# hasindu2008/sigtk

Measured on NVIDIA B200. Metric: event_detection_throughput, higher is better.
Workload: dtype f64

## Files before the change

### sigtk_b200/csrc/capi.cu

```cuda
#include "../../include/sigtk_b200.h"

#include <cstddef>
#include <cstdio>
#include <cstdlib>
#include <cstring>
#include <memory>
#include <new>
#include <utility>

#include "kernels.cuh"

using namespace sgpu;

namespace {

enum Out { EV_OFF, EV_START, EV_MEAN, EV_STDV, SEQ_ORDER, FIXUPS, STAT, ENT, JNN_CNT, JNN_SEG, PREFIX_POS, PREFIX_STAT,
           PA, N_OUT };
enum Live { LIVE_EV_OFF, LIVE_EV_START, LIVE_EV_LEN, LIVE_EV_MEAN, LIVE_EV_STDV, N_LIVE_OUT };
static_assert(EV_OFF == 0 && LIVE_EV_OFF == 0, "row 0 of both tables: ev_off, which sizes the event outputs");

enum Count : uint8_t {
    READS, READS_PLUS_1, EVENTS,
    SAMPLES,
    JNN_SLOTS,
};

constexpr int ANY_WANT = 0x100;

struct OutSpec {
    size_t field;
    uint32_t size;
    uint32_t want;
    Count count;
    uint32_t per;
    bool eager;
    int empty;
    bool pa_in;
};

#define OUTPUT(field, want, count, per, eager, empty, pa_in) \
    { offsetof(sgpu_result_t, field), sizeof *sgpu_result_t{}.field, want, count, per, eager, empty, pa_in }
constexpr OutSpec OUTS[] = {
    OUTPUT(ev_off,      SGPU_WANT_EVENTS, READS_PLUS_1, 1,   true,  0 | ANY_WANT, true),
    OUTPUT(ev_start,    SGPU_WANT_EVENTS, EVENTS,       1,   true,  -1,           true),
    OUTPUT(ev_mean,     SGPU_WANT_EVENTS, EVENTS,       1,   true,  -1,           true),
    OUTPUT(ev_stdv,     SGPU_WANT_EVENTS, EVENTS,       1,   true,  -1,           true),
    OUTPUT(seq_order,   SGPU_WANT_EVENTS, READS,        1,   true,  0,            true),
    OUTPUT(fixups,      SGPU_WANT_EVENTS, READS,        1,   true,  0,            true),
    OUTPUT(stat,        SGPU_WANT_STAT,   READS,        6,   true,  0,            false),
    OUTPUT(ent,         SGPU_WANT_ENT,    READS,        3,   false, 0,            false),
    OUTPUT(jnn_cnt,     SGPU_WANT_JNN,    READS,        1,   false, 0,            false),
    OUTPUT(jnn_seg,     SGPU_WANT_JNN,    JNN_SLOTS,    2,   false, -1,           false),
    OUTPUT(prefix_pos,  SGPU_WANT_PREFIX, READS,        4,   false, 0xff,         false),
    OUTPUT(prefix_stat, SGPU_WANT_PREFIX, READS,        6,   false, 0,            false),
    OUTPUT(pa,          SGPU_WANT_PA,     SAMPLES,      1,   false, -1,           false),
};
#undef OUTPUT
static_assert(sizeof OUTS / sizeof OUTS[0] == N_OUT, "one row per output");

#define LIVE_OUTPUT(field, count, empty) \
    { offsetof(sgpu_live_result_t, field), sizeof *sgpu_live_result_t{}.field, SGPU_WANT_EVENTS, count, 1, true, empty, \
      false }
constexpr OutSpec LIVE_OUTS[] = {
    LIVE_OUTPUT(ev_off,   READS_PLUS_1, 0 | ANY_WANT),
    LIVE_OUTPUT(ev_start, EVENTS,       -1),
    LIVE_OUTPUT(ev_len,   EVENTS,       -1),
    LIVE_OUTPUT(ev_mean,  EVENTS,       -1),
    LIVE_OUTPUT(ev_stdv,  EVENTS,       -1),
};
#undef LIVE_OUTPUT
static_assert(sizeof LIVE_OUTS / sizeof LIVE_OUTS[0] == N_LIVE_OUT, "one row per output");

constexpr uint32_t pa_input_wants(int k = 0) {
    return k == N_OUT ? 0u : (OUTS[k].pa_in ? OUTS[k].want : 0u) | pa_input_wants(k + 1);
}
constexpr bool pa_input_want_ok(uint32_t want) { return want != 0 && (want & ~pa_input_wants()) == 0; }
static_assert(pa_input_wants() == SGPU_WANT_EVENTS, "a pA run computes the event table only");

uint64_t out_elems(const OutSpec& s, uint64_t reads, uint64_t samples, uint64_t events) {
    switch (s.count) {
        case READS: return s.per * reads;
        case READS_PLUS_1: return s.per * (reads + 1);
        case EVENTS: return s.per * events;
        case SAMPLES: return s.per * samples;
        case JNN_SLOTS: return s.per * jnn_seg_capacity(samples, (uint32_t)reads);
    }
    return 0;
}

enum class Input : uint8_t { NONE, RAW, SVBZD, PA, LIVE, LIVE_PA };

bool is_live(Input k) { return k == Input::LIVE || k == Input::LIVE_PA; }

uint32_t allowed_wants(Input k) {
    if (k == Input::PA) return pa_input_wants();
    if (is_live(k)) return SGPU_WANT_EVENTS;
    return 63u;
}

struct Slot {
    sgpu_batch_t batch{};
    PinBuf<int16_t> samples;
    PinBuf<uint64_t> read_off;
    PinBuf<uint32_t> read_len;
    PinBuf<float> offset_f, raw_unit_f;
    uint64_t used = 0;
    DevBuf<int16_t> d_samples;
    DevBuf<uint64_t> d_read_off;
    DevBuf<uint32_t> d_read_len;
    DevBuf<float> d_offset, d_unit;
    DevBuf<void> dout[N_OUT];
    PinBuf<void> hout[N_OUT];
    PinBuf<unsigned long long> h_counters;
    PinBuf<int> h_status;
    cudaStream_t stream = nullptr;
    cudaEvent_t in_ready = nullptr, kernels_done = nullptr, small_back = nullptr;
    bool submitted = false;
    uint32_t want = 0;
    Input kind = Input::NONE;
    PinBuf<uint8_t> h_comp;
    DevBuf<uint8_t> d_comp;
    PinBuf<uint64_t> h_comp_off; DevBuf<uint64_t> d_comp_off;
    PinBuf<uint32_t> h_comp_len; DevBuf<uint32_t> d_comp_len;
    uint64_t comp_used = 0, svb_blocks = 0;
    PinBuf<uint32_t> h_channel, h_flags; DevBuf<uint32_t> d_channel, d_flags;
    DevBuf<void> live_dout[N_LIVE_OUT];
    PinBuf<void> live_hout[N_LIVE_OUT];
    std::unique_ptr<uint32_t[]> live_claim;
    uint32_t live_gen = 0;

    ~Slot() {
        if (stream) cudaStreamDestroy(stream);
        if (in_ready) cudaEventDestroy(in_ready);
        if (kernels_done) cudaEventDestroy(kernels_done);
        if (small_back) cudaEventDestroy(small_back);
    }
};

}

struct sgpu_ctx {
    int device = 0;
    int sm_count = 148;
    uint64_t max_samples = 0;
    uint32_t max_reads = 0;
    uint32_t n_slots = 0;
    uint32_t flags = 0;
    uint64_t ev_cap = 0;
    Scratch sc{};
    DevBuf<void> dev_out[N_OUT];
    std::unique_ptr<Slot[]> slots;
    SvbScratch svb{};
    DevBuf<float> jnn_mom;
    int pore_rna004 = 0;
    DevBuf<uint32_t> ent_ovf;
    PaScratch pa{};
    LiveScratch live{};
    DevBuf<void> live_dev_out[N_LIVE_OUT];
    std::unique_ptr<uint32_t[]> live_mirror;
    std::unique_ptr<uint8_t[]> live_form;
    bool live_mirror_stale = false;
    uint32_t live_gen = 0;
    uint64_t comp_cap = 0;
    cudaStream_t compute = nullptr;
    uint64_t last_launches = 0;
    static constexpr int MAX_STAGES = 16;
    cudaEvent_t stage_ev[MAX_STAGES + 1] = {};
    const char* stage_name[MAX_STAGES] = {};
    uint32_t stage_launches[MAX_STAGES] = {};
    int n_stages = 0;
    cudaStream_t stage_stream = nullptr;
    char err[512] = {0};

    ~sgpu_ctx() {
        if (compute) cudaStreamDestroy(compute);
        for (cudaEvent_t e : stage_ev) if (e) cudaEventDestroy(e);
    }
};

namespace {

bool cuda_fail(sgpu_ctx* c, cudaError_t e, const char* what, int line) {
    if (e == cudaSuccess) return false;
    if (c) snprintf(c->err, sizeof c->err, "%s: %s (%s) at capi.cu:%d", what, cudaGetErrorName(e),
                    cudaGetErrorString(e), line);
    return true;
}
#define CU(call)                                                         \
    do {                                                                 \
        if (cuda_fail(ctx, (call), #call, __LINE__)) return SGPU_E_CUDA; \
    } while (0)

uint64_t align_up(uint64_t v, uint64_t a) { return (v + a - 1) / a * a; }

template <size_t N, bool PINNED>
cudaError_t alloc_outputs(const OutSpec (&outs)[N], const sgpu_ctx* ctx, uint64_t ev_cap, Buf<void, PINNED>* o,
                          uint32_t want) {
    for (size_t k = 0; k < N; k++) {
        if (!outs[k].eager && !(want & outs[k].want)) continue;
        const uint64_t n = out_elems(outs[k], ctx->max_reads, ctx->max_samples, ev_cap);
        const cudaError_t e = o[k].ensure(n * outs[k].size);
        if (e != cudaSuccess) return e;
    }
    return cudaSuccess;
}

template <size_t N, typename R, bool PINNED>
void fill_result(const OutSpec (&outs)[N], R* r, const Buf<void, PINNED>* o, uint32_t want, bool all_eager) {
    for (size_t k = 0; k < N; k++)
        if ((want & outs[k].want) || (all_eager && outs[k].eager)) {
            void* const p = o[k];
            memcpy(reinterpret_cast<char*>(r) + outs[k].field, &p, sizeof p);
        }
}

template <size_t N>
cudaError_t queue_d2h(const OutSpec (&outs)[N], const DevBuf<void>* d, PinBuf<void>* h, const Slot& sl, uint32_t want,
                      bool by_events, uint64_t n_events) {
    for (size_t k = 0; k < N; k++) {
        if (!(want & outs[k].want) || (outs[k].count == EVENTS) != by_events) continue;
        const uint64_t n = out_elems(outs[k], sl.batch.n_reads, sl.used, n_events);
        const cudaError_t e = cudaMemcpyAsync(h[k], d[k], (size_t)n * outs[k].size, cudaMemcpyDeviceToHost, sl.stream);
        if (e != cudaSuccess) return e;
    }
    return cudaSuccess;
}

struct StageMarks {
    sgpu_ctx* ctx;
    cudaStream_t st;
    bool on;
    uint64_t launches = 0;
    StageMarks(sgpu_ctx* c, cudaStream_t s) : ctx(c), st(s), on((c->flags & SGPU_F_STAGE_TIMERS) != 0) {}
    int start() {
        CU(cudaMemsetAsync(ctx->sc.status, 0, sizeof(int), st));
        CU(cudaMemsetAsync(ctx->sc.counters, 0, 4 * sizeof(unsigned long long), st));
        ctx->n_stages = 0;
        ctx->stage_stream = st;
        if (on) cudaEventRecord(ctx->stage_ev[0], st);
        return SGPU_OK;
    }
    void done(const char* name, int n) {
        launches += (uint64_t)n;
        if (!on || ctx->n_stages >= sgpu_ctx::MAX_STAGES) return;
        const int k = ctx->n_stages++;
        ctx->stage_name[k] = name;
        ctx->stage_launches[k] = (uint32_t)n;
        cudaEventRecord(ctx->stage_ev[k + 1], st);
    }
    int finish() {
        CU(cudaGetLastError());
        ctx->last_launches = launches;
        return SGPU_OK;
    }
};

int alloc_svb_scratch(sgpu_ctx* ctx) {
    SvbScratch& w = ctx->svb;
    w.max_blocks = svbzd_max_blocks(ctx->max_samples, ctx->max_reads);
    CU(w.cnt.ensure(ctx->max_reads));
    CU(w.base.ensure((uint64_t)ctx->max_reads + 1));
    CU(w.blk_bytes.ensure(w.max_blocks));
    CU(w.blk_gpos.ensure(w.max_blocks + 1));
    CU(w.blk_sum.ensure(w.max_blocks));
    CU(w.blk_vpos.ensure(w.max_blocks + 1));
    CU(w.lane_sum.ensure(w.max_blocks * 32));
    CU(w.blk_read.ensure(w.max_blocks));
    return SGPU_OK;
}

template <size_t N>
int clear_empty_batch(const OutSpec (&outs)[N], uint64_t reads, uint64_t span, uint32_t want, DevBuf<void>* o,
                      StageMarks& run) {
    sgpu_ctx* const ctx = run.ctx;
    for (size_t k = 0; k < N; k++) {
        const OutSpec& s = outs[k];
        if (s.empty < 0 || !((want & s.want) || (s.empty & ANY_WANT))) continue;
        const uint64_t n = out_elems(s, reads, span, 0);
        if (n) CU(cudaMemsetAsync(o[k], s.empty & 0xff, (size_t)n * s.size, run.st));
    }
    return run.finish();
}

bool fits(const sgpu_ctx* ctx, const DevBatch& b) {
    return b.n_reads <= ctx->max_reads && b.span <= ctx->max_samples && !(b.span & (SGPU_ALIGN - 1));
}

int run_pipeline(sgpu_ctx* ctx, const DevBatch& b, uint32_t want, DevBuf<void>* o, cudaStream_t st,
                 const SvbBatch* svb = nullptr, int16_t* svb_out = nullptr) {
    Scratch& sc = ctx->sc;
    if (!fits(ctx, b)) return SGPU_E_INVAL;
    CU(alloc_outputs(OUTS, ctx, ctx->ev_cap, o, want));
    StageMarks marks(ctx, st);
    if (const int rc = marks.start()) return rc;
    if (b.n_reads == 0 || b.span == 0) return clear_empty_batch(OUTS, b.n_reads, b.span, want, o, marks);
    if (svb) marks.done("svbzd_decode", launch_svbzd_decode(*svb, ctx->svb, ctx->sc, svb_out, ctx->sm_count, st));
    const bool force_generic = (ctx->flags & SGPU_F_FORCE_GENERIC) != 0;
    const bool events = (want & SGPU_WANT_EVENTS) != 0;
    float* const pa = (want & SGPU_WANT_PA) ? static_cast<float*>(o[PA].get()) : nullptr;
    uint32_t* const seq = static_cast<uint32_t*>(o[SEQ_ORDER].get());
    uint32_t* const fix = static_cast<uint32_t*>(o[FIXUPS].get());
    if (pa && (!events || force_generic))
        marks.done("pa", launch_pa(b, pa, ctx->sm_count, st));
    if (want & SGPU_WANT_STAT) {
        float* const stat = static_cast<float*>(o[STAT].get());
        marks.done("stat_moments", launch_stat_moments(b, stat, ctx->sc.tune_stat_cta_min, ctx->sm_count, st));
        marks.done("stat_median", launch_stat_median(b, stat, ctx->sc.tune_stat_cta_min, ctx->sm_count, st));
    }
    if (want & SGPU_WANT_ENT) {
        if (!ctx->ent_ovf) {
            const uint64_t words = ent_overflow_words(ctx->sm_count);
            CU(ctx->ent_ovf.ensure(words));
            CU(cudaMemsetAsync(ctx->ent_ovf, 0, (size_t)words * sizeof(uint32_t), st));
        }
        marks.done("ent", launch_ent(b, ctx->ent_ovf, static_cast<double*>(o[ENT].get()), ctx->sm_count, st));
    }
    if (want & SGPU_WANT_JNN) {
        CU(ctx->jnn_mom.ensure((uint64_t)ctx->max_reads * 2));
        marks.done("jnn_moments", launch_jnn_moments(b, ctx->jnn_mom, ctx->sc.tune_stat_cta_min, ctx->sm_count, st));
        marks.done("jnn_walk", launch_jnn(b, ctx->jnn_mom, static_cast<uint32_t*>(o[JNN_CNT].get()),
                                          static_cast<int32_t*>(o[JNN_SEG].get()), ctx->sm_count, st));
    }
    if (want & SGPU_WANT_PREFIX)
        marks.done("prefix", launch_prefix(b, ctx->pore_rna004, static_cast<int32_t*>(o[PREFIX_POS].get()),
                                           static_cast<float*>(o[PREFIX_STAT].get()), ctx->sm_count, st));
    if (events) {
        const uint32_t n_tiles = fast_tiles_for(b.span);
        if (n_tiles > sc.max_tiles) return SGPU_E_INVAL;
        int n = launch_init_reads(b, sc, seq, fix, ctx->sm_count, st);
        if (force_generic) {
            CU(cudaMemsetAsync(sc.bitmap, 0, (size_t)n_tiles * (FAST_TILE / 32) * sizeof(uint32_t), st));
            marks.done("init", n);
        } else {
            marks.done("init", n);
            marks.done("walk_chunks", launch_walk(b, sc, pa, seq, ctx->sm_count, st));
            marks.done("long_jobs", launch_long_jobs(b, sc, seq, ctx->sm_count, st));
            marks.done("verify_chunks", launch_verify_chunks(b, sc, seq, fix, ctx->sm_count, st));
        }
        n = launch_build_seq_list(b, sc, seq, force_generic ? 1 : 0, ctx->sm_count, st);
        WorkList wl{sc.seq_list, sc.seq_sbase, sc.seq_count};
        n += launch_generic_detect(b, wl, sc, ctx->sm_count, st);
        marks.done("sequential_order_detect", n);
        uint64_t* const ev_off = static_cast<uint64_t*>(o[EV_OFF].get());
        uint32_t* const ev_start = static_cast<uint32_t*>(o[EV_START].get());
        float* const ev_mean = static_cast<float*>(o[EV_MEAN].get());
        float* const ev_stdv = static_cast<float*>(o[EV_STDV].get());
        marks.done("rank_events", launch_rank_events(b, sc, ev_off, ctx->sm_count, st));
        marks.done("emit_events",
                   launch_fast_emit(b, sc, ctx->ev_cap, ev_start, ev_mean, ev_stdv, fix, ctx->sm_count, st));
        marks.done("sequential_order_emit",
                   launch_generic_emit(b, wl, sc, ev_off, ctx->ev_cap, ev_start, ev_mean, ev_stdv, ctx->sm_count, st));
    }
    return marks.finish();
}

int alloc_pa_scratch(sgpu_ctx* ctx) {
    PaScratch& w = ctx->pa;
    w.max_tiles = pa_tile_capacity(ctx->max_samples, ctx->max_reads);
    CU(w.tile_cnt.ensure(ctx->max_reads));
    CU(w.tile_base.ensure((uint64_t)ctx->max_reads + 1));
    CU(w.tS.ensure(w.max_tiles));
    CU(w.tQ.ensure(w.max_tiles));
    CU(w.tA.ensure(w.max_tiles));
    CU(w.tB.ensure(w.max_tiles));
    CU(w.tmin.ensure(w.max_tiles));
    CU(w.ord_list.ensure(ctx->max_reads));
    CU(w.ord_sbase.ensure(ctx->max_reads));
    CU(w.ord_count.ensure(1));
    return SGPU_OK;
}

int grow_seq_scratch(sgpu_ctx* ctx) {
    Scratch& sc = ctx->sc;
    const uint64_t n = ctx->max_samples;
    DevBuf<double> S, Q;
    DevBuf<float> t1, t2;
    cudaError_t e = S.ensure(n);
    if (e == cudaSuccess) e = Q.ensure(n);
    if (e == cudaSuccess) e = t1.ensure(n);
    if (e == cudaSuccess) e = t2.ensure(n);
    if (e != cudaSuccess) {
        cudaGetLastError();
        snprintf(ctx->err, sizeof ctx->err, "growing the sequential-order scratch to %llu samples: %s",
                 (unsigned long long)n, cudaGetErrorString(e));
        return SGPU_E_NOMEM;
    }
    sc.Sinc = std::move(S); sc.Qinc = std::move(Q); sc.t1 = std::move(t1); sc.t2 = std::move(t2);
    sc.gen_cap = n;
    return SGPU_OK;
}

int run_pipeline_pa(sgpu_ctx* ctx, const DevBatch& b, const float* pa, uint32_t want, DevBuf<void>* o,
                    cudaStream_t st) {
    Scratch& sc = ctx->sc;
    if (!fits(ctx, b) || (b.n_reads && b.span && !pa)) return SGPU_E_INVAL;
    CU(alloc_outputs(OUTS, ctx, ctx->ev_cap, o, want));
    int rc = alloc_pa_scratch(ctx);
    if (!rc && b.span > sc.gen_cap) rc = grow_seq_scratch(ctx);
    if (rc) return rc;
    StageMarks marks(ctx, st);
    if ((rc = marks.start())) return rc;
    if (b.n_reads == 0 || b.span == 0) return clear_empty_batch(OUTS, b.n_reads, b.span, want, o, marks);
    const uint32_t n_tiles = fast_tiles_for(b.span);
    if (n_tiles > sc.max_tiles) return SGPU_E_INVAL;
    uint32_t* const seq = static_cast<uint32_t*>(o[SEQ_ORDER].get());
    uint32_t* const fix = static_cast<uint32_t*>(o[FIXUPS].get());
    CU(cudaMemsetAsync(sc.bitmap, 0, (size_t)n_tiles * (FAST_TILE / 32) * sizeof(uint32_t), st));
    const int force = (ctx->flags & SGPU_F_FORCE_GENERIC) ? 1 : 0;
    marks.done("pa_prefix", launch_pa_prefix(b, pa, ctx->pa, sc, seq, fix, force, ctx->sm_count, st));
    const WorkList ordered{ctx->pa.ord_list, ctx->pa.ord_sbase, ctx->pa.ord_count};
    const WorkList all{sc.seq_list, sc.seq_sbase, sc.seq_count};
    marks.done("sequential_order_detect", launch_generic_detect_pa(b, pa, ordered, all, sc, fix, ctx->sm_count, st));
    uint64_t* const ev_off = static_cast<uint64_t*>(o[EV_OFF].get());
    marks.done("rank_events", launch_rank_events(b, sc, ev_off, ctx->sm_count, st));
    marks.done("sequential_order_emit",
               launch_generic_emit(b, all, sc, ev_off, ctx->ev_cap, static_cast<uint32_t*>(o[EV_START].get()),
                                   static_cast<float*>(o[EV_MEAN].get()), static_cast<float*>(o[EV_STDV].get()),
                                   ctx->sm_count, st));
    return marks.finish();
}

int run_pipeline_live(sgpu_ctx* ctx, const LiveBatch& b, bool pa, DevBuf<void>* o, cudaStream_t st) {
    if (b.n_entries > ctx->max_reads || b.span > ctx->max_samples) return SGPU_E_INVAL;
    if (b.n_entries && (!b.samples || !b.read_off || !b.read_len || !b.channel || !b.flags ||
                        (!pa && (!b.offset || !b.unit))))
        return SGPU_E_INVAL;
    StageMarks marks(ctx, st);
    if (const int rc = marks.start()) return rc;
    if (b.n_entries == 0) return clear_empty_batch(LIVE_OUTS, 0, b.span, SGPU_WANT_EVENTS, o, marks);
    marks.done(pa ? "live_pa" : "live",
               launch_live(b, pa, ctx->live, ctx->sc, static_cast<uint64_t*>(o[LIVE_EV_OFF].get()),
                           static_cast<uint32_t*>(o[LIVE_EV_START].get()), static_cast<uint32_t*>(o[LIVE_EV_LEN].get()),
                           static_cast<float*>(o[LIVE_EV_MEAN].get()), static_cast<float*>(o[LIVE_EV_STDV].get()),
                           ctx->sm_count, st));
    return marks.finish();
}

int run_slot(sgpu_ctx* ctx, Slot& sl, uint32_t want) {
    const uint32_t nr = sl.batch.n_reads;
    const int rna = (int)sl.batch.rna;
    if (is_live(sl.kind)) {
        const LiveBatch b{sl.d_samples, sl.d_read_off, sl.d_read_len, sl.d_channel, sl.d_flags, sl.d_offset, sl.d_unit,
                          nr, sl.used};
        return run_pipeline_live(ctx, b, sl.kind == Input::LIVE_PA, sl.live_dout, ctx->compute);
    }
    CU(alloc_outputs(OUTS, ctx, ctx->ev_cap, sl.hout, want));
    if (sl.kind == Input::PA)
        return run_pipeline_pa(ctx, DevBatch{nullptr, sl.d_read_off, sl.d_read_len, nullptr, nullptr, nr, rna, sl.used},
                               reinterpret_cast<const float*>(sl.d_samples.get()), want, sl.dout, ctx->compute);
    const DevBatch b{sl.d_samples, sl.d_read_off, sl.d_read_len, sl.d_offset, sl.d_unit, nr, rna, sl.used};
    const SvbBatch svb{sl.d_comp, sl.comp_used, sl.d_comp_off, sl.d_comp_len, sl.d_read_off, sl.d_read_len, nr,
                       sl.svb_blocks};
    return run_pipeline(ctx, b, want, sl.dout, ctx->compute, sl.kind == Input::SVBZD ? &svb : nullptr, sl.d_samples);
}

bool accepts(const Slot& sl, Input k) { return !sl.submitted && (sl.kind == Input::NONE || sl.kind == k); }

int room_for(const sgpu_ctx* ctx, const Slot& sl, uint64_t n, uint64_t limit, uint64_t cap) {
    const uint64_t need = align_up(n, SGPU_ALIGN);
    if (n >= limit || need > cap) return SGPU_E_TOOBIG;
    if (sl.batch.n_reads >= ctx->max_reads || sl.used + need > cap) return SGPU_E_FULL;
    return SGPU_OK;
}

int64_t append_record(Slot& sl, uint64_t n, double digitisation, double offset, double range) {
    sgpu_batch_t& b = sl.batch;
    const uint32_t r = b.n_reads;
    b.read_off[r] = sl.used;
    b.read_len[r] = (uint32_t)n;
    const float range_f = (float)range, dig_f = (float)digitisation, off_f = (float)offset;
    volatile float unit = range_f / dig_f;
    b.offset_f[r] = off_f;
    b.raw_unit_f[r] = unit;
    sl.used += align_up(n, SGPU_ALIGN);
    b.n_reads = r + 1;
    b.read_off[r + 1] = sl.used;
    return (int64_t)r;
}

int add_live_entry(sgpu_ctx* ctx, Slot& sl, Input k, uint32_t channel, uint32_t flags, uint64_t n, uint64_t cap) {
    if (!accepts(sl, k) || !ctx->live.n_channels) return SGPU_E_STATE;
    if (channel >= ctx->live.n_channels || (flags & ~LIVE_FLAGS)) return SGPU_E_INVAL;
    if (const int rc = room_for(ctx, sl, n, 1ull << 31, cap)) return rc;
    if (sl.kind != k) {
        if (++ctx->live_gen == 0) {
            for (uint32_t s = 0; s < ctx->n_slots; s++)
                memset(ctx->slots[s].live_claim.get(), 0, (size_t)ctx->live.n_channels * sizeof(uint32_t));
            ctx->live_gen = 1;
        }
        sl.live_gen = ctx->live_gen;
    }
    if (sl.live_claim[channel] == sl.live_gen) return SGPU_E_INVAL;
    sl.live_claim[channel] = sl.live_gen;
    sl.kind = k;
    sl.h_channel[sl.batch.n_reads] = channel;
    sl.h_flags[sl.batch.n_reads] = flags;
    return SGPU_OK;
}

int map_dev_status(int s) {
    if (s == SGPU_DEV_E_EVCAP) return SGPU_E_EVCAP;
    if (s == SGPU_DEV_E_INVAL) return SGPU_E_INVAL;
    if (s == SGPU_DEV_E_STATE) return SGPU_E_STATE;
    if (s == SGPU_DEV_E_TOOBIG) return SGPU_E_TOOBIG;
    if (s == SGPU_DEV_E_SCRATCH) return SGPU_E_SCRATCH;
    if (s == SGPU_DEV_E_STREAM) return SGPU_E_STREAM;
    return SGPU_OK;
}

uint8_t live_form_of(Input k) { return k == Input::LIVE_PA ? LIVE_FORM_PA : LIVE_FORM_INT16; }

int check_live_entries(sgpu_ctx* ctx, const Slot& sl) {
    uint32_t* const mirror = ctx->live_mirror.get();
    uint8_t* const form = ctx->live_form.get();
    const uint32_t nc = ctx->live.n_channels;
    if (ctx->live_mirror_stale) {
        CU(cudaDeviceSynchronize());
        CU(cudaMemcpy(mirror, ctx->live.nopen, (size_t)nc * sizeof(uint32_t), cudaMemcpyDeviceToHost));
        CU(cudaMemcpy(form, ctx->live.form, (size_t)nc * sizeof(uint8_t), cudaMemcpyDeviceToHost));
        ctx->live_mirror_stale = false;
    }
    const uint8_t my_form = live_form_of(sl.kind);
    for (uint32_t e = 0; e < sl.batch.n_reads; e++) {
        const uint32_t c = sl.h_channel[e], f = sl.h_flags[e], no = mirror[c], len = sl.batch.read_len[e];
        const bool start = (f & SGPU_LIVE_START) != 0;
        if (!start && !(no & LIVE_OPEN) && (len || (f & SGPU_LIVE_END))) return SGPU_E_STATE;
        if (!start && (no & LIVE_OPEN) && form[c] != my_form) return SGPU_E_STATE;
        if ((start ? 0ull : (uint64_t)(no & ~LIVE_OPEN)) + len > 0x7fffffffull) return SGPU_E_TOOBIG;
    }
    return SGPU_OK;
}

void advance_live_mirror(sgpu_ctx* ctx, const Slot& sl) {
    uint32_t* const mirror = ctx->live_mirror.get();
    for (uint32_t e = 0; e < sl.batch.n_reads; e++) {
        const uint32_t c = sl.h_channel[e], f = sl.h_flags[e], no = mirror[c], len = sl.batch.read_len[e];
        const bool start = (f & SGPU_LIVE_START) != 0;
        if (!start && !(no & LIVE_OPEN)) continue;
        mirror[c] = (f & SGPU_LIVE_END) ? 0u : (uint32_t)((start ? 0u : (no & ~LIVE_OPEN)) + len) | LIVE_OPEN;
        if (start) ctx->live_form[c] = live_form_of(sl.kind);
    }
}

template <size_t N, typename R>
int wait_slot(sgpu_ctx* ctx, Slot& sl, const OutSpec (&outs)[N], const DevBuf<void>* d, PinBuf<void>* h,
              uint64_t ev_cap, R* out) {
    CU(cudaSetDevice(ctx->device));
    sl.submitted = false;
    CU(cudaEventSynchronize(sl.small_back));
    memset(out, 0, sizeof *out);
    const int dev_rc = map_dev_status(*sl.h_status);
    if (dev_rc) return dev_rc;
    const uint32_t nr = sl.batch.n_reads;
    if (sl.want & SGPU_WANT_EVENTS) {
        const uint64_t ne = nr ? static_cast<const uint64_t*>(h[0].get())[nr] : 0;
        if (ne > ev_cap) return SGPU_E_EVCAP;
        CU(queue_d2h(outs, d, h, sl, SGPU_WANT_EVENTS, true, ne));
        CU(cudaStreamSynchronize(sl.stream));
        out->n_events = ne;
    }
    fill_result(outs, out, h, sl.want, false);
    return SGPU_OK;
}

}

extern "C" {

int sgpu_abi_version(void) { return SGPU_ABI_VERSION; }

int sgpu_device_count(void) {
    int n = 0;
    if (cudaGetDeviceCount(&n) != cudaSuccess) return 0;
    return n;
}

const char* sgpu_strerror(int code) {
    switch (code) {
        case SGPU_OK: return "success";
        case SGPU_E_INVAL: return "invalid argument";
        case SGPU_E_CUDA: return "CUDA error (no usable B200 / kernel failure); there is no CPU fallback";
        case SGPU_E_NOMEM: return "out of memory";
        case SGPU_E_FULL: return "slot full";
        case SGPU_E_TOOBIG: return "read larger than the context's max_samples";
        case SGPU_E_STATE: return "call out of order";
        case SGPU_E_EVCAP: return "event capacity exceeded";
        case SGPU_E_SCRATCH: return "sequential-order scratch too small";
        case SGPU_E_STREAM: return "malformed svb-zd stream (length does not match its keys)";
        default: return "unknown error";
    }
}

const char* sgpu_last_error(const sgpu_ctx_t* ctx) { return ctx ? ctx->err : "no context"; }

int sgpu_create(sgpu_ctx_t** out, int device, uint64_t max_samples, uint32_t max_reads, uint32_t n_slots,
                uint32_t flags) {
    if (!out || max_samples == 0 || max_reads == 0 || (flags & ~15u)) return SGPU_E_INVAL;
    *out = nullptr;
    if (flags & SGPU_F_NO_HOST_SLOTS) n_slots = 0; else if (n_slots == 0) n_slots = 2;
    sgpu_ctx* ctx = new (std::nothrow) sgpu_ctx();
    if (!ctx) return SGPU_E_NOMEM;
    auto fail = [&](int code) { sgpu_destroy(ctx); return code; };
    {
        int ndev = 0;
        cudaError_t e = cudaGetDeviceCount(&ndev);
        if (e != cudaSuccess || device < 0 || device >= ndev) {
            fprintf(stderr, "[sigtk_b200] no usable CUDA device %d (%s); this library has no CPU fallback\n", device,
                    e == cudaSuccess ? "index out of range" : cudaGetErrorString(e));
            delete ctx;
            return SGPU_E_CUDA;
        }
    }
#define CUC(call)                                                               \
    do {                                                                        \
        if (cuda_fail(ctx, (call), #call, __LINE__)) {                          \
            fprintf(stderr, "[sigtk_b200] %s\n", ctx->err);                     \
            return fail(SGPU_E_CUDA);                                           \
        }                                                                       \
    } while (0)
    CUC(cudaSetDevice(device));
    ctx->device = device;
    cudaDeviceProp prop;
    CUC(cudaGetDeviceProperties(&prop, device));
    ctx->sm_count = prop.multiProcessorCount;
    max_samples = align_up(max_samples, 64);
    ctx->max_samples = max_samples;
    ctx->max_reads = max_reads;
    ctx->n_slots = n_slots;
    ctx->flags = flags;
    ctx->ev_cap = max_samples / 3 + 2ull * max_reads + 16;
    Scratch& sc = ctx->sc;
    sc.gen_cap = (max_samples <= (64ull << 20) || (flags & (SGPU_F_FORCE_GENERIC | SGPU_F_FULL_SEQ_SCRATCH)))
                     ? max_samples : max_samples / 8;
    CUC(sc.Sinc.ensure(sc.gen_cap));
    CUC(sc.Qinc.ensure(sc.gen_cap));
    CUC(sc.t1.ensure(sc.gen_cap));
    CUC(sc.t2.ensure(sc.gen_cap));
    sc.max_tiles = fast_tiles_for(max_samples) + 1;
    sc.bitmap_words = (uint64_t)sc.max_tiles * (FAST_TILE / 32);
    CUC(sc.bitmap.ensure(sc.bitmap_words));
    sc.wk_slots = walk_state_slots(max_samples, max_reads);
    CUC(sc.wk_begin.ensure(sc.wk_slots * 8));
    CUC(sc.wk_end.ensure(sc.wk_slots * 8));
    CUC(sc.wk_cnt.ensure(max_reads));
    CUC(sc.wk_ibase.ensure((uint64_t)max_reads + 1));
    sc.job_cap = walk_job_capacity(max_samples);
    CUC(sc.jobs.ensure((uint64_t)sc.job_cap * 4));
    CUC(sc.job_count.ensure(1));
    sc.tune_chunk_len = 0; sc.tune_warmup = 0; sc.tune_thr_long = 9.0f;
    sc.tune_stat_cta_min = STAT_CTA_MIN_DEFAULT;
    CUC(sc.tile_cnt.ensure(sc.max_tiles));
    CUC(sc.tile_read0.ensure(sc.max_tiles));
    CUC(sc.tile_base.ensure((uint64_t)sc.max_tiles + 1));
    CUC(sc.wit_min.ensure(max_reads));
    CUC(sc.wit_max.ensure(max_reads));
    CUC(sc.seq_list.ensure(max_reads));
    CUC(sc.seq_sbase.ensure((uint64_t)max_reads + 1));
    CUC(sc.seq_count.ensure(1));
    CUC(sc.cursor.ensure(1));
    {
        uint64_t most = sc.max_tiles > max_reads ? sc.max_tiles : max_reads;
        const uint64_t svb_blocks = svbzd_max_blocks(max_samples, max_reads);
        if (svb_blocks > most) most = svb_blocks;
        CUC(sc.scan_status.ensure(scan_tiles_for((uint32_t)most) + 1));
    }
    ctx->comp_cap = 2 * max_samples;
    if (flags & SGPU_F_STAGE_TIMERS)
        for (int k = 0; k <= sgpu_ctx::MAX_STAGES; k++) CUC(cudaEventCreate(&ctx->stage_ev[k]));
    CUC(sc.scan_ticket.ensure(1));
    CUC(sc.status.ensure(1));
    CUC(sc.counters.ensure(4));
    CUC(cudaStreamCreateWithFlags(&ctx->compute, cudaStreamNonBlocking));
    CUC(alloc_outputs(OUTS, ctx, ctx->ev_cap, ctx->dev_out, 0));
    if (n_slots) {
        ctx->slots.reset(new (std::nothrow) Slot[n_slots]);
        if (!ctx->slots) return fail(SGPU_E_NOMEM);
        for (uint32_t s = 0; s < n_slots; s++) {
            Slot& sl = ctx->slots[s];
            CUC(sl.samples.ensure(max_samples));
            CUC(sl.read_off.ensure((uint64_t)max_reads + 1));
            CUC(sl.read_len.ensure(max_reads));
            CUC(sl.offset_f.ensure(max_reads));
            CUC(sl.raw_unit_f.ensure(max_reads));
            CUC(sl.d_samples.ensure(max_samples));
            CUC(sl.d_read_off.ensure((uint64_t)max_reads + 1));
            CUC(sl.d_read_len.ensure(max_reads));
            CUC(sl.d_offset.ensure(max_reads));
            CUC(sl.d_unit.ensure(max_reads));
            CUC(alloc_outputs(OUTS, ctx, ctx->ev_cap, sl.dout, 0));
            CUC(alloc_outputs(OUTS, ctx, ctx->ev_cap, sl.hout, 0));
            CUC(sl.h_counters.ensure(4));
            CUC(sl.h_status.ensure(1));
            CUC(cudaStreamCreateWithFlags(&sl.stream, cudaStreamNonBlocking));
            CUC(cudaEventCreateWithFlags(&sl.in_ready, cudaEventDisableTiming));
            CUC(cudaEventCreateWithFlags(&sl.kernels_done, cudaEventDisableTiming));
            CUC(cudaEventCreateWithFlags(&sl.small_back, cudaEventDisableTiming));
            sl.batch = sgpu_batch_t{sl.samples, sl.read_off, sl.read_len, sl.offset_f, sl.raw_unit_f, 0, 0};
            sl.batch.read_off[0] = 0;
        }
    }
#undef CUC
    *out = ctx;
    return SGPU_OK;
}

void sgpu_destroy(sgpu_ctx_t* ctx) {
    if (!ctx) return;
    cudaSetDevice(ctx->device);
    cudaDeviceSynchronize();
    delete ctx;
}

int sgpu_slot_batch(sgpu_ctx_t* ctx, uint32_t slot, sgpu_batch_t** out) {
    if (!ctx || !out || slot >= ctx->n_slots) return SGPU_E_INVAL;
    *out = &ctx->slots[slot].batch;
    return SGPU_OK;
}

int sgpu_slot_reset(sgpu_ctx_t* ctx, uint32_t slot, uint32_t rna) {
    if (!ctx || slot >= ctx->n_slots) return SGPU_E_INVAL;
    Slot& sl = ctx->slots[slot];
    if (sl.submitted) return SGPU_E_STATE;
    sl.batch.n_reads = 0;
    sl.batch.rna = rna ? 1u : 0u;
    sl.batch.read_off[0] = 0;
    sl.used = 0;
    sl.kind = Input::NONE;
    sl.comp_used = 0;
    sl.svb_blocks = 0;
    return SGPU_OK;
}

int64_t sgpu_slot_add_read(sgpu_ctx_t* ctx, uint32_t slot, const int16_t* raw, uint64_t n, double digitisation,
                           double offset, double range) {
    if (!ctx || slot >= ctx->n_slots || (!raw && n)) return SGPU_E_INVAL;
    Slot& sl = ctx->slots[slot];
    if (!accepts(sl, Input::RAW)) return SGPU_E_STATE;
    if (const int rc = room_for(ctx, sl, n, 1ull << 31, ctx->max_samples)) return rc;
    sl.kind = Input::RAW;
    memcpy(sl.batch.samples + sl.used, raw, (size_t)n * sizeof(int16_t));
    return append_record(sl, n, digitisation, offset, range);
}

int64_t sgpu_slot_add_read_svbzd(sgpu_ctx_t* ctx, uint32_t slot, const uint8_t* stream, uint64_t n_bytes,
                                 double digitisation, double offset, double range) {
    if (!ctx || slot >= ctx->n_slots || !stream) return SGPU_E_INVAL;
    Slot& sl = ctx->slots[slot];
    if (!accepts(sl, Input::SVBZD)) return SGPU_E_STATE;
    if (n_bytes != 0 && n_bytes < 4) return SGPU_E_STREAM;
    uint32_t count = 0;
    if (n_bytes) memcpy(&count, stream, 4);
    const uint64_t n = count;
    if (n_bytes && (4u + (n + 3u) / 4u + n > n_bytes || n_bytes > 4u + (n + 3u) / 4u + 4u * n)) return SGPU_E_STREAM;
    const uint64_t cneed = align_up(n_bytes, 16);
    if (n_bytes > 0xffffffffull || cneed > ctx->comp_cap) return SGPU_E_TOOBIG;
    if (const int rc = room_for(ctx, sl, n, 1ull << 31, ctx->max_samples)) return rc;
    if (sl.comp_used + cneed > ctx->comp_cap) return SGPU_E_FULL;
    if (sl.kind != Input::SVBZD) {
        CU(cudaSetDevice(ctx->device));
        const int rc = alloc_svb_scratch(ctx);
        if (rc) return rc;
        CU(sl.h_comp.ensure(ctx->comp_cap));
        CU(sl.d_comp.ensure(ctx->comp_cap + 16));
        CU(sl.h_comp_off.ensure(ctx->max_reads));
        CU(sl.d_comp_off.ensure(ctx->max_reads));
        CU(sl.h_comp_len.ensure(ctx->max_reads));
        CU(sl.d_comp_len.ensure(ctx->max_reads));
    }
    sl.kind = Input::SVBZD;
    const uint32_t r = sl.batch.n_reads;
    if (n_bytes) memcpy(sl.h_comp + sl.comp_used, stream, (size_t)n_bytes);
    sl.h_comp_off[r] = sl.comp_used;
    sl.h_comp_len[r] = (uint32_t)n_bytes;
    sl.comp_used += cneed;
    sl.svb_blocks += svbzd_blocks_of(n);
    return append_record(sl, n, digitisation, offset, range);
}

int64_t sgpu_slot_add_read_pa(sgpu_ctx_t* ctx, uint32_t slot, const float* pa, uint64_t n) {
    if (!ctx || slot >= ctx->n_slots || (!pa && n)) return SGPU_E_INVAL;
    Slot& sl = ctx->slots[slot];
    if (!accepts(sl, Input::PA)) return SGPU_E_STATE;
    if (const int rc = room_for(ctx, sl, n, 1ull << 32, ctx->max_samples / 2)) return rc;
    sl.kind = Input::PA;
    memcpy(reinterpret_cast<float*>(sl.batch.samples) + sl.used, pa, (size_t)n * sizeof(float));
    return append_record(sl, n, 1.0, 0.0, 1.0);
}

int sgpu_submit(sgpu_ctx_t* ctx, uint32_t slot, uint32_t want) {
    if (!ctx || slot >= ctx->n_slots || (want & ~63u) || want == 0) return SGPU_E_INVAL;
    Slot& sl = ctx->slots[slot];
    if (sl.submitted) return SGPU_E_STATE;
    if (want & ~allowed_wants(sl.kind)) return SGPU_E_INVAL;
    CU(cudaSetDevice(ctx->device));
    const bool live = is_live(sl.kind);
    int rc = live ? check_live_entries(ctx, sl) : SGPU_OK;
    if (rc) return rc;
    const sgpu_batch_t& hb = sl.batch;
    const uint32_t nr = hb.n_reads;
    cudaStream_t st = sl.stream;
    if (sl.kind == Input::SVBZD) {
        CU(cudaMemcpyAsync(sl.d_comp, sl.h_comp, (size_t)sl.comp_used, cudaMemcpyHostToDevice, st));
        CU(cudaMemcpyAsync(sl.d_comp_off, sl.h_comp_off, (size_t)nr * sizeof(uint64_t), cudaMemcpyHostToDevice, st));
        CU(cudaMemcpyAsync(sl.d_comp_len, sl.h_comp_len, (size_t)nr * sizeof(uint32_t), cudaMemcpyHostToDevice, st));
    } else {
        const size_t sample_size = sl.kind == Input::PA || sl.kind == Input::LIVE_PA ? sizeof(float) : sizeof(int16_t);
        CU(cudaMemcpyAsync(sl.d_samples, hb.samples, (size_t)sl.used * sample_size, cudaMemcpyHostToDevice, st));
    }
    CU(cudaMemcpyAsync(sl.d_read_off, hb.read_off, ((size_t)nr + 1) * sizeof(uint64_t), cudaMemcpyHostToDevice, st));
    CU(cudaMemcpyAsync(sl.d_read_len, hb.read_len, (size_t)nr * sizeof(uint32_t), cudaMemcpyHostToDevice, st));
    CU(cudaMemcpyAsync(sl.d_offset, hb.offset_f, (size_t)nr * sizeof(float), cudaMemcpyHostToDevice, st));
    CU(cudaMemcpyAsync(sl.d_unit, hb.raw_unit_f, (size_t)nr * sizeof(float), cudaMemcpyHostToDevice, st));
    if (live) {
        CU(cudaMemcpyAsync(sl.d_channel, sl.h_channel, (size_t)nr * sizeof(uint32_t), cudaMemcpyHostToDevice, st));
        CU(cudaMemcpyAsync(sl.d_flags, sl.h_flags, (size_t)nr * sizeof(uint32_t), cudaMemcpyHostToDevice, st));
    }
    CU(cudaEventRecord(sl.in_ready, st));
    CU(cudaStreamWaitEvent(ctx->compute, sl.in_ready, 0));
    rc = run_slot(ctx, sl, want);
    if (rc) return rc;
    CU(cudaMemcpyAsync(sl.h_counters, ctx->sc.counters, 4 * sizeof(unsigned long long), cudaMemcpyDeviceToHost,
                       ctx->compute));
    CU(cudaMemcpyAsync(sl.h_status, ctx->sc.status, sizeof(int), cudaMemcpyDeviceToHost, ctx->compute));
    CU(cudaEventRecord(sl.kernels_done, ctx->compute));
    CU(cudaStreamWaitEvent(st, sl.kernels_done, 0));
    CU(live ? queue_d2h(LIVE_OUTS, sl.live_dout, sl.live_hout, sl, want, false, 0)
            : queue_d2h(OUTS, sl.dout, sl.hout, sl, want, false, 0));
    CU(cudaEventRecord(sl.small_back, st));
    if (live) advance_live_mirror(ctx, sl);
    sl.want = want;
    sl.submitted = true;
    return SGPU_OK;
}

int sgpu_wait(sgpu_ctx_t* ctx, uint32_t slot, sgpu_result_t* out) {
    if (!ctx || slot >= ctx->n_slots || !out) return SGPU_E_INVAL;
    Slot& sl = ctx->slots[slot];
    if (!sl.submitted || is_live(sl.kind)) return SGPU_E_STATE;
    return wait_slot(ctx, sl, OUTS, sl.dout, sl.hout, ctx->ev_cap, out);
}

int sgpu_run_device(sgpu_ctx_t* ctx, const sgpu_dev_batch_t* batch, uint32_t want, void* stream,
                    sgpu_result_t* out) {
    if (!ctx || !batch || !out || (want & ~63u) || want == 0) return SGPU_E_INVAL;
    CU(cudaSetDevice(ctx->device));
    DevBatch b{batch->samples, batch->read_off, batch->read_len, batch->offset_f, batch->raw_unit_f,
               batch->n_reads, (int)batch->rna, batch->span};
    const int rc = run_pipeline(ctx, b, want, ctx->dev_out, reinterpret_cast<cudaStream_t>(stream));
    if (rc) return rc;
    memset(out, 0, sizeof *out);
    fill_result(OUTS, out, ctx->dev_out, want, true);
    return SGPU_OK;
}

int sgpu_run_device_pa(sgpu_ctx_t* ctx, const sgpu_dev_pa_batch_t* batch, uint32_t want, void* stream,
                       sgpu_result_t* out) {
    if (!ctx || !batch || !out || !pa_input_want_ok(want)) return SGPU_E_INVAL;
    CU(cudaSetDevice(ctx->device));
    const DevBatch b{nullptr, batch->read_off, batch->read_len, nullptr, nullptr, batch->n_reads, (int)batch->rna,
                     batch->span};
    const int rc = run_pipeline_pa(ctx, b, batch->pa, want, ctx->dev_out, reinterpret_cast<cudaStream_t>(stream));
    if (rc) return rc;
    memset(out, 0, sizeof *out);
    fill_result(OUTS, out, ctx->dev_out, want, false);
    return SGPU_OK;
}

int sgpu_decode_svbzd_device(sgpu_ctx_t* ctx, const sgpu_svb_dev_batch_t* batch, int16_t* samples_out, void* stream) {
    if (!ctx || !batch || !samples_out) return SGPU_E_INVAL;
    if (batch->n_reads > ctx->max_reads || batch->n_blocks > svbzd_max_blocks(ctx->max_samples, ctx->max_reads))
        return SGPU_E_INVAL;
    CU(cudaSetDevice(ctx->device));
    const int arc = alloc_svb_scratch(ctx);
    if (arc) return arc;
    cudaStream_t st = reinterpret_cast<cudaStream_t>(stream);
    CU(cudaMemsetAsync(ctx->sc.status, 0, sizeof(int), st));
    SvbBatch s{batch->bytes, batch->n_bytes, batch->comp_off, batch->comp_len, batch->read_off, batch->read_len,
               batch->n_reads, batch->n_blocks};
    ctx->last_launches = (uint64_t)launch_svbzd_decode(s, ctx->svb, ctx->sc, samples_out, ctx->sm_count, st);
    CU(cudaGetLastError());
    return SGPU_OK;
}

int sgpu_counters(sgpu_ctx_t* ctx, sgpu_counters_t* out) {
    if (!ctx || !out) return SGPU_E_INVAL;
    CU(cudaSetDevice(ctx->device));
    CU(cudaDeviceSynchronize());
    unsigned long long c[4];
    int status = 0;
    CU(cudaMemcpy(c, ctx->sc.counters, sizeof c, cudaMemcpyDeviceToHost));
    CU(cudaMemcpy(&status, ctx->sc.status, sizeof status, cudaMemcpyDeviceToHost));
    out->n_events = c[0];
    out->n_seq_order_reads = c[1];
    out->n_fixups = c[2];
    out->n_kernel_launches = ctx->last_launches;
    out->status = map_dev_status(status);
    out->n_long_jobs = c[3];
    return SGPU_OK;
}

int sgpu_set_param(sgpu_ctx_t* ctx, int key, double value) {
    if (!ctx) return SGPU_E_INVAL;
    Scratch& sc = ctx->sc;
    switch (key) {
        case SGPU_PARAM_CHUNK_LEN:
            if (value < 0 || value > (double)(1u << 20)) return SGPU_E_INVAL;
            sc.tune_chunk_len = (uint32_t)value;
            return SGPU_OK;
        case SGPU_PARAM_WARMUP:
            if (value < 0 || value > 4096) return SGPU_E_INVAL;
            sc.tune_warmup = (uint32_t)value;
            return SGPU_OK;
        case SGPU_PARAM_PORE:
            if (value != 0 && value != 1) return SGPU_E_INVAL;
            ctx->pore_rna004 = (int)value;
            return SGPU_OK;
        case SGPU_PARAM_STAT_CTA_MIN:
            if (value < 0 || value > 4294967295.0) return SGPU_E_INVAL;
            sc.tune_stat_cta_min = (uint32_t)value;
            return SGPU_OK;
        case SGPU_PARAM_THR_LONG:
            if (!(value > 0 && value < 1e6)) return SGPU_E_INVAL;
            sc.tune_thr_long = (float)value;
            return SGPU_OK;
        default: return SGPU_E_INVAL;
    }
}

int sgpu_stage_times(sgpu_ctx_t* ctx, sgpu_stage_time_t* out, uint32_t cap) {
    if (!ctx || (!out && cap)) return SGPU_E_INVAL;
    if (!(ctx->flags & SGPU_F_STAGE_TIMERS)) return SGPU_E_STATE;
    CU(cudaSetDevice(ctx->device));
    if (ctx->n_stages == 0) return 0;
    CU(cudaEventSynchronize(ctx->stage_ev[ctx->n_stages]));
    int n = 0;
    for (int k = 0; k < ctx->n_stages && (uint32_t)k < cap; k++, n++) {
        float ms = 0.0f;
        CU(cudaEventElapsedTime(&ms, ctx->stage_ev[k], ctx->stage_ev[k + 1]));
        out[k].name = ctx->stage_name[k];
        out[k].ms = ms;
        out[k].launches = ctx->stage_launches[k];
    }
    return n;
}

int sgpu_memcpy_d2h(sgpu_ctx_t* ctx, void* dst, const void* src, uint64_t bytes) {
    if (!ctx || (!dst && bytes) || (!src && bytes)) return SGPU_E_INVAL;
    CU(cudaSetDevice(ctx->device));
    CU(cudaDeviceSynchronize());
    if (bytes) CU(cudaMemcpy(dst, src, (size_t)bytes, cudaMemcpyDeviceToHost));
    return SGPU_OK;
}

int sgpu_live_open(sgpu_ctx_t* ctx, uint32_t n_channels) {
    if (!ctx || n_channels == 0) return SGPU_E_INVAL;
    LiveScratch& w = ctx->live;
    if (w.n_channels) return SGPU_E_STATE;
    CU(cudaSetDevice(ctx->device));
    w.ev_cap = live_stage_base(ctx->max_samples, ctx->max_reads);
    CU(w.chan.ensure(n_channels));
    CU(w.nopen.ensure(n_channels));
    CU(w.claim.ensure(n_channels));
    CU(w.form.ensure(n_channels));
    CU(w.cnt.ensure(ctx->max_reads));
    CU(w.s_start.ensure(w.ev_cap));
    CU(w.s_len.ensure(w.ev_cap));
    CU(w.s_mean.ensure(w.ev_cap));
    CU(w.s_stdv.ensure(w.ev_cap));
    CU(cudaMemset(w.nopen, 0, (size_t)n_channels * sizeof(uint32_t)));
    CU(cudaMemset(w.claim, 0, (size_t)n_channels * sizeof(uint32_t)));
    CU(cudaMemset(w.form, LIVE_FORM_INT16, (size_t)n_channels * sizeof(uint8_t)));
    ctx->live_mirror.reset(new (std::nothrow) uint32_t[n_channels]());
    ctx->live_form.reset(new (std::nothrow) uint8_t[n_channels]());
    if (!ctx->live_mirror || !ctx->live_form) return SGPU_E_NOMEM;
    for (uint32_t s = 0; s < ctx->n_slots; s++) {
        Slot& sl = ctx->slots[s];
        CU(sl.h_channel.ensure(ctx->max_reads));
        CU(sl.h_flags.ensure(ctx->max_reads));
        CU(sl.d_channel.ensure(ctx->max_reads));
        CU(sl.d_flags.ensure(ctx->max_reads));
        CU(alloc_outputs(LIVE_OUTS, ctx, w.ev_cap, sl.live_dout, 0));
        CU(alloc_outputs(LIVE_OUTS, ctx, w.ev_cap, sl.live_hout, 0));
        sl.live_claim.reset(new (std::nothrow) uint32_t[n_channels]());
        if (!sl.live_claim) return SGPU_E_NOMEM;
    }
    w.n_channels = n_channels;
    return SGPU_OK;
}

int64_t sgpu_slot_add_live(sgpu_ctx_t* ctx, uint32_t slot, uint32_t channel, uint32_t flags, const int16_t* raw,
                           uint64_t n, double digitisation, double offset, double range) {
    if (!ctx || slot >= ctx->n_slots || (!raw && n)) return SGPU_E_INVAL;
    Slot& sl = ctx->slots[slot];
    if (const int rc = add_live_entry(ctx, sl, Input::LIVE, channel, flags, n, ctx->max_samples)) return rc;
    memcpy(sl.batch.samples + sl.used, raw, (size_t)n * sizeof(int16_t));
    return append_record(sl, n, digitisation, offset, range);
}

int64_t sgpu_slot_add_live_pa(sgpu_ctx_t* ctx, uint32_t slot, uint32_t channel, uint32_t flags, const float* pa,
                              uint64_t n) {
    if (!ctx || slot >= ctx->n_slots || (!pa && n)) return SGPU_E_INVAL;
    Slot& sl = ctx->slots[slot];
    if (const int rc = add_live_entry(ctx, sl, Input::LIVE_PA, channel, flags, n, ctx->max_samples / 2)) return rc;
    memcpy(reinterpret_cast<float*>(sl.batch.samples) + sl.used, pa, (size_t)n * sizeof(float));
    return append_record(sl, n, 1.0, 0.0, 1.0);
}

int sgpu_wait_live(sgpu_ctx_t* ctx, uint32_t slot, sgpu_live_result_t* out) {
    if (!ctx || slot >= ctx->n_slots || !out) return SGPU_E_INVAL;
    Slot& sl = ctx->slots[slot];
    if (!sl.submitted || !is_live(sl.kind)) return SGPU_E_STATE;
    return wait_slot(ctx, sl, LIVE_OUTS, sl.live_dout, sl.live_hout, ctx->live.ev_cap, out);
}

int sgpu_run_device_live(sgpu_ctx_t* ctx, const sgpu_dev_live_batch_t* batch, void* stream, sgpu_live_result_t* out) {
    if (!ctx || !batch || !out) return SGPU_E_INVAL;
    if (!ctx->live.n_channels) return SGPU_E_STATE;
    CU(cudaSetDevice(ctx->device));
    CU(alloc_outputs(LIVE_OUTS, ctx, ctx->live.ev_cap, ctx->live_dev_out, 0));
    const LiveBatch b{batch->samples, batch->read_off, batch->read_len, batch->channel, batch->flags, batch->offset_f,
                      batch->raw_unit_f, batch->n_entries, batch->span};
    const int rc = run_pipeline_live(ctx, b, false, ctx->live_dev_out, reinterpret_cast<cudaStream_t>(stream));
    if (rc) return rc;
    ctx->live_mirror_stale = true;
    memset(out, 0, sizeof *out);
    fill_result(LIVE_OUTS, out, ctx->live_dev_out, SGPU_WANT_EVENTS, false);
    return SGPU_OK;
}

int sgpu_run_device_live_pa(sgpu_ctx_t* ctx, const sgpu_dev_live_pa_batch_t* batch, void* stream,
                            sgpu_live_result_t* out) {
    if (!ctx || !batch || !out) return SGPU_E_INVAL;
    if (!ctx->live.n_channels) return SGPU_E_STATE;
    CU(cudaSetDevice(ctx->device));
    CU(alloc_outputs(LIVE_OUTS, ctx, ctx->live.ev_cap, ctx->live_dev_out, 0));
    LiveBatch b{nullptr, batch->read_off, batch->read_len, batch->channel, batch->flags, nullptr, nullptr,
                batch->n_entries, batch->span};
    b.pa = batch->pa;
    const int rc = run_pipeline_live(ctx, b, true, ctx->live_dev_out, reinterpret_cast<cudaStream_t>(stream));
    if (rc) return rc;
    ctx->live_mirror_stale = true;
    memset(out, 0, sizeof *out);
    fill_result(LIVE_OUTS, out, ctx->live_dev_out, SGPU_WANT_EVENTS, false);
    return SGPU_OK;
}

}
```

### sigtk_b200/csrc/common.cuh

```cuda
#pragma once
#include <cuda_runtime.h>
#include <float.h>
#include <stdint.h>

namespace sgpu {

struct DetParams {
    int w1, w2;
    float thr1, thr2;
    float height;
};

__host__ __device__ inline DetParams det_params(int rna) {
    DetParams p;
    if (rna) { p.w1 = 7; p.w2 = 14; p.thr1 = 2.5f; p.thr2 = 9.0f; p.height = 1.0f; }
    else     { p.w1 = 3; p.w2 = 6;  p.thr1 = 1.4f; p.thr2 = 9.0f; p.height = 0.2f; }
    return p;
}

struct DevBatch {
    const int16_t*  samples;
    const uint64_t* read_off;
    const uint32_t* read_len;
    const float*    offset;
    const float*    unit;
    uint32_t n_reads;
    int      rna;
    uint64_t span;
};

__device__ __forceinline__ float pa_of(int16_t raw, float off, float unit) {
    return __fmul_rn(__fadd_rn((float)raw, off), unit);
}

__device__ __forceinline__ float tstat_reference_chain(double sum1, double ssq1, double sum2d,
                                                       double ssq2d, float wf) {
    const double wd = (double)wf;
    const float sum2 = __double2float_rn(sum2d);
    const float ssq2 = __double2float_rn(ssq2d);
    const float mean1 = __double2float_rn(__ddiv_rn(sum1, wd));
    const float mean2 = __fdiv_rn(sum2, wf);
    const float m1sq = __fmul_rn(mean1, mean1);
    const float m2sq = __fmul_rn(mean2, mean2);
    const float v2 = __fdiv_rn(ssq2, wf);
    double acc = __ddiv_rn(ssq1, wd);
    acc = __dsub_rn(acc, (double)m1sq);
    acc = __dadd_rn(acc, (double)v2);
    acc = __dsub_rn(acc, (double)m2sq);
    const float cv = fmaxf(__double2float_rn(acc), FLT_MIN);
    const float delta = __fsub_rn(mean2, mean1);
    const float scaled = __fdiv_rn(cv, wf);
    return __double2float_rn(__ddiv_rn(fabs((double)delta), __dsqrt_rn((double)scaled)));
}


__device__ __forceinline__ void event_stats(double dsum, double dssq, uint32_t len, float* mean,
                                            float* stdv) {
    const float lenf = (float)len;
    const float m = __fdiv_rn(__double2float_rn(dsum), lenf);
    const float ex2 = __fdiv_rn(__double2float_rn(dssq), lenf);
    const float var = __fsub_rn(ex2, __fmul_rn(m, m));
    *mean = m;
    *stdv = __fsqrt_rn(fmaxf(var, 0.0f));
}

struct DetState {
    uint32_t masked_to;
    int32_t  peak_pos;
    float    peak_value;
    int32_t  valid;
};

__device__ __forceinline__ void det_reset(DetState& d) {
    d.masked_to = 0; d.peak_pos = -1; d.peak_value = FLT_MAX; d.valid = 0;
}

__device__ __forceinline__ int32_t det_step(DetState& d, DetState* other_long, bool is_short, uint32_t i,
                                            float cur, float thr, int w, float height) {
    if (d.masked_to >= i) return -1;
    if (d.peak_pos < 0) {
        if (cur < d.peak_value) {
            d.peak_value = cur;
        } else if (__fsub_rn(cur, d.peak_value) > height) {
            d.peak_value = cur;
            d.peak_pos = (int32_t)i;
        }
        return -1;
    }
    if (cur > d.peak_value) { d.peak_value = cur; d.peak_pos = (int32_t)i; }
    if (is_short && d.peak_value > thr) {
        other_long->masked_to = (uint32_t)d.peak_pos + (uint32_t)w;
        other_long->peak_pos = -1;
        other_long->peak_value = FLT_MAX;
        other_long->valid = 0;
    }
    if (__fsub_rn(d.peak_value, cur) > height && d.peak_value > thr) d.valid = 1;
    if (d.valid && (i - (uint32_t)d.peak_pos) > (uint32_t)(w / 2)) {
        const int32_t out = d.peak_pos;
        d.peak_pos = -1;
        d.peak_value = cur;
        d.valid = 0;
        return out;
    }
    return -1;
}

static inline int grid_cap(uint64_t work, int block, int max_blocks) {
    uint64_t g = (work + block - 1) / block;
    if (g < 1) g = 1;
    if (g > (uint64_t)max_blocks) g = max_blocks;
    return (int)g;
}

__device__ __forceinline__ uint32_t find_read(const uint64_t* __restrict__ off, uint32_t n, uint64_t p) {
    uint32_t lo = 0, hi = n;
    while (hi - lo > 1) {
        const uint32_t mid = (lo + hi) >> 1;
        if (off[mid] <= p) lo = mid; else hi = mid;
    }
    return lo;
}

}
```

### sigtk_b200/csrc/emit.cu

```cuda
#include "kernels.cuh"
#include "walk_core.cuh"

namespace sgpu {

namespace {

constexpr int EWT = 1024;
constexpr int EWARPS = 4;
constexpr int ELIST = EWT / 2 + 8;
constexpr int EFAST = EWT / 3 + 8;
constexpr int ELONG = 48;

struct EmitWarp {
    double S[EFAST + 32];
    double Q[EFAST + 32];
    uint16_t list[ELIST];
};

__device__ __forceinline__ uint32_t locate_read(const DevBatch& b, uint32_t r0, uint64_t p) {
    uint32_t r = r0;
#pragma unroll 1
    for (int k = 0; k < 4; k++) {
        if (r + 1 >= b.n_reads || b.read_off[r + 1] > p) return r;
        r++;
    }
    return find_read(b.read_off, b.n_reads, p);
}

__device__ __forceinline__ void add_raw(int raw, float off, float unit, double& as, double& aq) {
    const float x = __fmul_rn(__fadd_rn((float)raw, off), unit);
    as = __dadd_rn(as, walk::widen_pos(x));
    aq = __dadd_rn(aq, walk::widen_pos(__fmul_rn(x, x)));
}
__device__ __forceinline__ void add_raw_any(int raw, float off, float unit, double& as, double& aq, bool safe) {
    const float x = __fmul_rn(__fadd_rn((float)raw, off), unit);
    if (!safe || x > 0.0f) {
        as = __dadd_rn(as, walk::widen_pos(x));
        aq = __dadd_rn(aq, walk::widen_pos(__fmul_rn(x, x)));
    } else {
        as = __dadd_rn(as, (double)x);
        aq = __dadd_rn(aq, (double)__fmul_rn(x, x));
    }
}

__device__ __forceinline__ long long next_start(const uint32_t* __restrict__ bitmap, uint64_t w0, uint64_t n_words,
                                                long long rend) {
    for (uint64_t w = w0; w < n_words && (long long)(w << 5) < rend; w++) {
        const uint32_t nx = bitmap[w];
        if (nx) {
            const long long e = (long long)(w << 5) + __ffs(nx) - 1;
            return e < rend ? e : rend;
        }
    }
    return rend;
}

}

#ifndef EMIT_MINB
#define EMIT_MINB 7
#endif
#ifndef EMIT_GRID
#define EMIT_GRID 64
#endif
__global__ void __launch_bounds__(EWARPS * 32, EMIT_MINB) emit_events_kernel(DevBatch b, uint32_t n_tiles,
                                                                  const uint32_t* __restrict__ bitmap,
                                                                  const uint64_t* __restrict__ tile_base, uint64_t ev_cap,
                                                                  uint32_t* __restrict__ ev_start,
                                                                  float* __restrict__ ev_mean, float* __restrict__ ev_stdv,
                                                                  int* __restrict__ status,
                                                                  const uint32_t* __restrict__ tile_read0) {
    __shared__ EmitWarp smem[EWARPS];
    const int lane = threadIdx.x & 31;
    EmitWarp& sm = smem[threadIdx.x >> 5];
    const uint64_t n_wt = (uint64_t)n_tiles * (FAST_TILE / EWT);
    const uint64_t n_words = (uint64_t)n_tiles * (FAST_TILE / 32);
    const uint64_t warp0 = (uint64_t)blockIdx.x * EWARPS + (threadIdx.x >> 5), n_warps = (uint64_t)gridDim.x * EWARPS;
    const long long span = (long long)b.span;
    auto load_tile = [&](uint64_t wt, uint32_t& word, int4 (&rv)[4]) {
        const long long p0 = (long long)wt * EWT + lane * 32;
        word = 0u;
#pragma unroll
        for (int g = 0; g < 4; g++) rv[g] = make_int4(0, 0, 0, 0);
        if (wt < n_wt && (long long)wt * EWT < span) {
            word = bitmap[wt * 32 + lane];
            const int4* __restrict__ src = reinterpret_cast<const int4*>(b.samples + p0);
#pragma unroll
            for (int g = 0; g < 4; g++) if (p0 + 8 * g + 8 <= span) rv[g] = __ldg(src + g);
        }
    };
    uint32_t word_n;
    int4 rv_n[4];
    load_tile(warp0, word_n, rv_n);
    for (uint64_t wt = warp0; wt < n_wt; wt += n_warps) {
        const long long flat0 = (long long)wt * EWT;
        if (flat0 >= span) break;
        const uint32_t tile = (uint32_t)(wt / (FAST_TILE / EWT)), half = (uint32_t)(wt % (FAST_TILE / EWT));
        const uint32_t word = word_n;
        int4 rv[4];
#pragma unroll
        for (int g = 0; g < 4; g++) rv[g] = rv_n[g];
        load_tile(wt + n_warps, word_n, rv_n);
        const uint64_t tbase = tile_base[tile];
        const uint32_t tr0_raw = tile_read0[tile];
        const uint32_t tr0 = tr0_raw & 0x7fffffffu;
        const bool tile_low = (tr0_raw >> 31) != 0u;
        uint32_t before = half ? (uint32_t)__popc(bitmap[(uint64_t)tile * (FAST_TILE / 32) + lane]) : 0u;
        before = __reduce_add_sync(0xffffffffu, before);
        uint32_t incl = __popc(word);
        const uint32_t own = incl;
#pragma unroll
        for (int o = 1; o < 32; o <<= 1) {
            const uint32_t t = __shfl_up_sync(0xffffffffu, incl, o);
            if (lane >= o) incl += t;
        }
        uint32_t total = __shfl_sync(0xffffffffu, incl, 31);
        if (total == 0u) continue;
        if (total > (uint32_t)ELIST) { total = ELIST; if (lane == 0) atomicExch(status, SGPU_DEV_E_EVCAP); }
        __syncwarp();
        {
            uint32_t rem = word, idx = incl - own;
            while (rem) {
                if (idx < (uint32_t)ELIST) sm.list[idx] = (uint16_t)(lane * 32 + __ffs(rem) - 1);
                idx++;
                rem &= rem - 1u;
            }
        }
        const uint64_t kbase = tbase + before;
        const uint32_t r_first = locate_read(b, tr0, (uint64_t)flat0);
        const long long rs_first = (long long)b.read_off[r_first];
        const long long rend_first = rs_first + (long long)b.read_len[r_first];
        const float off_first = b.offset[r_first], unit_first = b.unit[r_first];
        const bool one_read = rs_first <= flat0 && flat0 + EWT <= rend_first && total <= (uint32_t)EFAST && !tile_low;
        if (one_read) {
            const uint64_t w_next = (wt + 1) * 32 + (uint64_t)lane;
            const bool w_valid = w_next < n_words && (long long)(w_next << 5) < rend_first;
            const uint32_t next_bits = w_valid ? bitmap[w_next] : 0u;
            const long long i_behind = flat0 + EWT + lane;
            const int raw_behind = i_behind < rend_first ? (int)__ldg(b.samples + i_behind) : 0;
            int slot = EFAST + lane;
            int next = (int)(incl - own);
            double as = 0.0, aq = 0.0;
#pragma unroll
            for (int g = 0; g < 4; g++) {
                const int v[4] = {rv[g].x, rv[g].y, rv[g].z, rv[g].w};
                float x[8];
                walk::cvt8(v, off_first, unit_first, x);
                float xq[8];
#pragma unroll
                for (int m = 0; m < 8; m += 2) {
                    const walk::F2 p = {x[m], x[m + 1]};
                    const walk::F2 q = walk::f2sq(p);
                    xq[m] = q.lo; xq[m + 1] = q.hi;
                }
#pragma unroll
                for (int m = 0; m < 8; m++) {
                    if ((word >> (8 * g + m)) & 1u) {
                        sm.S[slot] = as;
                        sm.Q[slot] = aq;
                        slot = next++;
                        as = 0.0;
                        aq = 0.0;
                    }
                    as = __dadd_rn(as, walk::widen_pos(x[m]));
                    aq = __dadd_rn(aq, walk::widen_pos(xq[m]));
                }
            }
            sm.S[slot] = as;
            sm.Q[slot] = aq;
            __syncwarp();
            const uint32_t nz = __ballot_sync(0xffffffffu, own != 0u);
            if (own != 0u && incl != own) {
                double hs = sm.S[EFAST + lane], hq = sm.Q[EFAST + lane];
                const uint32_t lower = nz & ((1u << lane) - 1u);
                for (int l2 = lane - 1; l2 > 31 - __clz(lower); l2--) {
                    hs = __dadd_rn(hs, sm.S[EFAST + l2]);
                    hq = __dadd_rn(hq, sm.Q[EFAST + l2]);
                }
                const int prev = (int)(incl - own) - 1;
                sm.S[prev] = __dadd_rn(sm.S[prev], hs);
                sm.Q[prev] = __dadd_rn(sm.Q[prev], hq);
            }
            __syncwarp();
            const int last_word = 31 - __clz(nz);
            long long e_tail;
            {
                const uint32_t m = __ballot_sync(0xffffffffu, next_bits != 0u);
                const uint32_t all_valid = __ballot_sync(0xffffffffu, w_valid);
                if (m) {
                    const int l0 = __ffs(m) - 1;
                    const uint32_t bits0 = __shfl_sync(0xffffffffu, next_bits, l0);
                    e_tail = (long long)(((wt + 1) * 32 + (uint64_t)l0) << 5) + __ffs(bits0) - 1;
                    if (e_tail > rend_first) e_tail = rend_first;
                } else if (all_valid == 0xffffffffu) {
                    e_tail = next_start(bitmap, (wt + 2) * 32, n_words, rend_first);
                } else {
                    e_tail = rend_first;
                }
            }
            double tail_s = lane > last_word ? sm.S[EFAST + lane] : 0.0, tail_q = lane > last_word ? sm.Q[EFAST + lane] : 0.0;
            if (i_behind < e_tail) add_raw_any(raw_behind, off_first, unit_first, tail_s, tail_q, true);
            for (long long i = i_behind + 32; i < e_tail; i += 32) add_raw_any((int)__ldg(b.samples + i), off_first, unit_first, tail_s, tail_q, true);
#pragma unroll
            for (int o = 16; o; o >>= 1) {
                tail_s = __dadd_rn(tail_s, __shfl_xor_sync(0xffffffffu, tail_s, o));
                tail_q = __dadd_rn(tail_q, __shfl_xor_sync(0xffffffffu, tail_q, o));
            }
            for (uint32_t j0 = 0; j0 < total; j0 += 32) {
                const uint32_t j = j0 + lane;
                if (j >= total) continue;
                const int pos = sm.list[j];
                double es = sm.S[j], eq = sm.Q[j];
                long long e;
                if (j + 1 < total) {
                    e = flat0 + sm.list[j + 1];
                } else {
                    es = __dadd_rn(es, tail_s);
                    eq = __dadd_rn(eq, tail_q);
                    e = e_tail;
                }
                const uint64_t k = kbase + j;
                if (k >= ev_cap) { atomicExch(status, SGPU_DEV_E_EVCAP); continue; }
                const long long s = flat0 + pos;
                float mean, stdv;
                event_stats(es, eq, (uint32_t)(e - s), &mean, &stdv);
                ev_start[k] = (uint32_t)(s - rs_first);
                ev_mean[k] = mean;
                ev_stdv[k] = stdv;
            }
            continue;
        }
        __syncwarp();
        const bool safe = true;
        for (uint32_t j0 = 0; j0 < total; j0 += 32) {
            const uint32_t j = j0 + lane;
            const bool have = j < total;
            long long i = 0, e = 0, rs = 0;
            float off = 0.0f, unit = 0.0f;
            double as = 0.0, aq = 0.0;
            uint32_t len = 0;
            if (have) {
                const long long s = flat0 + sm.list[j];
                const uint32_t r = locate_read(b, r_first, (uint64_t)s);
                rs = (long long)b.read_off[r];
                const long long rend = rs + (long long)b.read_len[r];
                off = b.offset[r];
                unit = b.unit[r];
                e = j + 1 < total ? flat0 + sm.list[j + 1] : next_start(bitmap, (wt + 1) * 32, n_words, rend);
                if (e > rend) e = rend;
                len = (uint32_t)(e - s);
                i = s;
                const long long stop = e - s > ELONG ? s + ELONG : e;
                for (; i < stop; i++) add_raw_any((int)__ldg(b.samples + i), off, unit, as, aq, safe);
            }
            uint32_t longs = __ballot_sync(0xffffffffu, have && i < e);
            while (longs) {
                const int src = __ffs(longs) - 1;
                longs &= longs - 1u;
                const long long li = __shfl_sync(0xffffffffu, i, src), le = __shfl_sync(0xffffffffu, e, src);
                const float lo = __shfl_sync(0xffffffffu, off, src), lu = __shfl_sync(0xffffffffu, unit, src);
                double ps = 0.0, pq = 0.0;
                for (long long p = li + lane; p < le; p += 32) add_raw_any((int)__ldg(b.samples + p), lo, lu, ps, pq, safe);
#pragma unroll
                for (int o = 16; o; o >>= 1) {
                    ps = __dadd_rn(ps, __shfl_xor_sync(0xffffffffu, ps, o));
                    pq = __dadd_rn(pq, __shfl_xor_sync(0xffffffffu, pq, o));
                }
                if (lane == src) { as = __dadd_rn(as, ps); aq = __dadd_rn(aq, pq); }
            }
            if (have) {
                const uint64_t k = kbase + j;
                if (k >= ev_cap) { atomicExch(status, SGPU_DEV_E_EVCAP); continue; }
                float mean, stdv;
                event_stats(as, aq, len, &mean, &stdv);
                ev_start[k] = (uint32_t)(e - (long long)len - rs);
                ev_mean[k] = mean;
                ev_stdv[k] = stdv;
            }
        }
    }
}

__global__ void __launch_bounds__(256) sum_fixups_kernel(uint32_t n_reads, const uint32_t* __restrict__ fixups,
                                                         unsigned long long* __restrict__ counters) {
    unsigned long long acc = 0;
    for (uint32_t r = blockIdx.x * blockDim.x + threadIdx.x; r < n_reads; r += gridDim.x * blockDim.x) acc += fixups[r];
    if (acc) atomicAdd(&counters[2], acc);
}

int launch_fast_emit(const DevBatch& b, Scratch& sc, uint64_t ev_cap, uint32_t* ev_start, float* ev_mean,
                     float* ev_stdv, const uint32_t* fixups, int sm_count, cudaStream_t st) {
    const uint32_t n_tiles = fast_tiles_for(b.span);
    const uint64_t n_wt = (uint64_t)n_tiles * (FAST_TILE / EWT);
    emit_events_kernel<<<grid_cap(n_wt, EWARPS, sm_count * EMIT_GRID), EWARPS * 32, 0, st>>>(
        b, n_tiles, sc.bitmap, sc.tile_base, ev_cap, ev_start, ev_mean, ev_stdv, sc.status, sc.tile_read0);
    sum_fixups_kernel<<<grid_cap(b.n_reads, 256, sm_count * 4), 256, 0, st>>>(b.n_reads, fixups, sc.counters);
    return 2;
}

}
```

### sigtk_b200/csrc/kernels.cuh

```cuda
#pragma once
#include <type_traits>

#include "common.cuh"

namespace sgpu {

template <typename T, bool PINNED = false>
class Buf {
  public:
    Buf() = default;
    Buf(const Buf&) = delete;
    Buf& operator=(const Buf&) = delete;
    Buf(Buf&& o) noexcept : p_(o.p_) { o.p_ = nullptr; }
    Buf& operator=(Buf&& o) noexcept {
        if (this != &o) { release(); p_ = o.p_; o.p_ = nullptr; }
        return *this;
    }
    ~Buf() { release(); }

    cudaError_t ensure(uint64_t count) {
        if (p_) return cudaSuccess;
        size_t bytes = (size_t)(count ? count : 1);
        if constexpr (!std::is_void_v<T>) bytes *= sizeof(T);
        void* q = nullptr;
        const cudaError_t e = PINNED ? cudaHostAlloc(&q, bytes, cudaHostAllocDefault) : cudaMalloc(&q, bytes);
        if (e == cudaSuccess) p_ = static_cast<T*>(q);
        return e;
    }
    T* get() const { return p_; }
    operator T*() const { return p_; }

  private:
    void release() {
        if (!p_) return;
        if (PINNED) cudaFreeHost(p_); else cudaFree(p_);
    }
    T* p_ = nullptr;
};
template <typename T> using DevBuf = Buf<T, false>;
template <typename T> using PinBuf = Buf<T, true>;

enum { SGPU_DEV_OK = 0, SGPU_DEV_E_EVCAP = 1, SGPU_DEV_E_SCRATCH = 2, SGPU_DEV_E_STREAM = 3, SGPU_DEV_E_INVAL = 4,
       SGPU_DEV_E_STATE = 5, SGPU_DEV_E_TOOBIG = 6 };

constexpr int FAST_TILE = 2048;

struct WorkList {
    const uint32_t* list;
    const uint64_t* sbase;
    const uint32_t* count;
};

struct Scratch {
    DevBuf<double> Sinc, Qinc; DevBuf<float> t1, t2;
    uint64_t gen_cap;
    DevBuf<uint32_t> bitmap; uint64_t bitmap_words;
    DevBuf<uint32_t> tile_cnt; DevBuf<uint64_t> tile_base;
    DevBuf<uint32_t> tile_read0;
    DevBuf<uint32_t> wk_cnt;
    DevBuf<uint64_t> wk_ibase;
    DevBuf<int> wk_begin, wk_end;
    uint64_t wk_slots;
    DevBuf<int> jobs;
    DevBuf<uint32_t> job_count;
    uint32_t job_cap;
    uint32_t tune_chunk_len, tune_warmup;
    float tune_thr_long;
    uint32_t tune_stat_cta_min;
    uint32_t max_tiles;
    DevBuf<uint32_t> wit_min, wit_max;
    DevBuf<uint32_t> seq_list;
    DevBuf<uint64_t> seq_sbase;
    DevBuf<uint32_t> seq_count;
    DevBuf<unsigned long long> cursor;
    DevBuf<unsigned long long> scan_status; DevBuf<uint32_t> scan_ticket;
    DevBuf<int> status; DevBuf<unsigned long long> counters;
};

int launch_generic_detect(const DevBatch& b, const WorkList& wl, Scratch& sc, int sm_count, cudaStream_t st);
int launch_generic_emit(const DevBatch& b, const WorkList& wl, Scratch& sc, const uint64_t* ev_off, uint64_t ev_cap,
                        uint32_t* ev_start, float* ev_mean, float* ev_stdv, int sm_count, cudaStream_t st);
int launch_generic_detect_pa(const DevBatch& b, const float* pa, const WorkList& ordered, const WorkList& all,
                             Scratch& sc, uint32_t* fixups, int sm_count, cudaStream_t st);
int launch_scan_u32(const uint32_t* cnt, uint32_t n, uint64_t* off, uint64_t* total_out, Scratch& sc, cudaStream_t st);
uint32_t scan_tiles_for(uint32_t n);

uint32_t fast_tiles_for(uint64_t span);
int launch_init_reads(const DevBatch& b, Scratch& sc, uint32_t* seq_flag, uint32_t* fixups, int sm_count,
                      cudaStream_t st);
int launch_walk(const DevBatch& b, Scratch& sc, float* pa_out, uint32_t* seq_flag, int sm_count, cudaStream_t st);
int launch_long_jobs(const DevBatch& b, Scratch& sc, uint32_t* seq_flag, int sm_count, cudaStream_t st);
int launch_verify_chunks(const DevBatch& b, Scratch& sc, uint32_t* seq_flag, uint32_t* fixups, int sm_count, cudaStream_t st);
uint64_t walk_state_slots(uint64_t max_samples, uint32_t max_reads);
uint32_t walk_chunk_len(uint64_t span, uint32_t n_reads, int rna, int sm_count, uint32_t forced);
uint32_t walk_warmup(int rna, uint32_t forced);
uint32_t walk_job_capacity(uint64_t max_samples);
int launch_build_seq_list(const DevBatch& b, Scratch& sc, uint32_t* seq_flag, int force_all, int sm_count,
                          cudaStream_t st);
int launch_rank_events(const DevBatch& b, Scratch& sc, uint64_t* ev_off, int sm_count, cudaStream_t st);
int launch_fast_emit(const DevBatch& b, Scratch& sc, uint64_t ev_cap, uint32_t* ev_start, float* ev_mean,
                     float* ev_stdv, const uint32_t* fixups, int sm_count, cudaStream_t st);
int launch_pa(const DevBatch& b, float* pa, int sm_count, cudaStream_t st);

struct PaScratch {
    DevBuf<uint32_t> tile_cnt;
    DevBuf<uint64_t> tile_base;
    DevBuf<double> tS, tQ;
    DevBuf<double> tA, tB;
    DevBuf<uint2> tmin;
    DevBuf<uint32_t> ord_list;
    DevBuf<uint64_t> ord_sbase; DevBuf<uint32_t> ord_count;
    uint64_t max_tiles;
};
uint64_t pa_tile_capacity(uint64_t max_samples, uint32_t max_reads);
int launch_pa_prefix(const DevBatch& b, const float* pa, PaScratch& w, Scratch& sc, uint32_t* seq_flag,
                     uint32_t* fixups, int force_all, int sm_count, cudaStream_t st);

struct SvbBatch {
    const uint8_t*  bytes;
    uint64_t        n_bytes;
    const uint64_t* comp_off;
    const uint32_t* comp_len;
    const uint64_t* read_off;
    const uint32_t* read_len;
    uint32_t n_reads;
    uint64_t n_blocks;
};
struct SvbScratch {
    DevBuf<uint32_t> cnt; DevBuf<uint64_t> base;
    DevBuf<uint32_t> blk_bytes; DevBuf<uint64_t> blk_gpos;
    DevBuf<uint32_t> blk_sum; DevBuf<uint64_t> blk_vpos;
    DevBuf<uint32_t> lane_sum;
    DevBuf<uint32_t> blk_read;
    uint64_t max_blocks;
};
uint64_t svbzd_max_blocks(uint64_t max_samples, uint32_t max_reads);
uint32_t svbzd_blocks_of(uint64_t n);
int launch_svbzd_decode(const SvbBatch& s, SvbScratch& w, Scratch& sc, int16_t* samples, int sm_count, cudaStream_t st);

constexpr uint32_t LIVE_FLAGS = 7u;
constexpr uint32_t LIVE_OPEN = 1u << 31;
constexpr int LIVE_TAIL = 28;
constexpr uint8_t LIVE_FORM_INT16 = 0, LIVE_FORM_PA = 1;
struct LiveChan {
    double tS[LIVE_TAIL], tQ[LIVE_TAIL];
    double pS[2], pQ[2];
    double aS, aQ;
    DetState det[2];
    uint32_t a;
    float offset, unit;
    uint32_t rna;
};
struct LiveBatch {
    union {
        const int16_t* samples;
        const float* pa;
    };
    const uint64_t* read_off;
    const uint32_t* read_len;
    const uint32_t* channel;
    const uint32_t* flags;
    const float* offset;
    const float* unit;
    uint32_t n_entries;
    uint64_t span;
};
__host__ __device__ inline uint64_t live_stage_base(uint64_t off, uint64_t e) { return off / 15 * 8 + 24 * e; }
struct LiveScratch {
    DevBuf<LiveChan> chan;
    DevBuf<uint32_t> nopen;
    DevBuf<uint32_t> claim;
    DevBuf<uint8_t> form;
    DevBuf<uint32_t> cnt;
    DevBuf<uint32_t> s_start, s_len;
    DevBuf<float> s_mean, s_stdv;
    uint32_t n_channels = 0;
    uint64_t ev_cap = 0;
    uint32_t stamp = 0;
};
int launch_live(const LiveBatch& b, bool pa, LiveScratch& w, Scratch& sc, uint64_t* ev_off, uint32_t* ev_start,
                uint32_t* ev_len, float* ev_mean, float* ev_stdv, int sm_count, cudaStream_t st);

constexpr uint32_t STAT_CTA_MIN_DEFAULT = 131072u;
int launch_stat_moments(const DevBatch& b, float* stat6, uint32_t cta_min, int sm_count, cudaStream_t st);
int launch_stat_median(const DevBatch& b, float* stat6, uint32_t cta_min, int sm_count, cudaStream_t st);
int launch_jnn_moments(const DevBatch& b, float* moments2, uint32_t cta_min, int sm_count, cudaStream_t st);

uint64_t jnn_seg_capacity(uint64_t max_samples, uint32_t max_reads);
int launch_jnn(const DevBatch& b, const float* moments, uint32_t* seg_cnt, int32_t* seg, int sm_count, cudaStream_t st);


int launch_prefix(const DevBatch& b, int rna004, int32_t* pos4, float* st6, int sm_count, cudaStream_t st);

uint64_t ent_overflow_words(int sm_count);
int launch_ent(const DevBatch& b, uint32_t* overflow, double* out3, int sm_count, cudaStream_t st);

}
```

### sigtk_b200/csrc/walk.cu

```cuda
#include <cstdlib>

#include "kernels.cuh"
#include "walk_core.cuh"

namespace sgpu {

namespace {

using namespace walk;

#ifndef WALK_NT
#define WALK_NT 128
#endif
#ifndef WALK_MINB
#define WALK_MINB 3
#endif
#ifndef WALK_MINB_RNA
#define WALK_MINB_RNA 2
#endif
constexpr int WNT = WALK_NT;

struct WalkParams {
    DevBatch b;
    int L, W;
    const uint64_t* ibase;
    float* pa;
    uint32_t* bitmap;
    int* st_begin;
    int* st_end;
    uint32_t* wit_min;
    uint32_t* wit_max;
    uint32_t* tile_read0;
    uint32_t edge_blocks;
    float thr_long;
    int4* jobs;
    uint32_t* job_count;
    uint32_t job_cap;
    uint32_t* seq_flag;
    unsigned long long* counters;
};

struct DevIo {
    const int16_t* __restrict__ sp;
    float* __restrict__ pa;
    uint32_t* __restrict__ bm;
    int* __restrict__ st_begin;
    int* __restrict__ st_end;
    uint32_t* __restrict__ wit_min;
    uint32_t* __restrict__ wit_max;
    uint32_t* __restrict__ tile_read0;
    uint64_t base;
    float off, unit;
    int4* __restrict__ jobs;
    uint32_t* __restrict__ job_count;
    uint32_t job_cap;
    uint32_t* __restrict__ seq_flag;
    int read, chunk;
    unsigned lanes;

    __device__ __forceinline__ void load8(int t, int (&v)[4]) const {
        const int4 w = __ldg(reinterpret_cast<const int4*>(sp + t));
        v[0] = w.x; v[1] = w.y; v[2] = w.z; v[3] = w.w;
    }
    __device__ __forceinline__ bool want_pa() const { return pa != nullptr; }
    __device__ __forceinline__ void prefetch(int t) const {
#if !defined(WALK_NO_PREFETCH)
        asm volatile("prefetch.global.L1 [%0];" ::"l"(sp + t));
#endif
    }
    __device__ __forceinline__ int warp_max(int v) const { return __reduce_max_sync(lanes, v); }
    __device__ __forceinline__ void store_pa8(int t, const float* x) const {
        float4* dst = reinterpret_cast<float4*>(pa + t);
        __stcs(dst, make_float4(x[0], x[1], x[2], x[3]));
        __stcs(dst + 1, make_float4(x[4], x[5], x[6], x[7]));
    }
    __device__ __forceinline__ void store_pa1(int t, float x) const { pa[t] = x; }
    __device__ __forceinline__ void peak(int pos) const { atomicOr(bm + ((uint32_t)pos >> 5), 1u << (pos & 31)); }
    __device__ __forceinline__ void peaks32(int ub, uint32_t mk) const {
        const uint32_t s = (uint32_t)ub & 31u;
        const uint32_t lo = mk << s, hi = __funnelshift_l(mk, 0u, s);
        uint32_t* w = bm + (ub >> 5);
        if (lo) atomicOr(w, lo);
        if (hi) atomicOr(w + 1, hi);
    }
    static __device__ __forceinline__ void store_canon(int* __restrict__ dst, const Canon& c) {
        int4* p = reinterpret_cast<int4*>(dst);
        p[0] = make_int4(c.v[0], c.v[1], c.v[2], c.v[3]);
        p[1] = make_int4(c.v[4], c.v[5], c.v[6], c.v[7]);
    }
    __device__ __forceinline__ void put_begin(const Canon& c) const { store_canon(st_begin, c); }
    __device__ __forceinline__ void put_end(const Canon& c) const { store_canon(st_end, c); }
    __device__ __forceinline__ void witness(int rmin, int rmax, int low_t) const {
        const float xh = __fmul_rn(__fadd_rn((float)rmax, off), unit);
        const float xa = __fmul_rn(__fadd_rn((float)rmin, off), unit);
        atomicMax(wit_max, max(__float_as_uint(xa) & 0x7fffffffu, __float_as_uint(xh) & 0x7fffffffu));
        const int gmin = rmin > low_t ? rmin : low_t + 1;
        if (gmin <= rmax) {
            const float xl = __fmul_rn(__fadd_rn((float)gmin, off), unit);
            atomicMin(wit_min, xl > 0.0f ? __float_as_uint(xl) : 1u);
        }
    }
    __device__ __forceinline__ void job(int l_start, int end) const {
        const uint32_t k = atomicAdd(job_count, 1u);
        if (k < job_cap) jobs[k] = make_int4(read, chunk, l_start, end);
        else seq_flag[read] = 1u;
    }
    __device__ __forceinline__ void low_samples(int t, uint32_t lo, uint32_t hi) const {
        atomicMin(wit_min, lo);
        atomicMax(wit_max, hi);
        atomicOr(tile_read0 + ((base + (uint64_t)(uint32_t)t) / FAST_TILE), 0x80000000u);
    }
};

__device__ __forceinline__ DevIo make_io(const WalkParams& p, uint32_t r, uint64_t sid, int chunk, int* sh) {
    const uint64_t base = p.b.read_off[r];
    *sh = (int)(base & 31u);
    DevIo io;
    io.sp = p.b.samples + base;
    io.pa = p.pa ? p.pa + base : nullptr;
    io.bm = p.bitmap + (base >> 5);
    io.st_begin = p.st_begin + sid * 8;
    io.st_end = p.st_end + sid * 8;
    io.wit_min = p.wit_min + r;
    io.wit_max = p.wit_max + r;
    io.tile_read0 = p.tile_read0;
    io.base = base;
    io.off = p.b.offset[r];
    io.unit = p.b.unit[r];
    io.jobs = p.jobs; io.job_count = p.job_count; io.job_cap = p.job_cap; io.seq_flag = p.seq_flag;
    io.read = (int)r; io.chunk = chunk;
    return io;
}

template <int RNA>
__device__ __noinline__ void walk_edge_dev(const WalkParams& p, uint32_t r, int last, unsigned lanes) {
    int sh;
    const int n = (int)p.b.read_len[r];
    DevIo io = make_io(p, r, 2ull * r + (uint64_t)last, last ? (int)n_chunks((uint32_t)n, (uint32_t)p.L) - 1 : 0, &sh);
    io.lanes = lanes;
    walk_edge<RNA>(io, n, io.off, io.unit, sh, p.L, p.W, last, p.thr_long);
}

__device__ __forceinline__ uint32_t find_chunk_read(const uint64_t* __restrict__ ibase, uint32_t n_reads, uint64_t i) {
    uint32_t lo = 0, hi = n_reads;
    while (hi - lo > 1) {
        const uint32_t mid = (lo + hi) >> 1;
        if (ibase[mid] <= i) lo = mid; else hi = mid;
    }
    return lo;
}

template <int RNA>
__global__ void __launch_bounds__(WNT, RNA ? WALK_MINB_RNA : WALK_MINB) walk_chunks_kernel(const WalkParams p) {
    if (blockIdx.x < p.edge_blocks) {
        const uint32_t per_kind = (p.b.n_reads + 31u) & ~31u;
        const uint64_t e = (uint64_t)blockIdx.x * WNT + threadIdx.x;
        const int last = e >= per_kind;
        const uint64_t r = last ? e - per_kind : e;
        const bool have = r < p.b.n_reads && e < 2ull * per_kind;
        const unsigned lanes = __ballot_sync(0xffffffffu, have);
        if (have) walk_edge_dev<RNA>(p, (uint32_t)r, last, lanes);
        return;
    }
    const uint64_t i = (uint64_t)(blockIdx.x - p.edge_blocks) * WNT + threadIdx.x;
    if (i >= p.ibase[p.b.n_reads]) return;
    const uint32_t r = find_chunk_read(p.ibase, p.b.n_reads, i);
    int sh;
    const int k = (int)(i - p.ibase[r]) + 1;
    DevIo io = make_io(p, r, 2ull * p.b.n_reads + i, k, &sh);
    walk_interior<RNA>(io, (int)p.b.read_len[r], io.off, io.unit, sh, p.L, p.W, k, p.thr_long);
}

struct JobIo {
    const int16_t* __restrict__ sp;
    uint32_t* __restrict__ bm;
    const int* __restrict__ st_end;
    uint64_t sid_first, sid_last, sid_int0;
    int nch;
    __device__ __forceinline__ void load8(int t, int (&v)[4]) const {
        const int4 w = __ldg(reinterpret_cast<const int4*>(sp + t));
        v[0] = w.x; v[1] = w.y; v[2] = w.z; v[3] = w.w;
    }
    __device__ __forceinline__ void peak(int pos) const { atomicOr(bm + ((uint32_t)pos >> 5), 1u << (pos & 31)); }
    __device__ __forceinline__ const int* rec(int kk) const {
        const uint64_t sid = kk == 0 ? sid_first : kk == nch - 1 ? sid_last : sid_int0 + (uint64_t)(kk - 1);
        return st_end + sid * 8;
    }
    __device__ __forceinline__ int end_lstart(int kk) const { return rec(kk)[6]; }
    __device__ __forceinline__ void end_short(int kk, float* pv, int* ps) const {
        const int* q = rec(kk);
        *pv = __int_as_float(q[0]); *ps = q[1];
    }
};

template <int RNA>
__device__ void long_job_warp(const JobIo& io, int n, int sh, float off, float unit, int L, int k, int l_start, int end,
                              float thr_long, int lane) {
    using C = Cfg<RNA>;
    constexpr int w1 = C::w1, w2 = C::w2;
    for (int kk = k - 1; l_start == LS_PRED && kk >= 0; kk--) l_start = io.end_lstart(kk);
    if (l_start == LS_PRED) return;
    const int stop = n + sh;
    const int own_end = end == LS_CONT ? (k + 1) * L - C::LAG + sh : (end < stop ? end : stop);
    float pv = FLT_MAX; int ps = PS_NONE;
    PeakAcc unused; unused.mk = 0u; unused.oldest = 0;
    bool b2; int p2;
    auto t_at = [&](int u, int w) -> float {
        const int i = u - sh;
        return (i >= w && i + w <= n) ? tstat_exact(io, i, w, n, off, unit) : 0.0f;
    };
    auto emit = [&](int pos) { if (lane == 0) io.peak(pos); };
    for (int base = l_start; base < own_end; base += 32) {
        const float t = base + lane < own_end ? t_at(base + lane, w2) : 0.0f;
        const int cnt = min(32, own_end - base);
        for (int q = 0; q < cnt; q++)
            det_one<false, RNA>(pv, ps, 0, base + q, __shfl_sync(0xffffffffu, t, q), thr_long, unused, b2, p2, emit);
    }
    if (end != LS_CONT) return;
    float spv; int sps;
    io.end_short(k, &spv, &sps);
    for (int base = own_end; base < stop; base += 32) {
        const bool in = base + lane < stop;
        const float t1 = in ? t_at(base + lane, w1) : 0.0f, t2 = in ? t_at(base + lane, w2) : 0.0f;
        const int cnt = min(32, stop - base);
        for (int q = 0; q < cnt; q++) {
            det_one<true, RNA>(spv, sps, 0, base + q, __shfl_sync(0xffffffffu, t1, q), thr_short<RNA>(), unused, b2, p2, NoEmit());
            if (b2) return;
            det_one<false, RNA>(pv, ps, 0, base + q, __shfl_sync(0xffffffffu, t2, q), thr_long, unused, b2, p2, emit);
        }
    }
}

template <int RNA>
__global__ void __launch_bounds__(128) long_jobs_kernel(const WalkParams p) {
    const uint32_t nj = min(*p.job_count, p.job_cap);
    if (blockIdx.x == 0 && threadIdx.x == 0) p.counters[3] = nj;
    const uint32_t tid = blockIdx.x * blockDim.x + threadIdx.x, nt = gridDim.x * blockDim.x;
    const int lane = threadIdx.x & 31;
    for (uint32_t j = RNA ? tid >> 5 : tid; j < nj; j += RNA ? nt >> 5 : nt) {
        const int4 job = p.jobs[j];
        const uint32_t r = (uint32_t)job.x;
        const uint64_t base = p.b.read_off[r];
        const int n = (int)p.b.read_len[r];
        JobIo io;
        io.sp = p.b.samples + base;
        io.bm = p.bitmap + (base >> 5);
        io.st_end = p.st_end;
        io.sid_first = 2ull * r; io.sid_last = 2ull * r + 1; io.sid_int0 = 2ull * p.b.n_reads + p.ibase[r];
        io.nch = (int)n_chunks((uint32_t)n, (uint32_t)p.L);
        if (RNA) long_job_warp<RNA>(io, n, (int)(base & 31u), p.b.offset[r], p.b.unit[r], p.L, job.y, job.z, job.w, p.thr_long, lane);
        else long_job<RNA>(io, n, (int)(base & 31u), p.b.offset[r], p.b.unit[r], p.L, job.y, job.z, job.w, p.thr_long);
    }
}

__global__ void __launch_bounds__(256) chunk_count_kernel(DevBatch b, uint32_t L, uint32_t* __restrict__ cnt) {
    for (uint32_t r = blockIdx.x * blockDim.x + threadIdx.x; r < b.n_reads; r += gridDim.x * blockDim.x) {
        const uint32_t nch = n_chunks(b.read_len[r], L);
        cnt[r] = nch > 2u ? nch - 2u : 0u;
    }
}

__global__ void __launch_bounds__(256) verify_chunks_kernel(DevBatch b, uint32_t L, const uint64_t* __restrict__ ibase,
                                                            const int* __restrict__ st_begin,
                                                            const int* __restrict__ st_end,
                                                            uint32_t* __restrict__ seq_flag,
                                                            uint32_t* __restrict__ fixups) {
    const uint64_t n_int = ibase[b.n_reads];
    const uint64_t total = n_int + b.n_reads;
    for (uint64_t t = (uint64_t)blockIdx.x * blockDim.x + threadIdx.x; t < total; t += (uint64_t)gridDim.x * blockDim.x) {
        uint32_t r;
        uint64_t cur, prev;
        if (t < n_int) {
            r = find_chunk_read(ibase, b.n_reads, t);
            cur = 2ull * b.n_reads + t;
            prev = (t == ibase[r]) ? 2ull * r : cur - 1;
        } else {
            r = (uint32_t)(t - n_int);
            const uint32_t nch = n_chunks(b.read_len[r], L);
            if (nch < 2u) continue;
            cur = 2ull * r + 1;
            prev = (nch == 2u) ? 2ull * r : 2ull * b.n_reads + ibase[r + 1] - 1;
        }
        const int4* a = reinterpret_cast<const int4*>(st_begin + cur * 8);
        const int4* e = reinterpret_cast<const int4*>(st_end + prev * 8);
        const int4 a0 = a[0], a1 = a[1], e0 = e[0], e1 = e[1];
        const bool same = a0.x == e0.x && a0.y == e0.y && a0.z == e0.z && a0.w == e0.w && a1.x == e1.x && a1.y == e1.y;
        if (!same) {
            seq_flag[r] = 1u;
            atomicAdd(&fixups[r], 1u);
        }
    }
}

}

uint32_t walk_chunk_len(uint64_t span, uint32_t n_reads, int rna, int sm_count, uint32_t forced) {
    const uint32_t lmin = rna ? 512u : 128u;
    const uint64_t want_chunks = (uint64_t)sm_count * (rna ? 2048ull : 384ull);
    uint32_t L = rna ? 4096u : 1024u;
    while (L > lmin && span / L < want_chunks) L >>= 1;
    if (n_reads) {
        const uint64_t per_read = span / n_reads / 12u / 128u * 128u;
        if (per_read < L) L = per_read > lmin ? (uint32_t)per_read : lmin;
    }
    if (forced >= lmin && forced % 32u == 0u) L = forced;
    return L;
}
uint32_t walk_warmup(int rna, uint32_t forced) {
    uint32_t W = rna ? 384u : 48u;
    const uint32_t u = rna ? 16u : 8u;
    if (forced != 0u && forced % u == 0u && forced <= W) W = forced;
    return W;
}
uint64_t walk_state_slots(uint64_t max_samples, uint32_t max_reads) { return 2ull * max_reads + max_samples / 128u + 1u; }
uint32_t walk_job_capacity(uint64_t max_samples) { return (uint32_t)(max_samples / 64u + 4096u); }

static WalkParams walk_params(const DevBatch& b, Scratch& sc, float* pa_out, uint32_t* seq_flag, int sm_count) {
    const uint32_t L = walk_chunk_len(b.span, b.n_reads, b.rna, sm_count, sc.tune_chunk_len), W = walk_warmup(b.rna, sc.tune_warmup);
    WalkParams p;
    p.b = b; p.L = (int)L; p.W = (int)W; p.ibase = sc.wk_ibase; p.pa = pa_out; p.bitmap = sc.bitmap;
    p.st_begin = sc.wk_begin; p.st_end = sc.wk_end; p.wit_min = sc.wit_min; p.wit_max = sc.wit_max; p.tile_read0 = sc.tile_read0;
    p.edge_blocks = (uint32_t)((2ull * ((b.n_reads + 31u) & ~31u) + WNT - 1) / WNT);
    p.thr_long = sc.tune_thr_long;
    p.jobs = reinterpret_cast<int4*>(sc.jobs.get()); p.job_count = sc.job_count; p.job_cap = sc.job_cap; p.seq_flag = seq_flag;
    p.counters = sc.counters;
    return p;
}

int launch_walk(const DevBatch& b, Scratch& sc, float* pa_out, uint32_t* seq_flag, int sm_count, cudaStream_t st) {
    const WalkParams p = walk_params(b, sc, pa_out, seq_flag, sm_count);
    const uint64_t words = (uint64_t)fast_tiles_for(b.span) * (FAST_TILE / 32);
    cudaMemsetAsync(sc.bitmap, 0, (size_t)words * sizeof(uint32_t), st);
    cudaMemsetAsync(sc.job_count, 0, sizeof(uint32_t), st);
    chunk_count_kernel<<<grid_cap(b.n_reads, 256, sm_count * 8), 256, 0, st>>>(b, (uint32_t)p.L, sc.wk_cnt);
    int n = 1 + launch_scan_u32(sc.wk_cnt, b.n_reads, sc.wk_ibase, nullptr, sc, st);
    const uint64_t max_interior = b.span / (uint32_t)p.L;
    const uint64_t grid = (uint64_t)p.edge_blocks + (max_interior + WNT - 1) / WNT;
    if (b.rna) walk_chunks_kernel<1><<<(unsigned)grid, WNT, 0, st>>>(p);
    else walk_chunks_kernel<0><<<(unsigned)grid, WNT, 0, st>>>(p);
    return n + 1;
}

int launch_long_jobs(const DevBatch& b, Scratch& sc, uint32_t* seq_flag, int sm_count, cudaStream_t st) {
    const WalkParams p = walk_params(b, sc, nullptr, seq_flag, sm_count);
    if (b.rna) long_jobs_kernel<1><<<sm_count * 16, 128, 0, st>>>(p);
    else long_jobs_kernel<0><<<sm_count * 4, 128, 0, st>>>(p);
    return 1;
}

int launch_verify_chunks(const DevBatch& b, Scratch& sc, uint32_t* seq_flag, uint32_t* fixups, int sm_count, cudaStream_t st) {
    const uint32_t L = walk_chunk_len(b.span, b.n_reads, b.rna, sm_count, sc.tune_chunk_len);
    const uint64_t max_interior = b.span / L;
    verify_chunks_kernel<<<grid_cap(max_interior + b.n_reads, 256, sm_count * 8), 256, 0, st>>>(
        b, L, sc.wk_ibase, sc.wk_begin, sc.wk_end, seq_flag, fixups);
    return 1;
}

}
```

### sigtk_b200/csrc/walk_core.cuh

```cuda
#pragma once
#include <float.h>
#include <math.h>
#include <stdint.h>
#include <string.h>

#if defined(__CUDACC__)
#define SGW_HD __host__ __device__ __forceinline__
#else
#define SGW_HD inline
#endif

namespace sgpu {
namespace walk {

#if defined(__CUDA_ARCH__)
SGW_HD double dadd(double a, double b) { return __dadd_rn(a, b); }
SGW_HD double dsub(double a, double b) { return __dsub_rn(a, b); }
SGW_HD double dmul(double a, double b) { return __dmul_rn(a, b); }
SGW_HD double dfma(double a, double b, double c) { return __fma_rn(a, b, c); }
SGW_HD double ddiv(double a, double b) { return __ddiv_rn(a, b); }
SGW_HD double dsqrt(double a) { return __dsqrt_rn(a); }
SGW_HD float fadd(float a, float b) { return __fadd_rn(a, b); }
SGW_HD float fsub(float a, float b) { return __fsub_rn(a, b); }
SGW_HD float fmul(float a, float b) { return __fmul_rn(a, b); }
SGW_HD float ffma(float a, float b, float c) { return __fmaf_rn(a, b, c); }
SGW_HD float fdiv(float a, float b) { return __fdiv_rn(a, b); }
SGW_HD float d2f(double a) { return __double2float_rn(a); }
SGW_HD uint32_t d_hi(double a) { return (uint32_t)__double2hiint(a); }
SGW_HD uint32_t d_lo(double a) { return (uint32_t)__double2loint(a); }
SGW_HD uint32_t f_bits(float a) { return __float_as_uint(a); }
SGW_HD float bits_f(uint32_t b) { return __uint_as_float(b); }
SGW_HD float rsqrt_seed(float a) {
    float y;
    asm("rsqrt.approx.ftz.f32 %0, %1;" : "=f"(y) : "f"(a));
    return y;
}
SGW_HD double widen_pos(float a) {
    return __longlong_as_double((long long)((unsigned long long)__float_as_uint(a) * 0x20000000ull + 0x3800000000000000ull));
}
SGW_HD double widen_abs(float a) { return (double)fabsf(a); }
SGW_HD uint32_t shr_clamp(uint32_t x, int s) {
    uint32_t r;
    asm("shr.b32 %0, %1, %2;" : "=r"(r) : "r"(x), "r"(s));
    return r;
}
struct F2 { float lo, hi; };
SGW_HD F2 f2mul(F2 a, F2 b) {
    F2 r;
    asm("{\n\t.reg .b64 a, b, d;\n\tmov.b64 a, {%2, %3};\n\tmov.b64 b, {%4, %5};\n\tmul.rn.f32x2 d, a, b;\n\t"
        "mov.b64 {%0, %1}, d;\n\t}" : "=f"(r.lo), "=f"(r.hi) : "f"(a.lo), "f"(a.hi), "f"(b.lo), "f"(b.hi));
    return r;
}
SGW_HD F2 f2sq(F2 a) {
    F2 r;
    asm("{\n\t.reg .b64 a, d;\n\tmov.b64 a, {%2, %3};\n\tmul.rn.f32x2 d, a, a;\n\tmov.b64 {%0, %1}, d;\n\t}"
        : "=f"(r.lo), "=f"(r.hi) : "f"(a.lo), "f"(a.hi));
    return r;
}
SGW_HD F2 f2add(F2 a, F2 b) {
    F2 r;
    asm("{\n\t.reg .b64 a, b, d;\n\tmov.b64 a, {%2, %3};\n\tmov.b64 b, {%4, %5};\n\tadd.rn.f32x2 d, a, b;\n\t"
        "mov.b64 {%0, %1}, d;\n\t}" : "=f"(r.lo), "=f"(r.hi) : "f"(a.lo), "f"(a.hi), "f"(b.lo), "f"(b.hi));
    return r;
}
SGW_HD F2 f2sub(F2 a, F2 b) {
    F2 r;
    asm("{\n\t.reg .b64 a, b, d;\n\tmov.b64 a, {%2, %3};\n\tmov.b64 b, {%4, %5};\n\tsub.rn.f32x2 d, a, b;\n\t"
        "mov.b64 {%0, %1}, d;\n\t}" : "=f"(r.lo), "=f"(r.hi) : "f"(a.lo), "f"(a.hi), "f"(b.lo), "f"(b.hi));
    return r;
}
SGW_HD F2 f2fma(F2 a, F2 b, F2 c) {
    F2 r;
    asm("{\n\t.reg .b64 a, b, c, d;\n\tmov.b64 a, {%2, %3};\n\tmov.b64 b, {%4, %5};\n\tmov.b64 c, {%6, %7};\n\t"
        "fma.rn.f32x2 d, a, b, c;\n\tmov.b64 {%0, %1}, d;\n\t}"
        : "=f"(r.lo), "=f"(r.hi) : "f"(a.lo), "f"(a.hi), "f"(b.lo), "f"(b.hi), "f"(c.lo), "f"(c.hi));
    return r;
}
#else
SGW_HD double dadd(double a, double b) { return a + b; }
SGW_HD double dsub(double a, double b) { return a - b; }
SGW_HD double dmul(double a, double b) { return a * b; }
SGW_HD double dfma(double a, double b, double c) { return fma(a, b, c); }
SGW_HD double ddiv(double a, double b) { return a / b; }
SGW_HD double dsqrt(double a) { return sqrt(a); }
SGW_HD float fadd(float a, float b) { return a + b; }
SGW_HD float fsub(float a, float b) { return a - b; }
SGW_HD float fmul(float a, float b) { return a * b; }
SGW_HD float ffma(float a, float b, float c) { return fmaf(a, b, c); }
SGW_HD float fdiv(float a, float b) { return a / b; }
SGW_HD float d2f(double a) { return (float)a; }
SGW_HD uint32_t d_hi(double a) { uint64_t b; memcpy(&b, &a, 8); return (uint32_t)(b >> 32); }
SGW_HD uint32_t d_lo(double a) { uint64_t b; memcpy(&b, &a, 8); return (uint32_t)b; }
SGW_HD uint32_t f_bits(float a) { uint32_t b; memcpy(&b, &a, 4); return b; }
SGW_HD float bits_f(uint32_t b) { float a; memcpy(&a, &b, 4); return a; }
SGW_HD float rsqrt_seed(float a) { return (float)(1.0 / sqrt((double)a)); }
SGW_HD double widen_pos(float a) {
    uint32_t b; memcpy(&b, &a, 4);
    const uint64_t v = (uint64_t)b * 0x20000000ull + 0x3800000000000000ull;
    double r; memcpy(&r, &v, 8); return r;
}
SGW_HD double widen_abs(float a) { return (double)fabsf(a); }
SGW_HD uint32_t shr_clamp(uint32_t x, int s) { return (unsigned)s < 32u ? x >> s : 0u; }
struct F2 { float lo, hi; };
SGW_HD F2 f2mul(F2 a, F2 b) { F2 r; r.lo = a.lo * b.lo; r.hi = a.hi * b.hi; return r; }
SGW_HD F2 f2sq(F2 a) { F2 r; r.lo = a.lo * a.lo; r.hi = a.hi * a.hi; return r; }
SGW_HD F2 f2add(F2 a, F2 b) { F2 r; r.lo = a.lo + b.lo; r.hi = a.hi + b.hi; return r; }
SGW_HD F2 f2sub(F2 a, F2 b) { F2 r; r.lo = a.lo - b.lo; r.hi = a.hi - b.hi; return r; }
SGW_HD F2 f2fma(F2 a, F2 b, F2 c) { F2 r; r.lo = fmaf(a.lo, b.lo, c.lo); r.hi = fmaf(a.hi, b.hi, c.hi); return r; }
#endif

template <int RNA>
struct Cfg {
    static constexpr int w1 = RNA ? 7 : 3;
    static constexpr int w2 = 2 * w1;
    static constexpr int LAG = w2 - 1;
    static constexpr int R1 = RNA ? 8 : 4;
    static constexpr int R2 = RNA ? 16 : 8;
    static constexpr int U = RNA ? 16 : 8;
    static constexpr int FILL = 2;
    static_assert(FILL * U >= 2 * w2 - 1, "fill covers the look-back of the first step");
};
template <int RNA> SGW_HD float thr_short() { return RNA ? 2.5f : 1.4f; }
template <int RNA> SGW_HD float thr_long() { return 9.0f; }
template <int RNA> SGW_HD float peak_h() { return RNA ? 1.0f : 0.2f; }

template <int W>
SGW_HD double ddivw(double a) {
    constexpr double r = 1.0 / (double)W;
    const double q0 = dmul(a, r);
    const double e = dfma(-(double)W, q0, a);
    return dfma(e, r, q0);
}
template <int W>
SGW_HD float fdivw(float a) {
    constexpr float r = 1.0f / (float)W;
    const float q0 = fmul(a, r);
    const float e = ffma(-(float)W, q0, a);
    return ffma(e, r, q0);
}

template <int WA, int WB>
SGW_HD F2 fdivw2(F2 a) {
    const F2 r = {1.0f / (float)WA, 1.0f / (float)WB};
    const F2 nw = {-(float)WA, -(float)WB};
    const F2 q0 = f2mul(a, r);
    const F2 e = f2fma(nw, q0, a);
    return f2fma(e, r, q0);
}

SGW_HD float tail(float delta, float scaled, float scaled_half, float cv, bool& ok) {
    const double ch = widen_pos(scaled_half);
    const double y0 = widen_pos(rsqrt_seed(scaled));
    const double th = dmul(ch, y0);
    const double eh = dfma(-th, y0, 0.5);
    const double q0 = dmul(widen_abs(delta), y0);
    const double q = dfma(q0, eh, q0);
    ok = ok & ((d_lo(q) * 8u - ((0x10000000u - 1024u) << 3)) >= (2048u << 3)) & (cv >= 2.0e-29f);
    return d2f(q);
}

template <int W>
SGW_HD void window_terms(double D, double E, float& A, double& Lq, float& B, double& Vd, double& B2d) {
    A = d2f(ddivw<W>(D));
    const F2 de = {d2f(D), d2f(E)};
    const F2 bv = fdivw2<W, W>(de);
    Lq = dsub(ddivw<W>(E), widen_pos(fmul(A, A)));
    B = bv.lo;
    Vd = widen_pos(bv.hi);
    B2d = widen_pos(fmul(B, B));
}
template <int W>
SGW_HD void tstat_two(float A0, double L0, float B0, double V0, double B0sq, float A1, double L1, float B1, double V1,
                      double B1sq, float& t0, bool& ok0, float& t1, bool& ok1) {
    const double acc0 = dsub(dadd(L0, V0), B0sq);
    const double acc1 = dsub(dadd(L1, V1), B1sq);
    const F2 cv = {d2f(acc0), d2f(acc1)};
    const F2 sc = fdivw2<W, W>(cv);
    const F2 half = {0.5f, 0.5f};
    const F2 sh = f2mul(sc, half);
#if defined(WALK_X_NOTAIL)
    t0 = fmul(fsub(B0, A0), sc.lo); t1 = fmul(fsub(B1, A1), sh.hi);
#else
    t0 = tail(fsub(B0, A0), sc.lo, sh.lo, cv.lo, ok0);
    t1 = tail(fsub(B1, A1), sc.hi, sh.hi, cv.hi, ok1);
#endif
}

template <class Io>
SGW_HD float sample_pa(const Io& io, int i, int n, float off, float unit) {
    if (i < 0 || i >= n) return 0.0f;
    int v[4];
    io.load8(i & ~7, v);
    const int q = i & 7;
    const int word = q < 2 ? v[0] : q < 4 ? v[1] : q < 6 ? v[2] : v[3];
    const int raw = (q & 1) ? (word >> 16) : (int)(int16_t)(word & 0xffff);
    return fmul(fadd((float)raw, off), unit);
}
template <class Io>
SGW_HD void window_sums(const Io& io, int a, int w, int n, float off, float unit, double& S, double& Q) {
    S = 0.0; Q = 0.0;
    for (int i = a; i < a + w; i++) {
        const float x = sample_pa(io, i, n, off, unit);
        S = dadd(S, (double)x);
        Q = dadd(Q, (double)fmul(x, x));
    }
}
SGW_HD float tstat_from_sums(double sum1, double ssq1, double sum2d, double ssq2d, int w) {
    const float wf = (float)w;
    const float sum2 = d2f(sum2d), ssq2 = d2f(ssq2d);
    const float mean1 = d2f(ddiv(sum1, (double)wf));
    const float mean2 = fdiv(sum2, wf);
    double acc = ddiv(ssq1, (double)wf);
    acc = dsub(acc, (double)fmul(mean1, mean1));
    acc = dadd(acc, (double)fdiv(ssq2, wf));
    acc = dsub(acc, (double)fmul(mean2, mean2));
    const float cv = fmaxf(d2f(acc), FLT_MIN);
    const float delta = fsub(mean2, mean1);
    return d2f(ddiv(fabs((double)delta), dsqrt((double)fdiv(cv, wf))));
}
template <class Io>
SGW_HD float tstat_exact(const Io& io, int i, int w, int n, float off, float unit) {
    double sum1, ssq1, sum2d, ssq2d;
    window_sums(io, i - w, w, n, off, unit, sum1, ssq1);
    window_sums(io, i, w, n, off, unit, sum2d, ssq2d);
    return tstat_from_sums(sum1, ssq1, sum2d, ssq2d, w);
}
template <class Io>
struct SlidingT {
    double s1, q1, s2, q2;
    int at;
    SGW_HD SlidingT() : s1(0.0), q1(0.0), s2(0.0), q2(0.0), at(-1) {}
    SGW_HD float next(const Io& io, int i, int w, int n, float off, float unit) {
        if (!(i >= w && i + w <= n)) { at = -1; return 0.0f; }
        if (at != i - 1) {
            window_sums(io, i - w, w, n, off, unit, s1, q1);
            window_sums(io, i, w, n, off, unit, s2, q2);
        } else {
            const float xa = sample_pa(io, i - 1 - w, n, off, unit);
            const float xb = sample_pa(io, i - 1, n, off, unit);
            const float xc = sample_pa(io, i - 1 + w, n, off, unit);
            const double da = (double)xa, db = (double)xb, dc = (double)xc;
            const double qa = (double)fmul(xa, xa), qb = (double)fmul(xb, xb), qc = (double)fmul(xc, xc);
            s1 = dadd(dsub(s1, da), db); q1 = dadd(dsub(q1, qa), qb);
            s2 = dadd(dsub(s2, db), dc); q2 = dadd(dsub(q2, qb), qc);
        }
        at = i;
        return tstat_from_sums(s1, q1, s2, q2, w);
    }
};
constexpr int PS_NONE = 0x7fff0000;
constexpr int PS_OPEN = 0x40000000;
constexpr int LS_PRED = -0x40000000;
constexpr int LS_CONT = 0x7fffffff;
struct WalkDet {
    float s_pv; int s_ps;
    int l_start;
    bool l_hot;
};
SGW_HD void det_cold(WalkDet& d, int first_step) {
    d.s_pv = FLT_MAX; d.s_ps = PS_NONE;
    d.l_start = first_step; d.l_hot = false;
}

struct Canon { int v[8]; };
template <int RNA>
SGW_HD Canon canon_of(const WalkDet& d, int b) {
    Canon c;
    (void)b;
    c.v[0] = (int)f_bits(d.s_pv); c.v[1] = d.s_ps; c.v[2] = 0; c.v[3] = 0; c.v[4] = 0; c.v[5] = 0;
    c.v[6] = d.l_start; c.v[7] = 0;
    return c;
}

template <int RNA> struct PkCfg {
    static constexpr int LEAD = 32 - Cfg<RNA>::U;
#if defined(WALK_TEST_FAR)
    static constexpr int FAR = 0;
#else
    static constexpr int FAR = LEAD - (Cfg<RNA>::w1 / 2 + 1);
#endif
};
struct PeakAcc { uint32_t mk; int oldest; int jobs, job_ls, job_end; };
struct NoEmit { SGW_HD void operator()(int) const {} };

template <bool SHORT, int RNA, class E>
SGW_HD int det_one(float& pv, int& ps, int m, int u, float c, float thr, PeakAcc& acc, bool& big2, int& p2,
                   const E& on_emit) {
    constexpr int w = SHORT ? Cfg<RNA>::w1 : Cfg<RNA>::w2;
    const float h = peak_h<RNA>();
    const bool none = ps == PS_NONE;
    const float df = fsub(c, pv);
    const float pvm = none ? fminf(pv, c) : fmaxf(pv, c);
    const bool rise1 = none & (df > h);
    const bool gt2 = !none & (df > 0.0f);
    big2 = !none & (pvm > thr);
    const bool drop = big2 & (df < -h);
    p2 = gt2 ? ((ps & PS_OPEN) | u) : ps;
    const int p3 = drop ? (p2 & ~PS_OPEN) : p2;
    const int over = (u - (w / 2 + 1)) - p3;
    const bool emit = over >= 0;
    acc.mk |= shr_clamp(1u << (PkCfg<RNA>::LEAD + m - (w / 2 + 1)), over);
    if (emit) on_emit(p3);
    pv = (rise1 | emit) ? c : pvm;
    ps = emit ? PS_NONE : p3;
    ps = rise1 ? (u | PS_OPEN) : ps;
    return over;
}

struct DualDet {
    float s_pv; int s_ps;
    float l_pv; int l_ps; int l_mt;
};
SGW_HD void dual_cold(DualDet& d, int first_step) {
    d.s_pv = FLT_MAX; d.s_ps = PS_NONE;
    d.l_pv = FLT_MAX; d.l_ps = PS_NONE; d.l_mt = first_step - 1;
}
SGW_HD Canon dual_canon(const DualDet& d, int b) {
    Canon c;
    c.v[0] = (int)f_bits(d.s_pv); c.v[1] = d.s_ps; c.v[2] = (int)f_bits(d.l_pv); c.v[3] = d.l_ps;
    c.v[4] = d.l_mt >= b ? d.l_mt : -1;
    c.v[5] = 0; c.v[6] = 0; c.v[7] = 0;
    return c;
}
template <int RNA, class E>
SGW_HD void dual_step(DualDet& d, int u, float c1, float c2, const E& on_emit) {
    bool maskl, unused_b; int p2, unused_p;
    PeakAcc unused; unused.mk = 0u; unused.oldest = 0;
    det_one<true, RNA>(d.s_pv, d.s_ps, 0, u, c1, thr_short<RNA>(), unused, maskl, p2, on_emit);
    d.l_mt = maskl ? (p2 & ~PS_OPEN) + Cfg<RNA>::w1 : d.l_mt;
    d.l_ps = maskl ? PS_NONE : d.l_ps;
    d.l_pv = maskl ? FLT_MAX : d.l_pv;
    const float c2m = d.l_mt < u ? c2 : FLT_MAX;
    det_one<false, RNA>(d.l_pv, d.l_ps, 0, u, c2m, thr_long<RNA>(), unused, unused_b, unused_p, on_emit);
}

constexpr int ZMAX = 1023;
struct LongK {
    float c0;
    float ca;
    float cw;
    float h2;
    float t2w;
    float cB;
    float thr;
};
template <int RNA>
SGW_HD LongK long_consts(int c0, float off, float thr_long) {
    constexpr float w = (float)Cfg<RNA>::w2;
    const float u = 5.9604644775390625e-08f;
    LongK k;
    k.c0 = (float)c0;
    const float M = fmul(fadd(fabsf(fadd(k.c0, off)), (float)(ZMAX + 2)), 1.0001f);
    k.ca = fmul(fmul(8.0f * u * w, M), 1.0001f);
    k.cw = w * (1.0f + 0.000244140625f);
    k.thr = thr_long;
    const float thr2 = fmul(thr_long, thr_long);
    k.h2 = fmul(thr2, 0.5f);
    k.t2w = fmul(thr2, w);
    k.cB = fmul(fmul(fmul(thr2, 64.0f * u * w * w), fmul(M, M)), 1.0001f);
    return k;
}
SGW_HD bool long_candidate(float dS, float T, float Q, const LongK& k) {
    const float g = fadd(fabsf(dS), k.ca);
    const float sq = ffma(T, T, fmul(dS, dS));
    const float lhs = ffma(fmul(g, g), k.cw, ffma(sq, k.h2, k.cB));
    const float rhs = fmul(Q, k.t2w);
    return !(lhs < rhs);
}

constexpr int DIRTY_BLOCKS = 3;
static_assert(2 * Cfg<0>::w2 - 1 <= 2 * Cfg<0>::U + 0 && 2 * Cfg<1>::w2 - 1 <= 2 * Cfg<1>::U, "windows reach at most two blocks ahead");

template <int RNA>
struct Rings {
    using C = Cfg<RNA>;
    double P[C::R1], PQ[C::R1];
    float A1[C::R1];
    double L1[C::R1];
    float T1c[C::w1];
    static constexpr int ZH2 = 2 * C::w2 - C::U;
    float Z1[C::U], Z2[ZH2];
    float zdS, zT, zQ;
    SGW_HD void clear() {
#pragma unroll
        for (int k = 0; k < C::R1; k++) { P[k] = 0.0; PQ[k] = 0.0; A1[k] = 0.0f; L1[k] = 0.0; }
#pragma unroll
        for (int k = 0; k < C::w1; k++) T1c[k] = 0.0f;
#pragma unroll
        for (int k = 0; k < C::U; k++) Z1[k] = 0.0f;
#pragma unroll
        for (int k = 0; k < ZH2; k++) Z2[k] = 0.0f;
        zdS = 0.0f; zT = 0.0f; zQ = 0.0f;
    }
};

template <int RNA, bool DIRECT, class E, class Io>
SGW_HD void det_step(WalkDet& d, int m, int u, float c1, bool cand, bool rec, PeakAcc& acc, const E& on_emit, Io& io) {
    bool maskl; int p2;
    const int over = det_one<true, RNA>(d.s_pv, d.s_ps, m, u, c1, thr_short<RNA>(), acc, maskl, p2, on_emit);
    acc.oldest = acc.oldest > over ? acc.oldest : over;
    bool hot = d.l_hot;
    if (maskl & hot & rec) {
        if (DIRECT) io.job(d.l_start, u);
        else { acc.job_ls = d.l_start; acc.job_end = u; acc.jobs++; }
    }
    const int ls = (p2 & ~PS_OPEN) + Cfg<RNA>::w1 + 1;
    d.l_start = maskl ? (ls > u ? ls : u) : d.l_start;
    hot = (hot & !maskl) | ((u >= d.l_start) & cand);
    d.l_hot = hot;
}

template <int RNA> struct Redo { WalkDet d; PeakAcc acc; float t1c[Cfg<RNA>::w1]; };
template <int RNA, bool EDGE, class Io>
#if defined(__CUDACC__)
__host__ __device__ __noinline__
#else
inline
#endif
Redo<RNA> redo_block(Io& io, Redo<RNA> in, int tau0, int n, int sh, bool rec, float off, float unit, float thr_long) {
    using C = Cfg<RNA>;
    constexpr int w1 = C::w1, w2 = C::w2, U = C::U;
    (void)thr_long;
    float e1[U];
    SlidingT<Io> slide;
    for (int m = 0; m < U; m++) e1[m] = slide.next(io, tau0 + m - w1 + 1, w1, n, off, unit);
    Redo<RNA> r;
    r.d = in.d; r.acc.mk = 0u; r.acc.oldest = 0; r.acc.jobs = 0;
    const int u0 = tau0 - w2 + 1 + sh;
    for (int m = 0; m < U; m++) {
        const int j2 = tau0 + m - w2 + 1;
        const float c1 = m >= w1 ? e1[m - w1] : in.t1c[m];
        if (!EDGE || (j2 >= 1 && j2 < n)) {
            PeakAcc unused; unused.mk = 0u; unused.oldest = 0; unused.jobs = 0;
            det_step<RNA, true>(r.d, 0, u0 + m, c1, true, rec, unused, [&](int pos) { if (rec) io.peak(pos); }, io);
        }
    }
    for (int k = 0; k < w1; k++) r.t1c[k] = e1[U - w1 + k];
    return r;
}

template <int RNA, bool EDGE, class Io>
SGW_HD void walk_block(Rings<RNA>& g, WalkDet& d, const float (&x)[Cfg<RNA>::U], const float (&z)[Cfg<RNA>::U], int tau0,
                       int n, int sh, bool rec, bool live, bool live_t1, int dirty, int zdirty, float off, float unit,
                       const LongK& lk, Io& io) {
    using C = Cfg<RNA>;
    constexpr int w1 = C::w1, w2 = C::w2, M1 = C::R1 - 1, M2 = C::R2 - 1, U = C::U;
    float t1v[U];
    bool ok = true, ok_t1 = true;
    const WalkDet d0 = d;
    PeakAcc acc;
    acc.mk = 0u; acc.oldest = 0; acc.jobs = 0;
    const int u0 = tau0 - w2 + 1 + sh;
    float xq[U];
#pragma unroll
    for (int m = 0; m < U; m += 2) {
        const F2 p = {x[m], x[m + 1]};
        const F2 q = f2sq(p);
        xq[m] = q.lo; xq[m + 1] = q.hi;
    }
    float zdS = g.zdS, zT = g.zT, zQ = g.zQ;
#pragma unroll
    for (int m0 = 0; m0 < U; m0 += 2) {
        float a1[2], b1[2]; double l1[2], v1[2], b1sq[2];
        float al[2]; double ll[2];
#pragma unroll
        for (int h = 0; h < 2; h++) {
            const int m = m0 + h;
            const double xd = widen_pos(x[m]);
            const double qd = widen_pos(xq[m]);
            const double pn = dadd(g.P[m & M1], EDGE ? (x[m] > 0.0f ? xd : 0.0) : xd);
            const double pqn = dadd(g.PQ[m & M1], EDGE ? (x[m] > 0.0f ? qd : 0.0) : qd);
            g.P[(m + 1) & M1] = pn;
            g.PQ[(m + 1) & M1] = pqn;
            const int s1 = (m - w1 + 1) & M1;
            const int s1l = (m - 2 * w1 + 1) & M1;
            const double d1 = dsub(pn, g.P[s1]), e1 = dsub(pqn, g.PQ[s1]);
            window_terms<w1>(d1, e1, a1[h], l1[h], b1[h], v1[h], b1sq[h]);
            al[h] = g.A1[s1l]; ll[h] = g.L1[s1l];
        }
        bool k0 = true, k1 = true;
        tstat_two<w1>(al[0], ll[0], b1[0], v1[0], b1sq[0], al[1], ll[1], b1[1], v1[1], b1sq[1], t1v[m0], k0, t1v[m0 + 1], k1);
#pragma unroll
        for (int h = 0; h < 2; h++) {
            const int m = m0 + h;
            bool kh = h ? k1 : k0;
            const int j1 = tau0 + m - w1 + 1;
            if (EDGE) {
                const bool in1 = (j1 >= w1) & (j1 + w1 <= n);
                kh = kh | !in1;
                t1v[m] = in1 ? t1v[m] : 0.0f;
            }
            if (m >= U - w1) ok_t1 = ok_t1 & kh; else ok = ok & kh;
            const int s1 = (m - w1 + 1) & M1;
            g.A1[s1] = a1[h]; g.L1[s1] = l1[h];
        }
#pragma unroll
        for (int h = 0; h < 2; h++) {
            const int m = m0 + h;
            const float zn = z[m];
            const float zm = m >= w2 ? z[m >= w2 ? m - w2 : 0] : g.Z1[m < w2 ? m + U - w2 : 0];
            const float zo = m >= 2 * w2 - U ? g.Z1[m >= 2 * w2 - U ? m + U - 2 * w2 : 0] : g.Z2[m < 2 * w2 - U ? m : 0];
#if defined(WALK_X_NOCAND)
            zT = fadd(zT, zn); (void)zm; (void)zo;
            bool cand = false;
#else
            zT = fadd(zT, fsub(zn, zo));
            zQ = fadd(zQ, fsub(fmul(zn, zn), fmul(zo, zo)));
            zdS = fadd(fadd(zdS, fadd(zn, zo)), fmul(zm, -2.0f));
            bool cand = long_candidate(zdS, zT, zQ, lk);
#endif
            const int j2 = tau0 + m - w2 + 1;
            if (EDGE) cand = cand & (j2 >= w2) & (j2 + w2 <= n);
            cand = cand | (zdirty > 0);
            const float c1 = m >= w1 ? t1v[m >= w1 ? m - w1 : 0] : g.T1c[m < w1 ? m : 0];
#if defined(WALK_X_NODET)
            d.s_pv = fadd(d.s_pv, c1); d.l_hot = d.l_hot | cand;
#elif defined(WALK_X_NOLIFE)
            { bool mk_; int p2_; const int over_ = det_one<true, RNA>(d.s_pv, d.s_ps, m, u0 + m, c1, thr_short<RNA>(), acc, mk_, p2_, NoEmit());
              acc.oldest = acc.oldest > over_ ? acc.oldest : over_; d.l_hot = d.l_hot | (cand & mk_); d.l_start += p2_ & 1; }
#else
            if (!EDGE || (j2 >= 1 && j2 < n)) det_step<RNA, false>(d, m, u0 + m, c1, cand, rec, acc, NoEmit(), io);
#endif
        }
    }
    g.zdS = zdS; g.zT = zT; g.zQ = zQ;
#pragma unroll
    for (int k = 0; k < Rings<RNA>::ZH2; k++) g.Z2[k] = g.Z1[k + U - Rings<RNA>::ZH2];
#pragma unroll
    for (int k = 0; k < U; k++) g.Z1[k] = z[k];
#if defined(WALK_TEST_REDO)
    ok = ok & ((tau0 / U) % 3 != 0);
#endif
    if (dirty > 0) { ok = false; ok_t1 = false; }
    if ((!ok & live) | (!ok_t1 & live_t1) | (rec & ((acc.oldest > PkCfg<RNA>::FAR) | (acc.jobs > 1)))) {
        Redo<RNA> in;
        in.d = d0; in.acc = acc;
#pragma unroll
        for (int k = 0; k < w1; k++) in.t1c[k] = g.T1c[k];
        const Redo<RNA> r = redo_block<RNA, EDGE>(io, in, tau0, n, sh, rec, off, unit, lk.thr);
        d = r.d; acc = r.acc;
#pragma unroll
        for (int k = 0; k < w1; k++) t1v[U - w1 + k] = r.t1c[k];
    }
    if (rec && acc.mk) io.peaks32(u0 - PkCfg<RNA>::LEAD, acc.mk);
    if (acc.jobs == 1) io.job(acc.job_ls, acc.job_end);
#pragma unroll
    for (int k = 0; k < w1; k++) g.T1c[k] = t1v[U - w1 + k];
}

SGW_HD uint32_t n_chunks(uint32_t n, uint32_t L) { return (n + L - 1u) / L; }

SGW_HD void cvt8(const int (&v)[4], float off, float unit, float c0, float* x, float* z) {
    const F2 bias = {8421376.0f, 8421376.0f}, off2 = {off, off}, unit2 = {unit, unit}, c2 = {c0, c0};
#pragma unroll
    for (int k = 0; k < 4; k++) {
        const uint32_t w = (uint32_t)v[k] ^ 0x80008000u;
        F2 r;
        r.lo = bits_f(0x4b000000u | (w & 0xffffu));
        r.hi = bits_f(0x4b000000u | (w >> 16));
        r = f2sub(r, bias);
        const F2 zz = f2sub(r, c2);
        r = f2mul(f2add(r, off2), unit2);
        x[2 * k] = r.lo;
        x[2 * k + 1] = r.hi;
        z[2 * k] = zz.lo;
        z[2 * k + 1] = zz.hi;
    }
}
SGW_HD void cvt8(const int (&v)[4], float off, float unit, float* x) {
    const F2 bias = {8421376.0f, 8421376.0f}, off2 = {off, off}, unit2 = {unit, unit};
#pragma unroll
    for (int k = 0; k < 4; k++) {
        const uint32_t w = (uint32_t)v[k] ^ 0x80008000u;
        F2 r;
        r.lo = bits_f(0x4b000000u | (w & 0xffffu));
        r.hi = bits_f(0x4b000000u | (w >> 16));
        r = f2mul(f2add(f2sub(r, bias), off2), unit2);
        x[2 * k] = r.lo;
        x[2 * k + 1] = r.hi;
    }
}
#if defined(__CUDA_ARCH__)
SGW_HD uint32_t min_s16x2(uint32_t a, uint32_t b) { return __vmins2(a, b); }
SGW_HD uint32_t max_s16x2(uint32_t a, uint32_t b) { return __vmaxs2(a, b); }
#else
SGW_HD uint32_t min_s16x2(uint32_t a, uint32_t b) {
    const int16_t al = (int16_t)(a & 0xffff), ah = (int16_t)(a >> 16), bl = (int16_t)(b & 0xffff), bh = (int16_t)(b >> 16);
    return (uint32_t)(uint16_t)(al < bl ? al : bl) | ((uint32_t)(uint16_t)(ah < bh ? ah : bh) << 16);
}
SGW_HD uint32_t max_s16x2(uint32_t a, uint32_t b) {
    const int16_t al = (int16_t)(a & 0xffff), ah = (int16_t)(a >> 16), bl = (int16_t)(b & 0xffff), bh = (int16_t)(b >> 16);
    return (uint32_t)(uint16_t)(al > bl ? al : bl) | ((uint32_t)(uint16_t)(ah > bh ? ah : bh) << 16);
}
#endif

#if defined(__CUDA_ARCH__)
SGW_HD bool any_le_s16x2(uint32_t a, uint32_t b) { return __vcmples2(a, b) != 0u; }
#else
SGW_HD bool any_le_s16x2(uint32_t a, uint32_t b) {
    return (int16_t)(a & 0xffff) <= (int16_t)(b & 0xffff) || (int16_t)(a >> 16) <= (int16_t)(b >> 16);
}
#endif
constexpr int LOW_MARGIN = 64;
SGW_HD int low_threshold(float off, bool* can) {
    float tf = floorf(-off);
    tf = tf < -40000.0f ? -40000.0f : tf > 40000.0f ? 40000.0f : tf;
    int t = (int)tf;
    for (int k = 0; k < 4 && fadd((float)(t + 1), off) <= 0.0f; k++) t++;
    for (int k = 0; k < 4 && fadd((float)t, off) > 0.0f; k++) t--;
    t += LOW_MARGIN;
    *can = t >= -32768;
    return t > 32767 ? 32767 : t < -32768 ? -32768 : t;
}
SGW_HD uint32_t pack_s16x2(int t) { return ((uint32_t)t & 0xffffu) * 0x10001u; }
SGW_HD int s16_lo(uint32_t v) { return (int)(int16_t)(v & 0xffffu); }
SGW_HD int s16_hi(uint32_t v) { return (int)v >> 16; }

SGW_HD int pivot_of(int a, int b, int c) {
    const int lo = a < b ? a : b, hi = a < b ? b : a;
    return c < lo ? lo : c > hi ? hi : c;
}

template <class Io>
SGW_HD void zero_low8(Io& io, int t, const int (&v)[4], int low_t, float* x) {
    uint32_t lo = 0xffffffffu, hi = 0u;
#pragma unroll
    for (int q = 0; q < 8; q++) {
        const int raw = (q & 1) ? (v[q >> 1] >> 16) : (int)(int16_t)(v[q >> 1] & 0xffff);
        if (raw <= low_t) {
            const uint32_t a = f_bits(x[q]) & 0x7fffffffu;
            if (a != 0u) { lo = a < lo ? a : lo; hi = a > hi ? a : hi; }
            x[q] = 0.0f;
        }
    }
    io.low_samples(t, lo, hi);
}

struct BlockCvt {
    bool can_low, zlo_on, zhi_on, pa;
    int low_t;
    uint32_t low2, zlo2, zhi2;
};
SGW_HD BlockCvt block_cvt(float off, int c0, bool want_pa) {
    BlockCvt k;
    k.low_t = low_threshold(off, &k.can_low);
    k.low2 = pack_s16x2(k.low_t);
    k.zlo2 = pack_s16x2(c0 - ZMAX - 1 < -32768 ? -32768 : c0 - ZMAX - 1);
    k.zhi2 = pack_s16x2(c0 + ZMAX + 1 > 32767 ? 32767 : c0 + ZMAX + 1);
    k.zlo_on = c0 - ZMAX - 1 >= -32768; k.zhi_on = c0 + ZMAX + 1 <= 32767;
    k.pa = want_pa;
    return k;
}
template <class Io>
SGW_HD void cvt_group(Io& io, const BlockCvt& k, const LongK& lk, const int (&v)[4], int t8, bool own, float off, float unit,
                      float* x, float* z, uint32_t& bmin, uint32_t& bmax, int& dirty) {
    const uint32_t m8 = min_s16x2(min_s16x2((uint32_t)v[0], (uint32_t)v[1]), min_s16x2((uint32_t)v[2], (uint32_t)v[3]));
    bmin = min_s16x2(bmin, m8);
    bmax = max_s16x2(max_s16x2(bmax, (uint32_t)v[0]), max_s16x2((uint32_t)v[1], max_s16x2((uint32_t)v[2], (uint32_t)v[3])));
    cvt8(v, off, unit, lk.c0, x, z);
    if (k.pa && own) io.store_pa8(t8, x);
    if (k.can_low & any_le_s16x2(m8, k.low2)) {
        dirty = DIRTY_BLOCKS;
        zero_low8(io, t8, v, k.low_t, x);
    }
}
template <int U>
SGW_HD void clamp_far(const BlockCvt& k, uint32_t bmin, uint32_t bmax, float* z, int& zdirty) {
    if ((k.zlo_on & any_le_s16x2(bmin, k.zlo2)) | (k.zhi_on & any_le_s16x2(k.zhi2, bmax))) {
        zdirty = DIRTY_BLOCKS;
#pragma unroll
        for (int q = 0; q < U; q++)
            z[q] = z[q] > (float)(ZMAX + 1) ? (float)(ZMAX + 1) : z[q] < -(float)(ZMAX + 1) ? -(float)(ZMAX + 1) : z[q];
    }
}

#if !defined(WALK_PF_BLOCKS)
#define WALK_PF_BLOCKS 12
#endif

template <int RNA, class Io>
SGW_HD void walk_interior(Io& io, int n, float off, float unit, int sh, int L, int W, int k, float thr_long) {
    using C = Cfg<RNA>;
    constexpr int U = C::U;
    const int s0 = k * L, s1 = s0 + L;
    const int t_live = s0 - W;
    Rings<RNA> g;
    g.clear();
    WalkDet d;
    det_cold(d, 0);
    float x[U], z[U];
    int v[4];
    uint32_t vmin = 0x7fff7fffu, vmax = 0x80008000u;
    int dirty = 0, zdirty = 0;
    int vn[U / 8][4];
#pragma unroll
    for (int h = 0; h < U / 8; h++) io.load8(t_live - C::FILL * U + 8 * h, vn[h]);
    const int c0 = pivot_of(s16_lo((uint32_t)vn[0][0]), s16_hi((uint32_t)vn[0][0]), s16_lo((uint32_t)vn[0][1]));
    const LongK lk = long_consts<RNA>(c0, off, thr_long);
    const BlockCvt bc = block_cvt(off, c0, io.want_pa());
#pragma unroll 1
    for (int tau = t_live - C::FILL * U; tau < s1; tau += U) {
        const bool own = tau >= s0;
        if (tau == t_live) det_cold(d, t_live - C::LAG + sh);
        if (tau == s0) {
            io.put_begin(canon_of<RNA>(d, s0 - C::LAG + sh));
            d.l_start = LS_PRED; d.l_hot = false;
        }
        const int tn = tau + U < s1 ? tau + U : tau;
        io.prefetch(tau + WALK_PF_BLOCKS * U < s1 ? tau + WALK_PF_BLOCKS * U : tau);
        uint32_t bmin = 0x7fff7fffu, bmax = 0x80008000u;
#pragma unroll
        for (int h = 0; h < U / 8; h++) {
#pragma unroll
            for (int q = 0; q < 4; q++) v[q] = vn[h][q];
            io.load8(tn + 8 * h, vn[h]);
            cvt_group(io, bc, lk, v, tau + 8 * h, own, off, unit, x + 8 * h, z + 8 * h, bmin, bmax, dirty);
        }
        vmin = min_s16x2(vmin, bmin);
        vmax = max_s16x2(vmax, bmax);
        clamp_far<U>(bc, bmin, bmax, z, zdirty);
        walk_block<RNA, false>(g, d, x, z, tau, n, sh, own, tau >= t_live, tau >= t_live - U, dirty, zdirty, off, unit, lk, io);
        dirty = dirty > 0 ? dirty - 1 : 0;
        zdirty = zdirty > 0 ? zdirty - 1 : 0;
    }
    if (d.l_hot) io.job(d.l_start, LS_CONT);
    io.put_end(canon_of<RNA>(d, s1 - C::LAG + sh));
    const int rmin0 = s16_lo(vmin), rmin1 = s16_hi(vmin);
    const int rmax0 = s16_lo(vmax), rmax1 = s16_hi(vmax);
    io.witness(rmin0 < rmin1 ? rmin0 : rmin1, rmax0 > rmax1 ? rmax0 : rmax1, bc.can_low ? bc.low_t : -32769);
}

#if defined(__CUDACC__)
#define SGW_PHASE __host__ __device__ __noinline__
#else
#define SGW_PHASE inline
#endif
template <int RNA>
struct EdgeCtx {
    Rings<RNA> g;
    WalkDet d;
    int rmin, rmax, dirty, zdirty;
    int n, sh, s0, s1, t_live, last, low_t, c0;
    float off, unit;
    bool pa;
    LongK lk;
    BlockCvt bc;
};
template <int RNA, class Io>
SGW_HD void edge_block_begin(Io& io, EdgeCtx<RNA>& e, int tau) {
    using C = Cfg<RNA>;
    if (e.last && tau == e.t_live) det_cold(e.d, e.t_live - C::LAG + e.sh);
    if (e.last && tau == e.s0) {
        io.put_begin(canon_of<RNA>(e.d, e.s0 - C::LAG + e.sh));
        e.d.l_start = LS_PRED; e.d.l_hot = false;
    }
}
template <int RNA, class Io>
SGW_PHASE void edge_inner(Io& io, EdgeCtx<RNA>& ec, int tau_from, int tau_to) {
    using C = Cfg<RNA>;
    constexpr int U = C::U;
    const int turns = io.warp_max(tau_to > tau_from ? (tau_to - tau_from) / U : 0);
    EdgeCtx<RNA> e = ec;
    float x[U], z[U];
    int vn[U / 8][4];
    if (tau_from < tau_to) {
#pragma unroll
        for (int h = 0; h < U / 8; h++) io.load8(tau_from + 8 * h, vn[h]);
    }
    int tau = tau_from;
#pragma unroll 1
    for (int turn = 0; turn < turns; turn++, tau += U) {
        if (tau >= tau_to) continue;
        const bool own = tau >= e.s0;
        edge_block_begin<RNA>(io, e, tau);
        const int tn = tau + U < tau_to ? tau + U : tau;
        io.prefetch(tau + WALK_PF_BLOCKS * U < tau_to ? tau + WALK_PF_BLOCKS * U : tau);
        uint32_t bmin = 0x7fff7fffu, bmax = 0x80008000u;
#pragma unroll
        for (int h = 0; h < U / 8; h++) {
            int v[4];
#pragma unroll
            for (int q = 0; q < 4; q++) v[q] = vn[h][q];
            io.load8(tn + 8 * h, vn[h]);
            cvt_group(io, e.bc, e.lk, v, tau + 8 * h, own, e.off, e.unit, x + 8 * h, z + 8 * h, bmin, bmax, e.dirty);
        }
        if (own) {
            const int b0 = s16_lo(bmin), b1 = s16_hi(bmin), c0x = s16_lo(bmax), c1x = s16_hi(bmax);
            e.rmin = b0 < e.rmin ? b0 : e.rmin; e.rmin = b1 < e.rmin ? b1 : e.rmin;
            e.rmax = c0x > e.rmax ? c0x : e.rmax; e.rmax = c1x > e.rmax ? c1x : e.rmax;
        }
        clamp_far<U>(e.bc, bmin, bmax, z, e.zdirty);
        walk_block<RNA, false>(e.g, e.d, x, z, tau, e.n, e.sh, own, tau >= e.t_live, tau >= e.t_live - U, e.dirty, e.zdirty,
                               e.off, e.unit, e.lk, io);
        e.dirty = e.dirty > 0 ? e.dirty - 1 : 0;
        e.zdirty = e.zdirty > 0 ? e.zdirty - 1 : 0;
    }
    ec = e;
}
template <int RNA, class Io>
SGW_PHASE void edge_checked(Io& io, EdgeCtx<RNA>& ec, int tau_from, int tau_to) {
    using C = Cfg<RNA>;
    constexpr int U = C::U;
    const int turns = io.warp_max(tau_to > tau_from ? (tau_to - tau_from) / U : 0);
    EdgeCtx<RNA> e = ec;
    float x[U], z[U];
    const int n = e.n, c0 = e.c0, low_t = e.low_t;
    int tau = tau_from;
#pragma unroll 1
    for (int turn = 0; turn < turns; turn++, tau += U) {
        if (tau >= tau_to) continue;
        const bool own = tau >= e.s0;
        edge_block_begin<RNA>(io, e, tau);
#pragma unroll
        for (int h = 0; h < U / 8; h++) {
            const int t8 = tau + 8 * h;
            int v[4] = {0, 0, 0, 0};
            if (t8 < n) io.load8(t8, v);
            float y[8], zy[8];
            cvt8(v, e.off, e.unit, e.lk.c0, y, zy);
#pragma unroll
            for (int q = 0; q < 8; q++) {
                const bool in = t8 + q < n;
                const int raw = (q & 1) ? (v[q >> 1] >> 16) : (int)(int16_t)(v[q >> 1] & 0xffff);
                const bool low = in & (raw <= low_t);
                x[8 * h + q] = (in & !low) ? y[q] : 0.0f;
                const bool zbad = in & ((raw - c0 > ZMAX) | (c0 - raw > ZMAX));
                z[8 * h + q] = !in ? 0.0f : !zbad ? zy[q] : raw > c0 ? (float)(ZMAX + 1) : -(float)(ZMAX + 1);
                if (zbad) e.zdirty = DIRTY_BLOCKS;
                if (low) {
                    e.dirty = DIRTY_BLOCKS;
                    const uint32_t a = f_bits(y[q]) & 0x7fffffffu;
                    io.low_samples(t8 + q, a != 0u ? a : 0xffffffffu, a);
                }
                if (own && in && t8 + q < e.s1) {
                    e.rmin = raw < e.rmin ? raw : e.rmin;
                    e.rmax = raw > e.rmax ? raw : e.rmax;
                    if (e.pa) io.store_pa1(t8 + q, y[q]);
                }
            }
        }
        walk_block<RNA, true>(e.g, e.d, x, z, tau, n, e.sh, own, tau >= e.t_live, tau >= e.t_live - U, e.dirty, e.zdirty,
                              e.off, e.unit, e.lk, io);
        e.dirty = e.dirty > 0 ? e.dirty - 1 : 0;
        e.zdirty = e.zdirty > 0 ? e.zdirty - 1 : 0;
    }
    ec = e;
}

template <int RNA, class Io>
SGW_HD void walk_edge(Io& io, int n, float off, float unit, int sh, int L, int W, int last, float thr_long) {
    using C = Cfg<RNA>;
    constexpr int U = C::U;
    const uint32_t nch = n_chunks((uint32_t)n, (uint32_t)L);
    const bool none = nch == 0u || (last && nch < 2u);
    EdgeCtx<RNA> e;
    e.n = n; e.sh = sh; e.off = off; e.unit = unit; e.last = last;
    e.s0 = last ? (int)(nch - 1u) * L : 0;
    const bool to_end = last || nch == 1u;
    e.s1 = to_end ? n : L;
    e.t_live = last ? e.s0 - W : 0;
    const int step_end = to_end ? n : e.s1 - C::LAG;
    e.g.clear();
    det_cold(e.d, sh + 1);
    e.rmin = 32767; e.rmax = -32768;
    bool can_low;
    const int low_t0 = low_threshold(off, &can_low);
    e.low_t = can_low ? low_t0 : -32769;
    e.dirty = 0; e.zdirty = 0;
    e.pa = io.want_pa();
    const int t_first = last ? e.t_live - C::FILL * U : 0;
    e.c0 = 0;
    if (!none) {
        int v0[4] = {0, 0, 0, 0};
        io.load8(t_first, v0);
        const int a = s16_lo((uint32_t)v0[0]), b = t_first + 1 < n ? s16_hi((uint32_t)v0[0]) : a;
        e.c0 = pivot_of(a, b, t_first + 2 < n ? s16_lo((uint32_t)v0[1]) : a);
    }
    e.lk = long_consts<RNA>(e.c0, off, thr_long);
    e.bc = block_cvt(off, e.c0, e.pa);
    constexpr int INNER_MIN = (2 * C::w2 - 1 + U - 1) / U * U;
    const int tau_end = none ? t_first : (step_end + C::LAG + U - 1) / U * U;
    int in0 = t_first > INNER_MIN ? t_first : INNER_MIN;
    in0 = in0 < tau_end ? in0 : tau_end;
    int in1 = n / U * U;
    in1 = in1 < tau_end ? in1 : tau_end;
    in1 = in1 > in0 ? in1 : in0;
    edge_checked<RNA>(io, e, t_first, in0);
    edge_inner<RNA>(io, e, in0, in1);
    edge_checked<RNA>(io, e, in1, tau_end);
    if (none) return;
    if (to_end) {
        if (e.d.l_hot) io.job(e.d.l_start, n + sh);
    } else {
        if (e.d.l_hot) io.job(e.d.l_start, LS_CONT);
        io.put_end(canon_of<RNA>(e.d, e.s1 - C::LAG + sh));
    }
    if (!last) io.peak(sh);
    if (e.rmin <= e.rmax) io.witness(e.rmin, e.rmax, e.low_t);
}

template <int RNA, class Jo>
SGW_HD void long_job(Jo& io, int n, int sh, float off, float unit, int L, int k, int l_start, int end, float thr_long) {
    using C = Cfg<RNA>;
    constexpr int w1 = C::w1, w2 = C::w2;
    for (int kk = k - 1; l_start == LS_PRED && kk >= 0; kk--) l_start = io.end_lstart(kk);
    if (l_start == LS_PRED) return;
    const int stop = n + sh;
    const int own_end = end == LS_CONT ? (k + 1) * L - C::LAG + sh : (end < stop ? end : stop);
    float pv = FLT_MAX; int ps = PS_NONE;
    PeakAcc unused; unused.mk = 0u; unused.oldest = 0;
    bool b2; int p2;
    SlidingT<Jo> slide;
    int u = l_start;
    for (; u + 4 <= own_end; u += 4) {
        float t[4];
#pragma unroll
        for (int q = 0; q < 4; q++) t[q] = slide.next(io, u + q - sh, w2, n, off, unit);
#pragma unroll
        for (int q = 0; q < 4; q++)
            det_one<false, RNA>(pv, ps, 0, u + q, t[q], thr_long, unused, b2, p2, [&](int pos) { io.peak(pos); });
    }
    for (; u < own_end; u++)
        det_one<false, RNA>(pv, ps, 0, u, slide.next(io, u - sh, w2, n, off, unit), thr_long, unused, b2, p2,
                            [&](int pos) { io.peak(pos); });
    if (end != LS_CONT) return;
    float spv; int sps;
    io.end_short(k, &spv, &sps);
    u = own_end;
    SlidingT<Jo> slide1;
    for (; u < stop; u++) {
        const float t1 = slide1.next(io, u - sh, w1, n, off, unit);
        const float t2 = slide.next(io, u - sh, w2, n, off, unit);
        det_one<true, RNA>(spv, sps, 0, u, t1, thr_short<RNA>(), unused, b2, p2, NoEmit());
        if (b2) return;
        det_one<false, RNA>(pv, ps, 0, u, t2, thr_long, unused, b2, p2, [&](int pos) { io.peak(pos); });
    }
}

}
}
```

Baseline: 127.0.

## Precompute long-window candidate bitmap in a separate pass before chunk walk

Adds a long_cand kernel that computes, for every sample, a bit marking whether the long t-stat window could fire, and stores it in a new bitmap. The walk kernels then read 32-bit candidate words and funnel-shift them per block, instead of keeping z-rings and running running-sum candidate tests inline. This removes register pressure and per-sample arithmetic from the sequential walk. In exchange it costs an extra full pass over the samples, a new scratch buffer and an extra kernel launch.

```diff
diff --git a/sigtk_b200/csrc/capi.cu b/sigtk_b200/csrc/capi.cu
--- a/sigtk_b200/csrc/capi.cu
+++ b/sigtk_b200/csrc/capi.cu
@@ -333,6 +333,7 @@
             marks.done("init", n);
         } else {
             marks.done("init", n);
+            marks.done("long_cand", launch_long_cand(b, sc, ctx->sm_count, st));
             marks.done("walk_chunks", launch_walk(b, sc, pa, seq, ctx->sm_count, st));
             marks.done("long_jobs", launch_long_jobs(b, sc, seq, ctx->sm_count, st));
             marks.done("verify_chunks", launch_verify_chunks(b, sc, seq, fix, ctx->sm_count, st));
@@ -639,6 +640,7 @@
     sc.max_tiles = fast_tiles_for(max_samples) + 1;
     sc.bitmap_words = (uint64_t)sc.max_tiles * (FAST_TILE / 32);
     CUC(sc.bitmap.ensure(sc.bitmap_words));
+    CUC(sc.cand.ensure(sc.bitmap_words + 1));
     sc.wk_slots = walk_state_slots(max_samples, max_reads);
     CUC(sc.wk_begin.ensure(sc.wk_slots * 8));
     CUC(sc.wk_end.ensure(sc.wk_slots * 8));
diff --git a/sigtk_b200/csrc/common.cuh b/sigtk_b200/csrc/common.cuh
--- a/sigtk_b200/csrc/common.cuh
+++ b/sigtk_b200/csrc/common.cuh
@@ -121,4 +121,14 @@
     return lo;
 }
 
+__device__ __forceinline__ uint32_t locate_read(const DevBatch& b, uint32_t r0, uint64_t p) {
+    uint32_t r = r0;
+#pragma unroll 1
+    for (int k = 0; k < 4; k++) {
+        if (r + 1 >= b.n_reads || b.read_off[r + 1] > p) return r;
+        r++;
+    }
+    return find_read(b.read_off, b.n_reads, p);
 }
+
+}
diff --git a/sigtk_b200/csrc/emit.cu b/sigtk_b200/csrc/emit.cu
--- a/sigtk_b200/csrc/emit.cu
+++ b/sigtk_b200/csrc/emit.cu
@@ -16,16 +16,6 @@
     double Q[EFAST + 32];
     uint16_t list[ELIST];
 };
-
-__device__ __forceinline__ uint32_t locate_read(const DevBatch& b, uint32_t r0, uint64_t p) {
-    uint32_t r = r0;
-#pragma unroll 1
-    for (int k = 0; k < 4; k++) {
-        if (r + 1 >= b.n_reads || b.read_off[r + 1] > p) return r;
-        r++;
-    }
-    return find_read(b.read_off, b.n_reads, p);
-}
 
 __device__ __forceinline__ void add_raw(int raw, float off, float unit, double& as, double& aq) {
     const float x = __fmul_rn(__fadd_rn((float)raw, off), unit);
diff --git a/sigtk_b200/csrc/kernels.cuh b/sigtk_b200/csrc/kernels.cuh
--- a/sigtk_b200/csrc/kernels.cuh
+++ b/sigtk_b200/csrc/kernels.cuh
@@ -57,6 +57,7 @@
     DevBuf<uint32_t> bitmap; uint64_t bitmap_words;
     DevBuf<uint32_t> tile_cnt; DevBuf<uint64_t> tile_base;
     DevBuf<uint32_t> tile_read0;
+    DevBuf<uint32_t> cand;
     DevBuf<uint32_t> wk_cnt;
     DevBuf<uint64_t> wk_ibase;
     DevBuf<int> wk_begin, wk_end;
@@ -88,6 +89,7 @@
 uint32_t fast_tiles_for(uint64_t span);
 int launch_init_reads(const DevBatch& b, Scratch& sc, uint32_t* seq_flag, uint32_t* fixups, int sm_count,
                       cudaStream_t st);
+int launch_long_cand(const DevBatch& b, Scratch& sc, int sm_count, cudaStream_t st);
 int launch_walk(const DevBatch& b, Scratch& sc, float* pa_out, uint32_t* seq_flag, int sm_count, cudaStream_t st);
 int launch_long_jobs(const DevBatch& b, Scratch& sc, uint32_t* seq_flag, int sm_count, cudaStream_t st);
 int launch_verify_chunks(const DevBatch& b, Scratch& sc, uint32_t* seq_flag, uint32_t* fixups, int sm_count, cudaStream_t st);
diff --git a/sigtk_b200/csrc/walk.cu b/sigtk_b200/csrc/walk.cu
--- a/sigtk_b200/csrc/walk.cu
+++ b/sigtk_b200/csrc/walk.cu
@@ -14,6 +14,12 @@
 #endif
 #ifndef WALK_MINB
 #define WALK_MINB 3
+#endif
+#ifndef WALK_CAND_NW
+#define WALK_CAND_NW 1
+#endif
+#ifndef WALK_CAND_MINB
+#define WALK_CAND_MINB 1
 #endif
 #ifndef WALK_MINB_RNA
 #define WALK_MINB_RNA 2
@@ -31,6 +37,7 @@
     uint32_t* wit_min;
     uint32_t* wit_max;
     uint32_t* tile_read0;
+    const uint32_t* cand;
     uint32_t edge_blocks;
     float thr_long;
     int4* jobs;
@@ -49,6 +56,7 @@
     uint32_t* __restrict__ wit_min;
     uint32_t* __restrict__ wit_max;
     uint32_t* __restrict__ tile_read0;
+    const uint32_t* __restrict__ cand;
     uint64_t base;
     float off, unit;
     int4* __restrict__ jobs;
@@ -63,6 +71,7 @@
         v[0] = w.x; v[1] = w.y; v[2] = w.z; v[3] = w.w;
     }
     __device__ __forceinline__ bool want_pa() const { return pa != nullptr; }
+    __device__ __forceinline__ uint32_t cand32(int q) const { return __ldg(cand + q); }
     __device__ __forceinline__ void prefetch(int t) const {
 #if !defined(WALK_NO_PREFETCH)
         asm volatile("prefetch.global.L1 [%0];" ::"l"(sp + t));
@@ -124,6 +133,7 @@
     io.wit_min = p.wit_min + r;
     io.wit_max = p.wit_max + r;
     io.tile_read0 = p.tile_read0;
+    io.cand = p.cand + (base >> 5);
     io.base = base;
     io.off = p.b.offset[r];
     io.unit = p.b.unit[r];
@@ -169,6 +179,48 @@
     const int k = (int)(i - p.ibase[r]) + 1;
     DevIo io = make_io(p, r, 2ull * p.b.n_reads + i, k, &sh);
     walk_interior<RNA>(io, (int)p.b.read_len[r], io.off, io.unit, sh, p.L, p.W, k, p.thr_long);
+}
+
+struct CandIo {
+    const int16_t* __restrict__ sp;
+    __device__ __forceinline__ void load8(int t, int (&v)[4]) const {
+        const int4 w = __ldg(reinterpret_cast<const int4*>(sp + t));
+        v[0] = w.x; v[1] = w.y; v[2] = w.z; v[3] = w.w;
+    }
+};
+
+constexpr int CAND_NW = WALK_CAND_NW;
+
+template <int RNA>
+__global__ void __launch_bounds__(256, WALK_CAND_MINB) long_cand_kernel(const DevBatch b, const uint32_t* __restrict__ tile_read0,
+                                                        uint32_t* __restrict__ cand, uint64_t n_units, float thr_long) {
+    const uint64_t stride = (uint64_t)gridDim.x * blockDim.x;
+    for (uint64_t u = (uint64_t)blockIdx.x * blockDim.x + threadIdx.x; u < n_units; u += stride) {
+        const uint64_t w0 = u * CAND_NW, p0 = w0 << 5;
+#if !defined(WALK_CAND_NOPF)
+        const uint64_t pn = p0 + (stride * CAND_NW << 5);
+        if (pn < b.span) {
+            asm volatile("prefetch.global.L2 [%0];" ::"l"(b.samples + pn));
+            asm volatile("prefetch.global.L2 [%0];" ::"l"(b.samples + pn + 32u * CAND_NW - 1u));
+            asm volatile("prefetch.global.L2 [%0];" ::"l"(tile_read0 + pn / FAST_TILE));
+        }
+#endif
+        uint32_t bits[CAND_NW];
+#pragma unroll
+        for (int w = 0; w < CAND_NW; w++) bits[w] = 0u;
+        if (p0 < b.span) {
+            for (uint32_t r = locate_read(b, tile_read0[p0 / FAST_TILE], p0); r < b.n_reads && b.read_off[r] < p0 + 32u * CAND_NW; r++) {
+                const uint64_t base = b.read_off[r];
+                const CandIo io{b.samples + base};
+                uint32_t o[CAND_NW];
+                cand_words<RNA, CAND_NW>(io, (int)(w0 - (base >> 5)), (int)b.read_len[r], (int)(base & 31u), b.offset[r], thr_long, o);
+#pragma unroll
+                for (int w = 0; w < CAND_NW; w++) bits[w] |= o[w];
+            }
+        }
+#pragma unroll
+        for (int w = 0; w < CAND_NW; w++) cand[w0 + w] = bits[w];
+    }
 }
 
 struct JobIo {
@@ -320,6 +372,7 @@
     WalkParams p;
     p.b = b; p.L = (int)L; p.W = (int)W; p.ibase = sc.wk_ibase; p.pa = pa_out; p.bitmap = sc.bitmap;
     p.st_begin = sc.wk_begin; p.st_end = sc.wk_end; p.wit_min = sc.wit_min; p.wit_max = sc.wit_max; p.tile_read0 = sc.tile_read0;
+    p.cand = sc.cand.get() + 1;
     p.edge_blocks = (uint32_t)((2ull * ((b.n_reads + 31u) & ~31u) + WNT - 1) / WNT);
     p.thr_long = sc.tune_thr_long;
     p.jobs = reinterpret_cast<int4*>(sc.jobs.get()); p.job_count = sc.job_count; p.job_cap = sc.job_cap; p.seq_flag = seq_flag;
@@ -341,6 +394,14 @@
     return n + 1;
 }
 
+int launch_long_cand(const DevBatch& b, Scratch& sc, int sm_count, cudaStream_t st) {
+    const uint64_t units = (uint64_t)fast_tiles_for(b.span) * (FAST_TILE / 32) / CAND_NW;
+    const int grid = grid_cap(units, 256, sm_count * 16);
+    if (b.rna) long_cand_kernel<1><<<grid, 256, 0, st>>>(b, sc.tile_read0, sc.cand.get() + 1, units, sc.tune_thr_long);
+    else long_cand_kernel<0><<<grid, 256, 0, st>>>(b, sc.tile_read0, sc.cand.get() + 1, units, sc.tune_thr_long);
+    return 1;
+}
+
 int launch_long_jobs(const DevBatch& b, Scratch& sc, uint32_t* seq_flag, int sm_count, cudaStream_t st) {
     const WalkParams p = walk_params(b, sc, nullptr, seq_flag, sm_count);
     if (b.rna) long_jobs_kernel<1><<<sm_count * 16, 128, 0, st>>>(p);
diff --git a/sigtk_b200/csrc/walk_core.cuh b/sigtk_b200/csrc/walk_core.cuh
--- a/sigtk_b200/csrc/walk_core.cuh
+++ b/sigtk_b200/csrc/walk_core.cuh
@@ -3,6 +3,8 @@
 #include <math.h>
 #include <stdint.h>
 #include <string.h>
+
+#include <utility>
 
 #if defined(__CUDACC__)
 #define SGW_HD __host__ __device__ __forceinline__
@@ -187,14 +189,17 @@
 }
 
 template <class Io>
-SGW_HD float sample_pa(const Io& io, int i, int n, float off, float unit) {
-    if (i < 0 || i >= n) return 0.0f;
+SGW_HD int raw_at(const Io& io, int i) {
     int v[4];
     io.load8(i & ~7, v);
     const int q = i & 7;
     const int word = q < 2 ? v[0] : q < 4 ? v[1] : q < 6 ? v[2] : v[3];
-    const int raw = (q & 1) ? (word >> 16) : (int)(int16_t)(word & 0xffff);
-    return fmul(fadd((float)raw, off), unit);
+    return (q & 1) ? (word >> 16) : (int)(int16_t)(word & 0xffff);
+}
+template <class Io>
+SGW_HD float sample_pa(const Io& io, int i, int n, float off, float unit) {
+    if (i < 0 || i >= n) return 0.0f;
+    return fmul(fadd((float)raw_at(io, i), off), unit);
 }
 template <class Io>
 SGW_HD void window_sums(const Io& io, int a, int w, int n, float off, float unit, double& S, double& Q) {
@@ -367,6 +372,15 @@
     const float rhs = fmul(Q, k.t2w);
     return !(lhs < rhs);
 }
+SGW_HD void long_candidate2(F2 dS, F2 T, F2 Q, const LongK& k, bool& lo, bool& hi) {
+    const F2 ad = {fabsf(dS.lo), fabsf(dS.hi)};
+    const F2 g = f2add(ad, F2{k.ca, k.ca});
+    const F2 sq = f2fma(T, T, f2mul(dS, dS));
+    const F2 lhs = f2fma(f2mul(g, g), F2{k.cw, k.cw}, f2fma(sq, F2{k.h2, k.h2}, F2{k.cB, k.cB}));
+    const F2 rhs = f2mul(Q, F2{k.t2w, k.t2w});
+    lo = !(lhs.lo < rhs.lo);
+    hi = !(lhs.hi < rhs.hi);
+}
 
 constexpr int DIRTY_BLOCKS = 3;
 static_assert(2 * Cfg<0>::w2 - 1 <= 2 * Cfg<0>::U + 0 && 2 * Cfg<1>::w2 - 1 <= 2 * Cfg<1>::U, "windows reach at most two blocks ahead");
@@ -378,19 +392,11 @@
     float A1[C::R1];
     double L1[C::R1];
     float T1c[C::w1];
-    static constexpr int ZH2 = 2 * C::w2 - C::U;
-    float Z1[C::U], Z2[ZH2];
-    float zdS, zT, zQ;
     SGW_HD void clear() {
 #pragma unroll
         for (int k = 0; k < C::R1; k++) { P[k] = 0.0; PQ[k] = 0.0; A1[k] = 0.0f; L1[k] = 0.0; }
 #pragma unroll
         for (int k = 0; k < C::w1; k++) T1c[k] = 0.0f;
-#pragma unroll
-        for (int k = 0; k < C::U; k++) Z1[k] = 0.0f;
-#pragma unroll
-        for (int k = 0; k < ZH2; k++) Z2[k] = 0.0f;
-        zdS = 0.0f; zT = 0.0f; zQ = 0.0f;
     }
 };
 
@@ -417,10 +423,9 @@
 #else
 inline
 #endif
-Redo<RNA> redo_block(Io& io, Redo<RNA> in, int tau0, int n, int sh, bool rec, float off, float unit, float thr_long) {
+Redo<RNA> redo_block(Io& io, Redo<RNA> in, int tau0, int n, int sh, bool rec, float off, float unit) {
     using C = Cfg<RNA>;
     constexpr int w1 = C::w1, w2 = C::w2, U = C::U;
-    (void)thr_long;
     float e1[U];
     SlidingT<Io> slide;
     for (int m = 0; m < U; m++) e1[m] = slide.next(io, tau0 + m - w1 + 1, w1, n, off, unit);
@@ -440,9 +445,8 @@
 }
 
 template <int RNA, bool EDGE, class Io>
-SGW_HD void walk_block(Rings<RNA>& g, WalkDet& d, const float (&x)[Cfg<RNA>::U], const float (&z)[Cfg<RNA>::U], int tau0,
-                       int n, int sh, bool rec, bool live, bool live_t1, int dirty, int zdirty, float off, float unit,
-                       const LongK& lk, Io& io) {
+SGW_HD void walk_block(Rings<RNA>& g, WalkDet& d, const float (&x)[Cfg<RNA>::U], int tau0, int n, int sh, bool rec,
+                       bool live, bool live_t1, int dirty, uint32_t cm, float off, float unit, Io& io) {
     using C = Cfg<RNA>;
     constexpr int w1 = C::w1, w2 = C::w2, M1 = C::R1 - 1, M2 = C::R2 - 1, U = C::U;
     float t1v[U];
@@ -458,7 +462,6 @@
         const F2 q = f2sq(p);
         xq[m] = q.lo; xq[m + 1] = q.hi;
     }
-    float zdS = g.zdS, zT = g.zT, zQ = g.zQ;
 #pragma unroll
     for (int m0 = 0; m0 < U; m0 += 2) {
         float a1[2], b1[2]; double l1[2], v1[2], b1sq[2];
@@ -497,37 +500,16 @@
 #pragma unroll
         for (int h = 0; h < 2; h++) {
             const int m = m0 + h;
-            const float zn = z[m];
-            const float zm = m >= w2 ? z[m >= w2 ? m - w2 : 0] : g.Z1[m < w2 ? m + U - w2 : 0];
-            const float zo = m >= 2 * w2 - U ? g.Z1[m >= 2 * w2 - U ? m + U - 2 * w2 : 0] : g.Z2[m < 2 * w2 - U ? m : 0];
-#if defined(WALK_X_NOCAND)
-            zT = fadd(zT, zn); (void)zm; (void)zo;
-            bool cand = false;
-#else
-            zT = fadd(zT, fsub(zn, zo));
-            zQ = fadd(zQ, fsub(fmul(zn, zn), fmul(zo, zo)));
-            zdS = fadd(fadd(zdS, fadd(zn, zo)), fmul(zm, -2.0f));
-            bool cand = long_candidate(zdS, zT, zQ, lk);
-#endif
+            const bool cand = (cm >> m) & 1u;
             const int j2 = tau0 + m - w2 + 1;
-            if (EDGE) cand = cand & (j2 >= w2) & (j2 + w2 <= n);
-            cand = cand | (zdirty > 0);
             const float c1 = m >= w1 ? t1v[m >= w1 ? m - w1 : 0] : g.T1c[m < w1 ? m : 0];
 #if defined(WALK_X_NODET)
             d.s_pv = fadd(d.s_pv, c1); d.l_hot = d.l_hot | cand;
-#elif defined(WALK_X_NOLIFE)
-            { bool mk_; int p2_; const int over_ = det_one<true, RNA>(d.s_pv, d.s_ps, m, u0 + m, c1, thr_short<RNA>(), acc, mk_, p2_, NoEmit());
-              acc.oldest = acc.oldest > over_ ? acc.oldest : over_; d.l_hot = d.l_hot | (cand & mk_); d.l_start += p2_ & 1; }
 #else
             if (!EDGE || (j2 >= 1 && j2 < n)) det_step<RNA, false>(d, m, u0 + m, c1, cand, rec, acc, NoEmit(), io);
 #endif
         }
     }
-    g.zdS = zdS; g.zT = zT; g.zQ = zQ;
-#pragma unroll
-    for (int k = 0; k < Rings<RNA>::ZH2; k++) g.Z2[k] = g.Z1[k + U - Rings<RNA>::ZH2];
-#pragma unroll
-    for (int k = 0; k < U; k++) g.Z1[k] = z[k];
 #if defined(WALK_TEST_REDO)
     ok = ok & ((tau0 / U) % 3 != 0);
 #endif
@@ -537,7 +519,7 @@
         in.d = d0; in.acc = acc;
 #pragma unroll
         for (int k = 0; k < w1; k++) in.t1c[k] = g.T1c[k];
-        const Redo<RNA> r = redo_block<RNA, EDGE>(io, in, tau0, n, sh, rec, off, unit, lk.thr);
+        const Redo<RNA> r = redo_block<RNA, EDGE>(io, in, tau0, n, sh, rec, off, unit);
         d = r.d; acc = r.acc;
 #pragma unroll
         for (int k = 0; k < w1; k++) t1v[U - w1 + k] = r.t1c[k];
@@ -550,23 +532,6 @@
 
 SGW_HD uint32_t n_chunks(uint32_t n, uint32_t L) { return (n + L - 1u) / L; }
 
-SGW_HD void cvt8(const int (&v)[4], float off, float unit, float c0, float* x, float* z) {
-    const F2 bias = {8421376.0f, 8421376.0f}, off2 = {off, off}, unit2 = {unit, unit}, c2 = {c0, c0};
-#pragma unroll
-    for (int k = 0; k < 4; k++) {
-        const uint32_t w = (uint32_t)v[k] ^ 0x80008000u;
-        F2 r;
-        r.lo = bits_f(0x4b000000u | (w & 0xffffu));
-        r.hi = bits_f(0x4b000000u | (w >> 16));
-        r = f2sub(r, bias);
-        const F2 zz = f2sub(r, c2);
-        r = f2mul(f2add(r, off2), unit2);
-        x[2 * k] = r.lo;
-        x[2 * k + 1] = r.hi;
-        z[2 * k] = zz.lo;
-        z[2 * k + 1] = zz.hi;
-    }
-}
 SGW_HD void cvt8(const int (&v)[4], float off, float unit, float* x) {
     const F2 bias = {8421376.0f, 8421376.0f}, off2 = {off, off}, unit2 = {unit, unit};
 #pragma unroll
@@ -637,41 +602,169 @@
 }
 
 struct BlockCvt {
-    bool can_low, zlo_on, zhi_on, pa;
+    bool can_low, pa;
     int low_t;
-    uint32_t low2, zlo2, zhi2;
+    uint32_t low2;
 };
-SGW_HD BlockCvt block_cvt(float off, int c0, bool want_pa) {
+SGW_HD BlockCvt block_cvt(float off, bool want_pa) {
     BlockCvt k;
     k.low_t = low_threshold(off, &k.can_low);
     k.low2 = pack_s16x2(k.low_t);
-    k.zlo2 = pack_s16x2(c0 - ZMAX - 1 < -32768 ? -32768 : c0 - ZMAX - 1);
-    k.zhi2 = pack_s16x2(c0 + ZMAX + 1 > 32767 ? 32767 : c0 + ZMAX + 1);
-    k.zlo_on = c0 - ZMAX - 1 >= -32768; k.zhi_on = c0 + ZMAX + 1 <= 32767;
     k.pa = want_pa;
     return k;
 }
 template <class Io>
-SGW_HD void cvt_group(Io& io, const BlockCvt& k, const LongK& lk, const int (&v)[4], int t8, bool own, float off, float unit,
-                      float* x, float* z, uint32_t& bmin, uint32_t& bmax, int& dirty) {
+SGW_HD void cvt_group(Io& io, const BlockCvt& k, const int (&v)[4], int t8, bool own, float off, float unit, float* x,
+                      uint32_t& bmin, uint32_t& bmax, int& dirty) {
     const uint32_t m8 = min_s16x2(min_s16x2((uint32_t)v[0], (uint32_t)v[1]), min_s16x2((uint32_t)v[2], (uint32_t)v[3]));
     bmin = min_s16x2(bmin, m8);
     bmax = max_s16x2(max_s16x2(bmax, (uint32_t)v[0]), max_s16x2((uint32_t)v[1], max_s16x2((uint32_t)v[2], (uint32_t)v[3])));
-    cvt8(v, off, unit, lk.c0, x, z);
+    cvt8(v, off, unit, x);
     if (k.pa && own) io.store_pa8(t8, x);
     if (k.can_low & any_le_s16x2(m8, k.low2)) {
         dirty = DIRTY_BLOCKS;
         zero_low8(io, t8, v, k.low_t, x);
     }
 }
-template <int U>
-SGW_HD void clamp_far(const BlockCvt& k, uint32_t bmin, uint32_t bmax, float* z, int& zdirty) {
-    if ((k.zlo_on & any_le_s16x2(bmin, k.zlo2)) | (k.zhi_on & any_le_s16x2(k.zhi2, bmax))) {
-        zdirty = DIRTY_BLOCKS;
-#pragma unroll
-        for (int q = 0; q < U; q++)
-            z[q] = z[q] > (float)(ZMAX + 1) ? (float)(ZMAX + 1) : z[q] < -(float)(ZMAX + 1) ? -(float)(ZMAX + 1) : z[q];
-    }
+
+template <int RNA, int NW> struct CandCfg {
+    static constexpr int w2 = Cfg<RNA>::w2;
+    static constexpr int H = 16 * NW;
+    static constexpr int PRE = (w2 + 7) / 8 * 8;
+    static constexpr int G = (32 * NW + 2 * PRE) / 8;
+    static constexpr int NP = H - 1 + 2 * w2;
+};
+template <int RNA, int NW, class Io>
+SGW_HD void cand_words(const Io& io, int q, int n, int sh, float off, float thr_long, uint32_t (&out)[NW]) {
+    using K = CandCfg<RNA, NW>;
+    constexpr int w2 = K::w2, H = K::H, PRE = K::PRE, G = K::G, NP = K::NP;
+    const int j0 = 32 * q - sh;
+    uint32_t range[NW];
+    bool any = false;
+#pragma unroll
+    for (int w = 0; w < NW; w++) {
+        const int klo = w2 - j0 - 32 * w, khi = n - w2 - j0 - 32 * w;
+        range[w] = (khi < 0 || klo > 31 || khi < klo) ? 0u
+                   : (0xffffffffu << (klo > 0 ? klo : 0)) & (0xffffffffu >> (khi < 31 ? 31 - khi : 0));
+        any = any | (range[w] != 0u);
+        out[w] = 0u;
+    }
+    if (!any) return;
+    const int a0 = j0 - PRE;
+    int v[G][4];
+    int c0;
+    if (a0 >= 0 && a0 + 8 * G <= n) {
+#pragma unroll
+        for (int g = 0; g < G; g++) io.load8(a0 + 8 * g, v[g]);
+        constexpr int gp = (PRE + H) / 8;
+        c0 = pivot_of(s16_lo((uint32_t)v[gp][0]), s16_hi((uint32_t)v[gp][0]), s16_lo((uint32_t)v[gp][1]));
+    } else {
+        const int ip = j0 + H < 0 ? 0 : j0 + H > n - 3 ? n - 3 : j0 + H;
+        c0 = pivot_of(raw_at(io, ip), raw_at(io, ip + 1), raw_at(io, ip + 2));
+        const uint32_t cc = pack_s16x2(c0);
+#pragma unroll
+        for (int g = 0; g < G; g++) {
+            const int t8 = a0 + 8 * g;
+            v[g][0] = 0; v[g][1] = 0; v[g][2] = 0; v[g][3] = 0;
+            if (t8 >= 0 && t8 < n) io.load8(t8, v[g]);
+#pragma unroll
+            for (int h = 0; h < 4; h++) {
+                const int i = t8 + 2 * h;
+                const uint32_t m = ((i >= 0) & (i < n) ? 0xffffu : 0u) | ((i + 1 >= 0) & (i + 1 < n) ? 0xffff0000u : 0u);
+                v[g][h] = (int)(((uint32_t)v[g][h] & m) | (cc & ~m));
+            }
+        }
+    }
+    uint32_t mn = 0x7fff7fffu, mx = 0x80008000u;
+#pragma unroll
+    for (int g = 0; g < G; g++)
+#pragma unroll
+        for (int h = 0; h < 4; h++) { mn = min_s16x2(mn, (uint32_t)v[g][h]); mx = max_s16x2(mx, (uint32_t)v[g][h]); }
+    const int rmin = s16_lo(mn) < s16_hi(mn) ? s16_lo(mn) : s16_hi(mn);
+    const int rmax = s16_lo(mx) > s16_hi(mx) ? s16_lo(mx) : s16_hi(mx);
+    if ((rmax - c0 > ZMAX) | (c0 - rmin > ZMAX)) {
+#pragma unroll
+        for (int w = 0; w < NW; w++) out[w] = range[w];
+        return;
+    }
+    const float cz = 8421376.0f + (float)c0;
+    auto pair = [&](int i) -> F2 {
+        const int a = PRE - w2 + i, b = a + H;
+        const uint32_t wa = (uint32_t)v[a >> 3][(a & 7) >> 1] ^ 0x80008000u, wb = (uint32_t)v[b >> 3][(b & 7) >> 1] ^ 0x80008000u;
+        const F2 f = {bits_f(0x4b000000u | ((a & 1) ? (wa >> 16) : (wa & 0xffffu))),
+                      bits_f(0x4b000000u | ((b & 1) ? (wb >> 16) : (wb & 0xffffu)))};
+        return f2sub(f, F2{cz, cz});
+    };
+    F2 P[NP];
+#pragma unroll
+    for (int i = 0; i < 2 * w2; i++) P[i] = pair(i);
+    F2 sl = P[0], sr = P[w2], Q = f2sq(P[0]);
+#pragma unroll
+    for (int i = 1; i < w2; i++) { sl = f2add(sl, P[i]); sr = f2add(sr, P[w2 + i]); }
+#pragma unroll
+    for (int i = 1; i < 2 * w2; i++) Q = f2fma(P[i], P[i], Q);
+    F2 T = f2add(sl, sr), dS = f2sub(sr, sl);
+    const LongK lk = long_consts<RNA>(c0, off, thr_long);
+    const F2 m2 = {-2.0f, -2.0f};
+#pragma unroll
+    for (int k = 0; k < H; k++) {
+        bool c_lo, c_hi;
+        long_candidate2(dS, T, Q, lk, c_lo, c_hi);
+        out[k >> 5] |= c_lo ? 1u << (k & 31) : 0u;
+        out[(k + H) >> 5] |= c_hi ? 1u << ((k + H) & 31) : 0u;
+        if (k < H - 1) {
+            P[k + 2 * w2] = pair(k + 2 * w2);
+            const F2 zn = P[k + 2 * w2], zm = P[k + w2], zo = P[k];
+            const F2 dz = f2sub(zn, zo), sz = f2add(zn, zo);
+            T = f2add(T, dz);
+            Q = f2fma(dz, sz, Q);
+            dS = f2fma(zm, m2, f2add(dS, sz));
+        }
+    }
+#pragma unroll
+    for (int w = 0; w < NW; w++) out[w] &= range[w];
+}
+template <int RNA, class Io>
+SGW_HD uint32_t cand_word(const Io& io, int q, int n, int sh, float off, float thr_long) {
+    uint32_t o[1];
+    cand_words<RNA, 1>(io, q, n, sh, off, thr_long, o);
+    return o[0];
+}
+
+template <class T, class = void> struct HasCand { static constexpr bool value = false; };
+template <class T> struct HasCand<T, decltype((void)std::declval<const T&>().cand32(0))> { static constexpr bool value = true; };
+template <int RNA, class Io>
+SGW_HD uint32_t cand_at(const Io& io, int q, int n, int sh, float off, float thr_long) {
+    if constexpr (HasCand<Io>::value) {
+        (void)n; (void)sh; (void)off; (void)thr_long;
+        return io.cand32(q);
+    } else {
+        return cand_word<RNA>(io, q, n, sh, off, thr_long);
+    }
+}
+SGW_HD uint32_t funnel_r(uint32_t lo, uint32_t hi, int s) {
+    return (uint32_t)((((uint64_t)hi << 32) | lo) >> s);
+}
+struct CandRun {
+    uint32_t cur, nxt;
+    int n, sh;
+    float off, thr_long;
+};
+template <int RNA, class Io>
+SGW_HD CandRun cand_start(const Io& io, int u0, int n, int sh, float off, float thr_long) {
+    CandRun c;
+    c.n = n; c.sh = sh; c.off = off; c.thr_long = thr_long;
+    c.cur = cand_at<RNA>(io, u0 >> 5, n, sh, off, thr_long);
+    c.nxt = cand_at<RNA>(io, (u0 + Cfg<RNA>::U - 1) >> 5, n, sh, off, thr_long);
+    return c;
+}
+template <int RNA, class Io>
+SGW_HD uint32_t cand_block(const Io& io, CandRun& c, int u0) {
+    constexpr int U = Cfg<RNA>::U;
+    const uint32_t cm = funnel_r(c.cur, c.nxt, u0 & 31) & (0xffffffffu >> (32 - U));
+    c.cur = c.nxt;
+    c.nxt = cand_at<RNA>(io, (u0 + 2 * U - 1) >> 5, c.n, c.sh, c.off, c.thr_long);
+    return cm;
 }
 
 #if !defined(WALK_PF_BLOCKS)
@@ -688,16 +781,15 @@
     g.clear();
     WalkDet d;
     det_cold(d, 0);
-    float x[U], z[U];
+    float x[U];
     int v[4];
     uint32_t vmin = 0x7fff7fffu, vmax = 0x80008000u;
-    int dirty = 0, zdirty = 0;
+    int dirty = 0;
     int vn[U / 8][4];
 #pragma unroll
     for (int h = 0; h < U / 8; h++) io.load8(t_live - C::FILL * U + 8 * h, vn[h]);
-    const int c0 = pivot_of(s16_lo((uint32_t)vn[0][0]), s16_hi((uint32_t)vn[0][0]), s16_lo((uint32_t)vn[0][1]));
-    const LongK lk = long_consts<RNA>(c0, off, thr_long);
-    const BlockCvt bc = block_cvt(off, c0, io.want_pa());
+    const BlockCvt bc = block_cvt(off, io.want_pa());
+    CandRun cr = cand_start<RNA>(io, t_live - C::FILL * U - C::LAG + sh, n, sh, off, thr_long);
 #pragma unroll 1
     for (int tau = t_live - C::FILL * U; tau < s1; tau += U) {
         const bool own = tau >= s0;
@@ -708,20 +800,19 @@
         }
         const int tn = tau + U < s1 ? tau + U : tau;
         io.prefetch(tau + WALK_PF_BLOCKS * U < s1 ? tau + WALK_PF_BLOCKS * U : tau);
+        const uint32_t cm = cand_block<RNA>(io, cr, tau - C::LAG + sh);
         uint32_t bmin = 0x7fff7fffu, bmax = 0x80008000u;
 #pragma unroll
         for (int h = 0; h < U / 8; h++) {
 #pragma unroll
             for (int q = 0; q < 4; q++) v[q] = vn[h][q];
             io.load8(tn + 8 * h, vn[h]);
-            cvt_group(io, bc, lk, v, tau + 8 * h, own, off, unit, x + 8 * h, z + 8 * h, bmin, bmax, dirty);
+            cvt_group(io, bc, v, tau + 8 * h, own, off, unit, x + 8 * h, bmin, bmax, dirty);
         }
         vmin = min_s16x2(vmin, bmin);
         vmax = max_s16x2(vmax, bmax);
-        clamp_far<U>(bc, bmin, bmax, z, zdirty);
-        walk_block<RNA, false>(g, d, x, z, tau, n, sh, own, tau >= t_live, tau >= t_live - U, dirty, zdirty, off, unit, lk, io);
+        walk_block<RNA, false>(g, d, x, tau, n, sh, own, tau >= t_live, tau >= t_live - U, dirty, cm, off, unit, io);
         dirty = dirty > 0 ? dirty - 1 : 0;
-        zdirty = zdirty > 0 ? zdirty - 1 : 0;
     }
     if (d.l_hot) io.job(d.l_start, LS_CONT);
     io.put_end(canon_of<RNA>(d, s1 - C::LAG + sh));
@@ -739,12 +830,12 @@
 struct EdgeCtx {
     Rings<RNA> g;
     WalkDet d;
-    int rmin, rmax, dirty, zdirty;
-    int n, sh, s0, s1, t_live, last, low_t, c0;
+    int rmin, rmax, dirty;
+    int n, sh, s0, s1, t_live, last, low_t;
     float off, unit;
     bool pa;
-    LongK lk;
     BlockCvt bc;
+    CandRun cr;
 };
 template <int RNA, class Io>
 SGW_HD void edge_block_begin(Io& io, EdgeCtx<RNA>& e, int tau) {
@@ -761,7 +852,7 @@
     constexpr int U = C::U;
     const int turns = io.warp_max(tau_to > tau_from ? (tau_to - tau_from) / U : 0);
     EdgeCtx<RNA> e = ec;
-    float x[U], z[U];
+    float x[U];
     int vn[U / 8][4];
     if (tau_from < tau_to) {
 #pragma unroll
@@ -775,6 +866,7 @@
         edge_block_begin<RNA>(io, e, tau);
         const int tn = tau + U < tau_to ? tau + U : tau;
         io.prefetch(tau + WALK_PF_BLOCKS * U < tau_to ? tau + WALK_PF_BLOCKS * U : tau);
+        const uint32_t cm = cand_block<RNA>(io, e.cr, tau - C::LAG + e.sh);
         uint32_t bmin = 0x7fff7fffu, bmax = 0x80008000u;
 #pragma unroll
         for (int h = 0; h < U / 8; h++) {
@@ -782,18 +874,16 @@
 #pragma unroll
             for (int q = 0; q < 4; q++) v[q] = vn[h][q];
             io.load8(tn + 8 * h, vn[h]);
-            cvt_group(io, e.bc, e.lk, v, tau + 8 * h, own, e.off, e.unit, x + 8 * h, z + 8 * h, bmin, bmax, e.dirty);
+            cvt_group(io, e.bc, v, tau + 8 * h, own, e.off, e.unit, x + 8 * h, bmin, bmax, e.dirty);
         }
         if (own) {
             const int b0 = s16_lo(bmin), b1 = s16_hi(bmin), c0x = s16_lo(bmax), c1x = s16_hi(bmax);
             e.rmin = b0 < e.rmin ? b0 : e.rmin; e.rmin = b1 < e.rmin ? b1 : e.rmin;
             e.rmax = c0x > e.rmax ? c0x : e.rmax; e.rmax = c1x > e.rmax ? c1x : e.rmax;
         }
-        clamp_far<U>(e.bc, bmin, bmax, z, e.zdirty);
-        walk_block<RNA, false>(e.g, e.d, x, z, tau, e.n, e.sh, own, tau >= e.t_live, tau >= e.t_live - U, e.dirty, e.zdirty,
-                               e.off, e.unit, e.lk, io);
+        walk_block<RNA, false>(e.g, e.d, x, tau, e.n, e.sh, own, tau >= e.t_live, tau >= e.t_live - U, e.dirty, cm, e.off,
+                               e.unit, io);
         e.dirty = e.dirty > 0 ? e.dirty - 1 : 0;
-        e.zdirty = e.zdirty > 0 ? e.zdirty - 1 : 0;
     }
     ec = e;
 }
@@ -803,30 +893,28 @@
     constexpr int U = C::U;
     const int turns = io.warp_max(tau_to > tau_from ? (tau_to - tau_from) / U : 0);
     EdgeCtx<RNA> e = ec;
-    float x[U], z[U];
-    const int n = e.n, c0 = e.c0, low_t = e.low_t;
+    float x[U];
+    const int n = e.n, low_t = e.low_t;
     int tau = tau_from;
 #pragma unroll 1
     for (int turn = 0; turn < turns; turn++, tau += U) {
         if (tau >= tau_to) continue;
         const bool own = tau >= e.s0;
         edge_block_begin<RNA>(io, e, tau);
+        const uint32_t cm = cand_block<RNA>(io, e.cr, tau - C::LAG + e.sh);
 #pragma unroll
         for (int h = 0; h < U / 8; h++) {
             const int t8 = tau + 8 * h;
             int v[4] = {0, 0, 0, 0};
             if (t8 < n) io.load8(t8, v);
-            float y[8], zy[8];
-            cvt8(v, e.off, e.unit, e.lk.c0, y, zy);
+            float y[8];
+            cvt8(v, e.off, e.unit, y);
 #pragma unroll
             for (int q = 0; q < 8; q++) {
                 const bool in = t8 + q < n;
                 const int raw = (q & 1) ? (v[q >> 1] >> 16) : (int)(int16_t)(v[q >> 1] & 0xffff);
                 const bool low = in & (raw <= low_t);
                 x[8 * h + q] = (in & !low) ? y[q] : 0.0f;
-                const bool zbad = in & ((raw - c0 > ZMAX) | (c0 - raw > ZMAX));
-                z[8 * h + q] = !in ? 0.0f : !zbad ? zy[q] : raw > c0 ? (float)(ZMAX + 1) : -(float)(ZMAX + 1);
-                if (zbad) e.zdirty = DIRTY_BLOCKS;
                 if (low) {
                     e.dirty = DIRTY_BLOCKS;
                     const uint32_t a = f_bits(y[q]) & 0x7fffffffu;
@@ -839,10 +927,9 @@
                 }
             }
         }
-        walk_block<RNA, true>(e.g, e.d, x, z, tau, n, e.sh, own, tau >= e.t_live, tau >= e.t_live - U, e.dirty, e.zdirty,
-                              e.off, e.unit, e.lk, io);
+        walk_block<RNA, true>(e.g, e.d, x, tau, n, e.sh, own, tau >= e.t_live, tau >= e.t_live - U, e.dirty, cm, e.off,
+                              e.unit, io);
         e.dirty = e.dirty > 0 ? e.dirty - 1 : 0;
-        e.zdirty = e.zdirty > 0 ? e.zdirty - 1 : 0;
     }
     ec = e;
 }
@@ -866,18 +953,11 @@
     bool can_low;
     const int low_t0 = low_threshold(off, &can_low);
     e.low_t = can_low ? low_t0 : -32769;
-    e.dirty = 0; e.zdirty = 0;
+    e.dirty = 0;
     e.pa = io.want_pa();
     const int t_first = last ? e.t_live - C::FILL * U : 0;
-    e.c0 = 0;
-    if (!none) {
-        int v0[4] = {0, 0, 0, 0};
-        io.load8(t_first, v0);
-        const int a = s16_lo((uint32_t)v0[0]), b = t_first + 1 < n ? s16_hi((uint32_t)v0[0]) : a;
-        e.c0 = pivot_of(a, b, t_first + 2 < n ? s16_lo((uint32_t)v0[1]) : a);
-    }
-    e.lk = long_consts<RNA>(e.c0, off, thr_long);
-    e.bc = block_cvt(off, e.c0, e.pa);
+    e.bc = block_cvt(off, e.pa);
+    e.cr = cand_start<RNA>(io, t_first - C::LAG + sh, n, sh, off, thr_long);
     constexpr int INNER_MIN = (2 * C::w2 - 1 + U - 1) / U * U;
     const int tau_end = none ? t_first : (step_end + C::LAG + U - 1) / U * U;
     int in0 = t_first > INNER_MIN ? t_first : INNER_MIN;
```

Measured after the change: 123.4 (median of 6 runs). 0.972x the previous value.
